# abhisrkckl/PulsePortraiture

Hardware: AMD Instinct MI355X
Metric: subint portrait fits/sec (phase+DM, 512ch×2048bin) at 1/2/4/8 MI355X (higher is better)
Workload: dtype f64

## Files before the change

pulseportraiture_amd/csrc/ppf_api.cpp:

```cpp
#include <hip/hip_runtime.h>

#include <algorithm>
#include <atomic>
#include <chrono>
#include <cmath>
#include <cstdarg>
#include <cstdio>
#include <cstdlib>
#include <cstring>
#include <map>
#include <mutex>
#include <string>
#include <thread>
#include <utility>
#include <vector>

#include "../../include/ppfit.h"
#include "ppf_internal.hpp"
#include "ppf_device.hpp"

struct ppf_ctx {
    int device;
    std::string err;
    mutable std::mutex err_mu;
    std::map<int, double2 *> tw;
    std::map<std::pair<int, int>, double2 *> cz;
    std::mutex tw_mu;
    bool prof = false;
    static constexpr int kRing = 256;
    static constexpr int kEv = 9;
    hipEvent_t ring[kRing][kEv] = {};
    bool ran[kRing][6] = {};
    std::vector<std::pair<hipEvent_t, hipEvent_t>> pass_ev[kRing];
    int npass[kRing] = {};
    std::vector<std::pair<hipEvent_t, hipEvent_t>> solv_ev[kRing];
    std::vector<int> solv_kind[kRing];
    int nsolv[kRing] = {};
    long ncalls = 0;
    unsigned *host_active = nullptr;
    void *lscr = nullptr;
    size_t lscr_bytes = 0;
    std::mutex lscr_mu;
};

namespace {

int fail(ppf_ctx *ctx, int code, const char *fmt, ...) {
    char buf[512];
    va_list ap;
    va_start(ap, fmt);
    vsnprintf(buf, sizeof buf, fmt, ap);
    va_end(ap);
    if (ctx) {
        std::lock_guard<std::mutex> lk(ctx->err_mu);
        ctx->err = buf;
    }
    return code;
}

int hip_fail(ppf_ctx *ctx, hipError_t e, const char *where) {
    return fail(ctx, PPF_EHIP, "%s: %s", where, hipGetErrorString(e));
}

bool pow2_in_range(int nbin) {
    return nbin >= 32 && nbin <= 8192 && (nbin & (nbin - 1)) == 0;
}

bool nbin_supported(int nbin) {
    return nbin >= 32 && nbin <= 8192 && ppf::fft_len_supported(ppf::rfft_len(nbin));
}

int fft_log2(int n) {
    if (n < 1 || (n & (n - 1))) return 0;
    int l = 0;
    while ((1 << l) < n) ++l;
    return l;
}

int rfft_log2(int nbin) { return (nbin & 1) ? 0 : fft_log2(nbin / 2); }

int ilog2(int n) {
    int l = 0;
    while ((1 << l) < n) ++l;
    return l;
}

int noise_kc(int nharm, int frac) {
    return (int)((1.0 - std::pow((double)frac, -1.0)) * (double)nharm);
}

int twiddles(ppf_ctx *ctx, int nbin, hipStream_t st, const double2 **T, const double2 **T2) {
    std::lock_guard<std::mutex> lock(ctx->tw_mu);
    auto it = ctx->tw.find(nbin);
    if (it == ctx->tw.end()) {
        const int N = ppf::rfft_len(nbin);
        double2 *p = nullptr;
        hipError_t e = hipMalloc(&p, sizeof(double2) * 2 * (size_t)N);
        if (e != hipSuccess) return hip_fail(ctx, e, "hipMalloc(twiddles)");
        e = ppf::launch_twiddles(N, p, p + N, st);
        if (e != hipSuccess) return hip_fail(ctx, e, "k_twiddles");
        e = hipStreamSynchronize(st);
        if (e != hipSuccess) return hip_fail(ctx, e, "hipStreamSynchronize(twiddles)");
        it = ctx->tw.emplace(nbin, p).first;
    }
    *T = it->second;
    *T2 = it->second + ppf::rfft_len(nbin);
    return PPF_OK;
}

constexpr unsigned kUnset = 0xFFFFFFFFu;
int read_back(ppf_ctx *ctx, unsigned *host, const unsigned *dev, int n, hipStream_t st, bool spin) {
    volatile unsigned *h = host;
    for (int i = 0; i < n; ++i) h[i] = kUnset;
    std::atomic_thread_fence(std::memory_order_seq_cst);
    hipError_t e = hipMemcpyAsync(host, dev, n * sizeof(unsigned), hipMemcpyDeviceToHost, st);
    if (e != hipSuccess) return hip_fail(ctx, e, "hipMemcpyAsync");
    if (spin) {
        const auto t0 = std::chrono::steady_clock::now();
        for (;;) {
            bool done = true;
            for (int i = 0; i < n; ++i) done = done && h[i] != kUnset;
            if (done) {
                std::atomic_thread_fence(std::memory_order_seq_cst);
                return PPF_OK;
            }
            const auto dt = std::chrono::steady_clock::now() - t0;
            if (dt > std::chrono::seconds(2)) break;
            if (dt > std::chrono::microseconds(50)) std::this_thread::yield();
            else __builtin_ia32_pause();
        }
    }
    if ((e = hipStreamSynchronize(st)) != hipSuccess) return hip_fail(ctx, e, "hipStreamSynchronize");
    return PPF_OK;
}

bool cz_plan(int Ns, int K, ppf::CzPlan &c) {
    if (Ns < 2 * ppf::kBlock || K < 2) return false;
    int P = 64;
    while (P < K + 255) P *= 2;
    if (P < 512 || P > 2048) return false;
    c.Ns = Ns; c.K = K; c.P = P; c.J = P - K + 1; c.Q = (Ns + c.J - 1) / c.J;
    return true;
}
int cz_tables(ppf_ctx *ctx, const ppf::CzPlan &c, hipStream_t st, const double2 **B, const double2 **T) {
    const double2 *T2;
    int rc = twiddles(ctx, 2 * c.P, st, T, &T2);
    if (rc) return rc;
    std::lock_guard<std::mutex> lock(ctx->tw_mu);
    const auto key = std::make_pair(c.Ns, c.K);
    auto it = ctx->cz.find(key);
    if (it == ctx->cz.end()) {
        double2 *p = nullptr;
        hipError_t e = hipMalloc(&p, sizeof(double2) * (size_t)c.Q * c.P);
        if (e != hipSuccess) return hip_fail(ctx, e, "hipMalloc(cz)");
        e = ppf::launch_cz_table(c, p, *T, st);
        if (e != hipSuccess) return hip_fail(ctx, e, "k_cz_table");
        e = hipStreamSynchronize(st);
        if (e != hipSuccess) return hip_fail(ctx, e, "hipStreamSynchronize(cz)");
        it = ctx->cz.emplace(key, p).first;
    }
    *B = it->second;
    return PPF_OK;
}

struct FitLayout {
    size_t M, X, chan, stats, x0, gP, gw, nuref, Msum, gpart, gwx, gflag, state, partials, active, mom, dphi,
        mres, hcen, Mpow, MP, KC, needx, xslot, xtile, rclist, Bt, total;
    int lng;
    size_t spec, lchirp, lA, lY, gprof, gspec, gsh;
    int64_t lrows;
    int nblk, cb, cbd, nblkd;
    int fused;
    int momx;
    int xcap;
    int tiled;
    int xnh;
};

static bool mom16_layout(const FitLayout &L, int nbin) {
    return L.momx || (!L.fused && !ppf::is_pow2(ppf::rfft_len(nbin)));
}


size_t align256(size_t x) { return (x + 255) & ~(size_t)255; }

bool bluestein_plan(int64_t nbin, int64_t n, bool packed, ppf::LongNoiseArgs &a);

bool grid_gsh(int nbin, int Ns, bool lng) {
    const size_t fb = lng ? 0 : (size_t)ppf::rfft_len(nbin) * sizeof(double2);
    return fb + ((size_t)nbin / 2 + 2) * sizeof(double2) + (size_t)(Ns + 8) * sizeof(double) > 150u * 1024u;
}
bool long_fit_ok(const ppf_fit_desc *d) {
    ppf::LongNoiseArgs f;
    if (d->guess && ((size_t)d->nbin / 2 + 2) * sizeof(double2) > 150u * 1024u) return false;
    return !nbin_supported(d->nbin) && d->nbin > 4095 &&
           bluestein_plan(d->nbin, (d->nbin & 1) ? d->nbin : d->nbin / 2, !(d->nbin & 1), f);
}

FitLayout fit_layout(const ppf_fit_desc *d) {
    FitLayout L{};
    const size_t nharm = (size_t)d->nbin / 2 + 1;
    const size_t nsub = (size_t)d->nsub, nchan = (size_t)d->nchan;
    L.cb = d->nchan < 32 ? d->nchan : 32;
    L.nblk = (d->nchan + L.cb - 1) / L.cb;
    L.fused = ppf::xspec_wave_supported(rfft_log2(d->nbin), L.cb) ? 1 : 0;
    const bool mom_auto = d->guess && rfft_log2(d->nbin) == 10;
    L.momx = (L.fused && !(d->options & PPF_OPT_FUSED_MOM) &&
              ((d->options & PPF_OPT_MOM_X) || mom_auto)) ? 1 : 0;
    L.xcap = (L.fused && d->x_subints > 0 && d->x_subints < d->nsub) ? d->x_subints : d->nsub;
    if (L.fused && (d->options & PPF_OPT_NO_X)) L.xcap = 0;
    if (L.momx) L.xcap = d->nsub;
    L.cbd = d->nchan < 128 ? d->nchan : 128;
    L.nblkd = (d->nchan + L.cbd - 1) / L.cbd;
    size_t o = 0;
    L.M = o;     o += align256(sizeof(double2) * (size_t)(d->nmodel > 0 ? d->nmodel : 1) * nchan * nharm);
    L.tiled = (L.momx && ppf::xspec_tiled(rfft_log2(d->nbin))) ? 1 : 0;
    L.xnh = L.tiled ? (int)ppf::xtile_harm((int64_t)nharm) : (int)nharm;
    L.X = o;     o += align256(sizeof(double2) * (size_t)L.xcap * nchan * (size_t)L.xnh);
    L.chan = o;  o += align256(sizeof(double) * nsub * nchan * 4);
    L.stats = o; o += align256(sizeof(double) * nsub * 2 * nchan * 10);
    L.x0 = o;    o += align256(sizeof(double) * nsub * 8);
    L.state = o; o += align256(ppf::tr_state_bytes() * nsub);
    L.partials = o; o += align256(sizeof(double) * nsub * (size_t)ppf::pass_blocks(d->nchan) * 21);
    L.active = o; o += 256;
    L.mom = o;   o += align256(sizeof(double2) * nsub * 2 * nchan * (size_t)ppf::kMoments);
    L.dphi = o;  o += align256(sizeof(double) * nsub * nchan * 2);
    L.mres = o;  o += align256(sizeof(double) * nsub * 2 * nchan);
    L.hcen = o;  o += mom16_layout(L, d->nbin) ? align256(sizeof(double) * nsub * 2 * nchan) : 0;
    L.Mpow = o;  o += align256(sizeof(double) * (size_t)(d->nmodel > 0 ? d->nmodel : 1) * nchan);
    L.MP = o;    o += align256(sizeof(double) * (size_t)(d->nmodel > 0 ? d->nmodel : 1) * nchan * nharm);
    L.KC = o;    o += align256(sizeof(int32_t) * (size_t)(d->nmodel > 0 ? d->nmodel : 1) * nchan);
    L.needx = o; o += align256(nsub);
    L.xslot = o; o += align256(sizeof(int32_t) * nsub);
    L.xtile = o; o += L.tiled ? align256(nsub) : 0;
    L.rclist = o; o += align256(sizeof(int32_t) * nsub);
    L.Bt = o;    o += align256(sizeof(double) * (nharm - 1) / 2 * 16);
    if (d->guess) {
        L.gP = o; o += align256(sizeof(double) * nsub * (size_t)L.nblkd * (size_t)d->nbin);
        L.gw = o; o += align256(sizeof(double) * nsub * (size_t)L.nblkd * 2);
        L.nuref = o; o += align256(sizeof(double) * nsub);
        L.Msum = o; o += align256(sizeof(double2) * (size_t)(d->nmodel > 0 ? d->nmodel : 1) * nharm);
        if (L.fused) {
            const size_t ng = (size_t)ppf::guess_slots(rfft_log2(d->nbin));
            L.gpart = o; o += align256(sizeof(double2) * nsub * (size_t)L.nblk * ng);
            L.gwx = o;   o += align256(sizeof(double) * nsub * (size_t)L.nblk * 3);
            L.gflag = o; o += align256(nsub);
        }
    }
    L.lng = long_fit_ok(d) ? 1 : 0;
    if (L.lng) {
        ppf::LongNoiseArgs f;
        bluestein_plan(d->nbin, (d->nbin & 1) ? d->nbin : d->nbin / 2, !(d->nbin & 1), f);
        const size_t row_b = (size_t)f.M * sizeof(double2);
        const int64_t rows = (int64_t)(nsub > (size_t)(d->nmodel > 0 ? d->nmodel : 1) ? nsub
                                       : (size_t)(d->nmodel > 0 ? d->nmodel : 1)) * (int64_t)nchan;
        int64_t rc = (int64_t)((size_t)(256u << 20) / (2 * row_b));
        if (rc < 1) rc = 1;
        L.lrows = rows < rc ? rows : rc;
        L.spec = o;   o += align256(sizeof(double2) * nsub * nchan * nharm);
        if (d->guess) {
            L.gprof = o; o += align256(sizeof(double) * nsub * (size_t)d->nbin);
            L.gspec = o; o += align256(sizeof(double2) * nsub * nharm);
        }
        L.lchirp = o; o += align256(2 * row_b);
        L.lA = o;     o += align256((size_t)L.lrows * row_b);
        L.lY = o;     o += align256((size_t)L.lrows * row_b);
    }
    if (d->guess && grid_gsh(d->nbin, d->guess_Ns, L.lng)) {
        L.gsh = o; o += align256(sizeof(double) * nsub * ((size_t)d->guess_Ns + 8));
    }
    L.total = o;
    return L;
}

int long_rfft_rows(ppf_ctx *ctx, const FitLayout &L, char *ws, int64_t nbin, int64_t nrows, int dtype,
                   const void *in, double2 *out, bool chirp_ready, hipStream_t st) {
    ppf::LongNoiseArgs f;
    if (!bluestein_plan(nbin, (nbin & 1) ? nbin : nbin / 2, !(nbin & 1), f))
        return fail(ctx, PPF_EUNSUP, "nbin=%lld", (long long)nbin);
    const double2 *T1, *T2, *unused;
    int rc;
    if ((rc = twiddles(ctx, (int)(2 * f.M1), st, &T1, &unused))) return rc;
    if ((rc = twiddles(ctx, (int)(2 * f.M2), st, &T2, &unused))) return rc;
    double2 *Bf = (double2 *)(ws + L.lchirp);
    hipError_t e;
    if (!chirp_ready && (e = ppf::launch_chirp_ft(f, Bf, Bf + f.M, T1, T2, st)) != hipSuccess)
        return hip_fail(ctx, e, "k_lf_chirp");
    f.in_dtype = dtype;
    f.in = in;
    for (int64_t r0 = 0; r0 < nrows; r0 += L.lrows) {
        f.row0 = r0;
        const int64_t nr = nrows - r0 < L.lrows ? nrows - r0 : L.lrows;
        if ((e = ppf::launch_rfft_long(f, nr, (double2 *)(ws + L.lA), (double2 *)(ws + L.lY), Bf, out, T1, T2,
                                       st)) != hipSuccess)
            return hip_fail(ctx, e, "k_lr_spec");
    }
    return PPF_OK;
}

int check_fit_desc(ppf_ctx *ctx, const ppf_fit_desc *d) {
    if (!d) return fail(ctx, PPF_EINVAL, "null descriptor");
    if (d->nsub < 1 || d->nchan < 1) return fail(ctx, PPF_EINVAL, "nsub=%d nchan=%d", d->nsub, d->nchan);
    if (!nbin_supported(d->nbin) && !long_fit_ok(d))
        return fail(ctx, PPF_EUNSUP,
                    "nbin=%d: must be even in [32, 8192] or odd in [33, 4095], or longer without the "
                    "GetTOAs guess (up to 2^23 transform points)", d->nbin);
    if (d->data_dtype != PPF_F32 && d->data_dtype != PPF_F64)
        return fail(ctx, PPF_EINVAL, "data_dtype=%d", d->data_dtype);
    if (d->nmodel < 1) return fail(ctx, PPF_EINVAL, "nmodel=%d", d->nmodel);
    if (!d->data || !d->model || !d->freqs || !d->P || !d->init || !d->fit_flags || !d->nu_fits ||
        !d->nu_outs || !d->results || !d->scales || !d->scale_errs || !d->channel_snrs ||
        !d->covariance)
        return fail(ctx, PPF_EINVAL, "required pointer is NULL");
    if (d->mode != PPF_MODE_FULL && d->mode != PPF_MODE_LEGACY2)
        return fail(ctx, PPF_EINVAL, "mode=%d", d->mode);
    if (d->guess) {
        if (!d->guess_weights || !d->guess_DM) return fail(ctx, PPF_EINVAL, "guess needs weights and DM");
        if (d->guess_Ns < 1 || d->guess_Ns > 65536) return fail(ctx, PPF_EINVAL, "guess_Ns=%d", d->guess_Ns);
    }
    if (!d->workspace) return fail(ctx, PPF_EINVAL, "workspace is NULL");
    FitLayout L = fit_layout(d);
    if (d->workspace_bytes < L.total)
        return fail(ctx, PPF_ENOMEM, "workspace %zu < %zu bytes", d->workspace_bytes, L.total);
    return PPF_OK;
}

}

extern "C" {

int ppf_abi_version(void) { return PPF_ABI_VERSION; }
size_t ppf_sizeof_fit_desc(void) { return sizeof(ppf_fit_desc); }
size_t ppf_sizeof_result(void) { return sizeof(ppf_result); }

int ppf_create(int device, ppf_ctx **out) {
    if (!out) return PPF_EINVAL;
    *out = nullptr;
    int n = 0;
    hipError_t e = hipGetDeviceCount(&n);
    if (e != hipSuccess || n == 0) return PPF_EHIP;
    if (device < 0 || device >= n) return PPF_EINVAL;
    ppf_ctx *c = new ppf_ctx();
    c->device = device;
    *out = c;
    return PPF_OK;
}

void ppf_destroy(ppf_ctx *ctx) {
    if (!ctx) return;
    (void)hipSetDevice(ctx->device);
    for (auto &kv : ctx->tw) (void)hipFree(kv.second);
    for (auto &kv : ctx->cz) (void)hipFree(kv.second);
    for (auto &set : ctx->ring)
        for (auto &e : set)
            if (e) (void)hipEventDestroy(e);
    for (auto &v : ctx->pass_ev)
        for (auto &pr : v) {
            (void)hipEventDestroy(pr.first);
            (void)hipEventDestroy(pr.second);
        }
    for (auto &v : ctx->solv_ev)
        for (auto &pr : v) {
            (void)hipEventDestroy(pr.first);
            (void)hipEventDestroy(pr.second);
        }
    if (ctx->host_active) (void)hipHostFree(ctx->host_active);
    if (ctx->lscr) (void)hipFree(ctx->lscr);
    delete ctx;
}

int ppf_set_profiling(ppf_ctx *ctx, int enable) {
    if (!ctx) return PPF_EINVAL;
    hipError_t e = hipSetDevice(ctx->device);
    if (e != hipSuccess) return hip_fail(ctx, e, "hipSetDevice");
    if (enable && !ctx->ring[0][0])
        for (auto &set : ctx->ring)
            for (auto &ev : set)
                if ((e = hipEventCreate(&ev)) != hipSuccess) return hip_fail(ctx, e, "hipEventCreate");
    ctx->prof = enable != 0;
    ctx->ncalls = 0;
    return PPF_OK;
}

int ppf_stage_ms_history(ppf_ctx *ctx, int n, double *ms) {
    if (!ctx || !ms || n < 0) return PPF_EINVAL;
    if (!ctx->prof) return fail(ctx, PPF_EINVAL, "profiling is off");
    long avail = ctx->ncalls < ppf_ctx::kRing ? ctx->ncalls : ppf_ctx::kRing;
    if (n > avail) n = (int)avail;
    for (int c = 0; c < n; ++c) {
        int slot = (int)((ctx->ncalls - n + c) % ppf_ctx::kRing);
        hipError_t e = hipEventSynchronize(ctx->ring[slot][4]);
        if (e != hipSuccess) return hip_fail(ctx, e, "hipEventSynchronize");
        for (int i = 0; i < 4; ++i) {
            float t = 0.f;
            if (ctx->ran[slot][i]) {
                e = hipEventElapsedTime(&t, ctx->ring[slot][i], ctx->ring[slot][i + 1]);
                if (e != hipSuccess) return hip_fail(ctx, e, "hipEventElapsedTime");
            }
// ... 11 lines not shown
    for (int c = 0; c < n; ++c) {
        int slot = (int)((ctx->ncalls - n + c) % ppf_ctx::kRing);
        hipError_t e = hipEventSynchronize(ctx->ring[slot][4]);
        if (e != hipSuccess) return hip_fail(ctx, e, "hipEventSynchronize");
        for (int i = 0; i < 2; ++i) {
            float t = 0.f;
            if (ctx->ran[slot][4 + i]) {
                e = hipEventElapsedTime(&t, ctx->ring[slot][5 + 2 * i], ctx->ring[slot][6 + 2 * i]);
                if (e != hipSuccess) return hip_fail(ctx, e, "hipEventElapsedTime");
            }
            ms[c * 2 + i] = (double)t;
        }
    }
    return n;
}

int ppf_pass_ms_history(ppf_ctx *ctx, int n, double *ms) {
    if (!ctx || !ms || n < 0) return PPF_EINVAL;
    if (!ctx->prof) return fail(ctx, PPF_EINVAL, "profiling is off");
    long avail = ctx->ncalls < ppf_ctx::kRing ? ctx->ncalls : ppf_ctx::kRing;
    if (n > avail) n = (int)avail;
    for (int c = 0; c < n; ++c) {
        int slot = (int)((ctx->ncalls - n + c) % ppf_ctx::kRing);
        double tot = 0.0;
        for (int i = 0; i < ctx->npass[slot]; ++i) {
            const auto &pr = ctx->pass_ev[slot][i];
            hipError_t e = hipEventSynchronize(pr.second);
            if (e != hipSuccess) return hip_fail(ctx, e, "hipEventSynchronize");
            float t = 0.f;
            e = hipEventElapsedTime(&t, pr.first, pr.second);
            if (e != hipSuccess) return hip_fail(ctx, e, "hipEventElapsedTime");
            tot += (double)t;
        }
        ms[c * 2 + 0] = tot;
        ms[c * 2 + 1] = (double)ctx->npass[slot];
    }
    return n;
}

int ppf_solver_ms_history(ppf_ctx *ctx, int n, double *ms) {
    if (!ctx || !ms || n < 0) return PPF_EINVAL;
    if (!ctx->prof) return fail(ctx, PPF_EINVAL, "profiling is off");
    long avail = ctx->ncalls < ppf_ctx::kRing ? ctx->ncalls : ppf_ctx::kRing;
    if (n > avail) n = (int)avail;
    for (int c = 0; c < n; ++c) {
        int slot = (int)((ctx->ncalls - n + c) % ppf_ctx::kRing);
        double *o = ms + c * 6;
        for (int i = 0; i < 6; ++i) o[i] = 0.0;
        for (int i = 0; i < ctx->nsolv[slot]; ++i) {
            const auto &pr = ctx->solv_ev[slot][i];
            hipError_t e = hipEventSynchronize(pr.second);
            if (e != hipSuccess) return hip_fail(ctx, e, "hipEventSynchronize");
            float t = 0.f;
            e = hipEventElapsedTime(&t, pr.first, pr.second);
            if (e != hipSuccess) return hip_fail(ctx, e, "hipEventElapsedTime");
            const int k = ctx->solv_kind[slot][i];
            o[2 * k] += (double)t;
            o[2 * k + 1] += 1.0;
        }
    }
    return n;
}

int ppf_last_stage_ms(ppf_ctx *ctx, double *ms4) {
    int n = ppf_stage_ms_history(ctx, 1, ms4);
    if (n < 0) return n;
    return n == 1 ? PPF_OK : fail(ctx, PPF_EINVAL, "no profiled call yet");
}

const char *ppf_last_error(const ppf_ctx *ctx) {
    if (!ctx) return "null context";
    thread_local std::string copy;
    std::lock_guard<std::mutex> lk(ctx->err_mu);
    copy = ctx->err;
    return copy.c_str();
}

size_t ppf_fit_workspace_bytes(const ppf_fit_desc *desc) {
    if (!desc || desc->nsub < 1 || desc->nchan < 1 || (!nbin_supported(desc->nbin) && !long_fit_ok(desc)))
        return 0;
    return fit_layout(desc).total;
}

int ppf_fit_batch(ppf_ctx *ctx, const ppf_fit_desc *d, void *stream) {
    if (!ctx) return PPF_EINVAL;
    int rc = check_fit_desc(ctx, d);
    if (rc) return rc;
    hipError_t e = hipSetDevice(ctx->device);
    if (e != hipSuccess) return hip_fail(ctx, e, "hipSetDevice");
    hipStream_t st = (hipStream_t)stream;
    const FitLayout L = fit_layout(d);
    const double2 *T = nullptr, *T2 = nullptr;
    if (!L.lng && (rc = twiddles(ctx, d->nbin, st, &T, &T2))) return rc;
    char *ws = (char *)d->workspace;
    double2 *Mft = (double2 *)(ws + L.M);
    const int nharm = d->nbin / 2 + 1;
    const int kc = noise_kc(nharm, 4);

    const int slot = (int)(ctx->ncalls % ppf_ctx::kRing);
    auto mark = [&](int i) {
        if (ctx->prof) (void)hipEventRecord(ctx->ring[slot][i], st);
    };
    for (int i = 0; i < 4; ++i) ctx->ran[slot][i] = true;
    ctx->npass[slot] = 0;
    ctx->nsolv[slot] = 0;
    auto solv_begin = [&](int kind) -> std::pair<hipEvent_t, hipEvent_t> * {
        if (!ctx->prof) return nullptr;
        auto &v = ctx->solv_ev[slot];
        auto &kv = ctx->solv_kind[slot];
        if ((int)v.size() <= ctx->nsolv[slot]) {
            std::pair<hipEvent_t, hipEvent_t> pr{};
            if (hipEventCreate(&pr.first) != hipSuccess) return nullptr;
            if (hipEventCreate(&pr.second) != hipSuccess) {
                (void)hipEventDestroy(pr.first);
                return nullptr;
            }
            v.push_back(pr);
            kv.push_back(0);
        }
        kv[ctx->nsolv[slot]] = kind;
        auto *pe = &v[ctx->nsolv[slot]++];
        (void)hipEventRecord(pe->first, st);
        return pe;
    };
    auto solv_end = [&](std::pair<hipEvent_t, hipEvent_t> *pe) {
        if (pe) (void)hipEventRecord(pe->second, st);
    };
    ctx->ran[slot][2] = d->guess != 0;
    ctx->ran[slot][4] = ctx->ran[slot][5] = false;
    mark(0);
    if (L.lng) {
        if ((rc = long_rfft_rows(ctx, L, ws, d->nbin, (int64_t)d->nmodel * d->nchan, PPF_F64, d->model, Mft,
                                 false, st)))
            return rc;
    } else {
        ppf::RfftArgs ra{d->nbin, rfft_log2(d->nbin), PPF_F64, d->model, T, T2, Mft};
        if ((e = ppf::launch_rfft_rows(ra, (int64_t)d->nmodel * d->nchan, st)) != hipSuccess)
            return hip_fail(ctx, e, "k_rfft_rows");
    }
    double *Mpow = (double *)(ws + L.Mpow);
    if ((e = ppf::launch_model_pow_t(Mft, d->nchan, nharm, d->nmodel, (double *)(ws + L.MP), st)) !=
        hipSuccess)
        return hip_fail(ctx, e, "k_model_pow_t");
    if ((e = ppf::launch_model_cut((const double *)(ws + L.MP), d->nchan, nharm, d->nmodel,
                                   (d->options & PPF_OPT_NO_HCUT) != 0, (int32_t *)(ws + L.KC),
                                   st)) != hipSuccess)
        return hip_fail(ctx, e, "k_model_cut");
    if ((e = ppf::launch_model_pow(Mft, d->nchan, nharm, d->nmodel, Mpow, st)) != hipSuccess)
        return hip_fail(ctx, e, "k_model_pow");
    const int use_moments = 1;
    uint8_t *needx = (uint8_t *)(ws + L.needx);
    int32_t *xslot = (int32_t *)(ws + L.xslot);
    uint8_t *xtile = L.tiled ? (uint8_t *)(ws + L.xtile) : nullptr;
    if ((e = ppf::launch_classify(d->nsub, d->fit_flags, d->init, d->log10_tau, L.fused && !L.momx, L.xcap,
                                  needx, xslot, xtile, st)) != hipSuccess)
        return hip_fail(ctx, e, "k_classify");
    uint8_t *gflag = nullptr;
    if (d->guess && L.fused && ppf::xspec_guess_fused_n(rfft_log2(d->nbin))) {
        gflag = (uint8_t *)(ws + L.gflag);
        const int klim = 64 * ppf::guess_npl(rfft_log2(d->nbin));
        if ((e = ppf::launch_gflag(d->nsub, d->nchan, needx, (const int32_t *)(ws + L.KC),
                                   d->model_index, klim, gflag, st)) != hipSuccess)
            return hip_fail(ctx, e, "k_gflag");
    }
    mark(1);

    ppf::XspecArgs xa{};
    xa.nsub = d->nsub; xa.nchan = d->nchan; xa.nbin = d->nbin; xa.log2N = rfft_log2(d->nbin);
    xa.kc = kc; xa.nblk = L.nblk; xa.cb = L.cb; xa.dtype = d->data_dtype;
    constexpr long long kOrder2Bytes = 32ll << 20;
    const long long model_bytes = (long long)d->nchan * (d->nbin / 2 + 1) * 16;
    const int xcd1 = (L.nblk % 8 == 0) ? 1 : 0;
    xa.xcd_swizzle = (xcd1 && model_bytes > kOrder2Bytes) ? 2 : xcd1;
    xa.data = d->data; xa.Mft = Mft; xa.model_index = d->model_index; xa.mask = d->chan_mask;
    xa.errs = d->errs; xa.freqs = d->freqs; xa.P = d->P; xa.T = T; xa.T2 = T2;
    xa.X = (double2 *)(ws + L.X); xa.chan = (double *)(ws + L.chan);
    xa.Mpow = Mpow;
    xa.xslot = xslot;
    xa.xtile = xtile;
    xa.xnh = L.xnh;
    xa.gflag = gflag;
    if (gflag) {
        xa.gpart = (double2 *)(ws + L.gpart);
        xa.gw = (double *)(ws + L.gwx);
        xa.guess_weights = d->guess_weights;
        xa.guess_DM = d->guess_DM;
        xa.nu_fits = d->nu_fits;
        xa.guess_ref = d->guess_ref;
    }
    const bool wave = L.fused != 0;
    const bool fused = wave && use_moments && !L.momx;
    xa.needx = (fused || L.momx) ? needx : nullptr;
    xa.KC = (fused || L.momx || !wave) ? (const int32_t *)(ws + L.KC) : nullptr;
    if (wave) {
        if (!(fused && L.xcap == 0) &&
            (e = ppf::launch_xspec_wave(xa, st)) != hipSuccess)
            return hip_fail(ctx, e, "k_xspec_w");
    } else if (L.lng) {
        double2 *spec = (double2 *)(ws + L.spec);
        if ((rc = long_rfft_rows(ctx, L, ws, d->nbin, (int64_t)d->nsub * d->nchan, d->data_dtype, d->data, spec,
                                 true, st)))
            return rc;
        xa.spec = spec;
        if ((e = ppf::launch_xspec_spec(xa, st)) != hipSuccess) return hip_fail(ctx, e, "k_xspec_spec");
    } else {
        if ((e = ppf::launch_xspec(xa, st)) != hipSuccess) return hip_fail(ctx, e, "k_xspec");
    }
    mark(2);

    if (d->guess) {
        ppf::DsumArgs da{};
        da.nsub = d->nsub; da.nchan = d->nchan; da.nbin = d->nbin; da.dtype = d->data_dtype;
        da.cbd = L.cbd; da.nblkd = L.nblkd; da.data = d->data; da.mask = d->chan_mask;
        da.freqs = d->freqs; da.P = d->P; da.guess_DM = d->guess_DM;
        da.guess_weights = d->guess_weights;
        da.guess_ref = d->guess_ref; da.nu_fits = d->nu_fits;
        da.gP = (double *)(ws + L.gP); da.gw = (double *)(ws + L.gw);
        da.nuref = (double *)(ws + L.nuref);
        da.gflag = gflag;
        mark(7);
        if ((e = ppf::launch_dsum(da, st)) != hipSuccess) return hip_fail(ctx, e, "k_dsum");
        mark(8);
        ctx->ran[slot][5] = true;
        double2 *msum = (double2 *)(ws + L.Msum);
        if ((e = ppf::launch_model_sum(Mft, d->nchan, nharm, d->nmodel, msum, st)) != hipSuccess)
            return hip_fail(ctx, e, "k_model_sum");
        ppf::GuessArgs ga{};
        ga.nsub = d->nsub; ga.nchan = d->nchan; ga.nbin = d->nbin; ga.log2N = rfft_log2(d->nbin);
        ga.kc = kc; ga.nblkd = L.nblkd; ga.Ns = d->guess_Ns; ga.mask = d->chan_mask;
        ga.guess_ref = d->guess_ref;
        ga.freqs = d->freqs; ga.P = d->P; ga.guess_DM = d->guess_DM; ga.guess_tau = d->guess_tau;
        ga.nu_fits = d->nu_fits; ga.gP = da.gP; ga.gw = da.gw; ga.T = T; ga.T2 = T2;
        ga.KC = (const int32_t *)(ws + L.KC);
        ga.x0 = (double *)(ws + L.x0); ga.Msum = msum; ga.Mft = Mft;
        ga.model_index = d->model_index;
        ga.gflag = gflag;
        ga.gpart = xa.gpart;
        ga.gwx = xa.gw;
        ga.nblk = L.nblk;
        if (L.lng) {
            double *prof = (double *)(ws + L.gprof);
            double2 *gspec = (double2 *)(ws + L.gspec);
            if ((e = ppf::launch_gsum(d->nsub, L.nblkd, d->nbin, da.gP, prof, st)) != hipSuccess)
                return hip_fail(ctx, e, "k_gsum");
            if ((rc = long_rfft_rows(ctx, L, ws, d->nbin, d->nsub, PPF_F64, prof, gspec, true, st))) return rc;
            ga.gspec = gspec;
        }
        if (grid_gsh(d->nbin, ga.Ns, L.lng)) ga.gsh = (double *)(ws + L.gsh);
        ppf::CzPlan cz{};
        if (cz_plan(ga.Ns, d->nbin / 2 + 1, cz)) {
            if ((rc = cz_tables(ctx, cz, st, &ga.czB, &ga.czT))) return rc;
            ga.czP = cz.P; ga.czJ = cz.J; ga.czQ = cz.Q; ga.czK = cz.K;
        }
        if ((e = ppf::launch_guess(ga, st)) != hipSuccess) return hip_fail(ctx, e, "k_guess");
    }
    mark(3);

    ppf::SolveArgs sa{};
    sa.nsub = d->nsub; sa.nchan = d->nchan; sa.nbin = d->nbin;
    sa.X = xa.X; sa.Mft = Mft; sa.model_index = d->model_index; sa.chan = xa.chan;
    sa.MP = (const double *)(ws + L.MP);
    sa.KC = (const int32_t *)(ws + L.KC);
    sa.freqs = d->freqs; sa.P = d->P; sa.mask = d->chan_mask; sa.init = d->init;
    sa.fit_flags = d->fit_flags; sa.nu_fits = d->nu_fits; sa.nu_outs = d->nu_outs;
    sa.bounds = d->bounds;
    sa.log10_tau = d->log10_tau; sa.option = d->option; sa.is_toa = d->is_toa; sa.mode = d->mode;
    sa.max_iter = d->max_iter; sa.guess = d->guess; sa.x0 = (double *)(ws + L.x0);
    sa.newton = (d->options & PPF_OPT_SCIPY_TR) ? 0 : 1;
    sa.stats = (double *)(ws + L.stats); sa.results = d->results; sa.scales = d->scales;
    sa.scale_errs = d->scale_errs; sa.channel_snrs = d->channel_snrs; sa.covariance = d->covariance;
    sa.any_plain = 1;
    sa.any_scat = 1;
    sa.state = (ppf::TRState *)(ws + L.state);
    sa.partials = (double *)(ws + L.partials);
    sa.active = (unsigned *)(ws + L.active);
    sa.rc_count = sa.active + 1;
    sa.rc_list = (int32_t *)(ws + L.rclist);
    sa.kinds = (unsigned *)(ws + L.active + 16);
    if (!ctx->host_active) {
        e = hipHostMalloc((void **)&ctx->host_active, 4 * sizeof(unsigned));
        if (e != hipSuccess) return hip_fail(ctx, e, "hipHostMalloc");
    }
    if ((e = hipMemsetAsync(sa.kinds, 0, 2 * sizeof(unsigned), st)) != hipSuccess)
        return hip_fail(ctx, e, "hipMemsetAsync");
    sa.moments = use_moments;
    sa.mom = (double2 *)(ws + L.mom);
    sa.dphi = (double *)(ws + L.dphi);
    sa.mres = (double *)(ws + L.mres);
    const bool m16 = mom16_layout(L, d->nbin);
    sa.mom16 = m16;
    sa.hcen = m16 ? (double *)(ws + L.hcen) : nullptr;
    sa.xslot = xslot;
    sa.xtile = xtile;
    sa.xnh = L.xnh;
    if (sa.moments) sa.any_plain = 0;
    if ((e = ppf::launch_tr_init(sa, st)) != hipSuccess) return hip_fail(ctx, e, "k_tr_init");
    const bool no_stream = sa.moments && L.fused && L.xcap == 0;
    bool kinds_late = !no_stream && sa.moments && (d->options & PPF_OPT_NO_X);
    bool any_mom = true, any_pass = false;
    if (!no_stream && !kinds_late) {
        if ((rc = read_back(ctx, ctx->host_active + 1, sa.kinds, 2, st, d->options & PPF_OPT_SPIN_WAIT))) return rc;
        any_mom = ctx->host_active[1] != 0;
        any_pass = ctx->host_active[2] != 0;
    }
    ppf::XmomArgs ma{};
    ma.nsub = d->nsub; ma.nchan = d->nchan; ma.nbin = d->nbin; ma.log2N = xa.log2N;
    ma.nblk = L.nblk; ma.cb = L.cb; ma.dtype = d->data_dtype; ma.xcd_swizzle = xcd1;
    ma.data = d->data; ma.Mft = Mft; ma.model_index = d->model_index; ma.mask = d->chan_mask;
    ma.chan = xa.chan; ma.dphi = sa.dphi; ma.T = T; ma.T2 = T2; ma.state = sa.state;
    ma.mom = (double *)sa.mom;
    ma.Bt = (const double *)(ws + L.Bt);
    ma.kc = kc; ma.errs = d->errs; ma.Mpow = Mpow; ma.mres = sa.mres; ma.nmodel = d->nmodel;
    ma.rc_count = sa.rc_count; ma.rc_list = sa.rc_list;
    ma.KC = (const int32_t *)(ws + L.KC);
    if (fused && (e = ppf::launch_btab(d->nbin / 2, (double *)(ws + L.Bt), st)) != hipSuccess)
        return hip_fail(ctx, e, "k_btab");
    const int maxiter = d->max_iter > 0 ? d->max_iter : 200 * 5;
    int iter = 0;
    for (int group = (sa.moments && !any_pass) ? 1 : (sa.moments ? 3 : 6); any_mom || any_pass;
         group = sa.moments ? 2 : 4) {
        for (int g = 0; g < group; ++g) {
            if (any_pass) {
                std::pair<hipEvent_t, hipEvent_t> *pe = nullptr;
                if (ctx->prof) {
                    auto &v = ctx->pass_ev[slot];
                    if ((int)v.size() <= ctx->npass[slot]) {
                        std::pair<hipEvent_t, hipEvent_t> pr{};
                        if ((e = hipEventCreate(&pr.first)) != hipSuccess)
                            return hip_fail(ctx, e, "hipEventCreate");
                        if ((e = hipEventCreate(&pr.second)) != hipSuccess) {
                            (void)hipEventDestroy(pr.first);
                            return hip_fail(ctx, e, "hipEventCreate");
                        }
                        v.push_back(pr);
                    }
                    pe = &v[ctx->npass[slot]++];
                    (void)hipEventRecord(pe->first, st);
                }
                if ((e = ppf::launch_pass(sa, st)) != hipSuccess) return hip_fail(ctx, e, "k_pass");
                if (pe) (void)hipEventRecord(pe->second, st);
            }
            if (sa.moments && any_mom) {
                const bool full = iter == 0 && g == 0;
                if (full) mark(5);
                if (fused && !full) {
                    ppf::XmomArgs mr = ma;
                    if (mr.cb > 8) {
                        mr.cb = 8;
                        mr.nblk = (d->nchan + 7) / 8;
                        mr.xcd_swizzle = (mr.nblk % 8 == 0) ? 1 : 0;
                    }
                    e = ppf::launch_xmom(mr, false, st);
                } else {
                    e = fused ? ppf::launch_xmom(ma, full, st) : ppf::launch_moments(sa, st);
                }
                if (e != hipSuccess) return hip_fail(ctx, e, fused ? "k_xmom" : "k_moments");
                if (full) {
                    mark(6);
                    ctx->ran[slot][4] = true;
                }
            }
            if ((e = hipMemsetAsync(sa.active, 0, 2 * sizeof(unsigned), st)) != hipSuccess)
                return hip_fail(ctx, e, "hipMemsetAsync");
            if (any_pass) {
                auto *pe = solv_begin(1);
                if ((e = ppf::launch_tr_step(sa, st)) != hipSuccess) return hip_fail(ctx, e, "k_tr_step");
                solv_end(pe);
            }
            if (sa.moments && any_mom) {
                auto *pe = solv_begin(0);
                if ((e = ppf::launch_tr_mom(sa, st)) != hipSuccess) return hip_fail(ctx, e, "k_tr_mom");
                solv_end(pe);
            }
        }
        iter += group;
        if (kinds_late && (e = hipMemcpyAsync(ctx->host_active + 1, sa.kinds, 2 * sizeof(unsigned),
                                              hipMemcpyDeviceToHost, st)) != hipSuccess)
            return hip_fail(ctx, e, "hipMemcpyAsync");
        if ((rc = read_back(ctx, ctx->host_active, sa.active, 1, st, d->options & PPF_OPT_SPIN_WAIT))) return rc;
        if (kinds_late) {
            kinds_late = false;
            if (ctx->host_active[2] != 0) {
                any_pass = true;
                continue;
            }
        }
        if (*ctx->host_active == 0 || iter > maxiter + 2) break;
    }
    {
        auto *pe = solv_begin(2);
        if ((e = ppf::launch_postfit(sa, st)) != hipSuccess) return hip_fail(ctx, e, "k_postfit");
        solv_end(pe);
    }
    mark(4);
    if (ctx->prof) ++ctx->ncalls;
    return PPF_OK;
}

int ppf_fit2_batch(ppf_ctx *ctx, const ppf_fit_desc *desc, void *stream) {
    if (!desc) return fail(ctx, PPF_EINVAL, "null descriptor");
    ppf_fit_desc d = *desc;
    d.mode = PPF_MODE_LEGACY2;
    return ppf_fit_batch(ctx, &d, stream);
}

static int rotate_batch(ppf_ctx *ctx, int64_t nrows, int32_t nbin, int32_t in_dtype, const void *in,
                        const double *phases, double *out, void *stream, bool ref_len) {
    if (!ctx) return PPF_EINVAL;
    if (!nbin_supported(nbin)) return fail(ctx, PPF_EUNSUP, "nbin=%d unsupported", nbin);
    if (nrows < 0 || (nrows > 0 && (!in || !phases || !out)))
        return fail(ctx, PPF_EINVAL, "bad rotate arguments");
    if (in_dtype != PPF_F32 && in_dtype != PPF_F64) return fail(ctx, PPF_EINVAL, "in_dtype");
    if (nrows == 0) return PPF_OK;
    hipError_t e = hipSetDevice(ctx->device);
    if (e != hipSuccess) return hip_fail(ctx, e, "hipSetDevice");
    hipStream_t st = (hipStream_t)stream;
    const double2 *T, *T2;
    int rc = twiddles(ctx, nbin, st, &T, &T2);
    if (rc) return rc;
    ppf::RotateArgs a{nbin, rfft_log2(nbin), in_dtype, in, phases, T, T2, out, 0, T, T2};
    if (ref_len && (nbin & 1)) {
        a.ref_len = 1;
        if ((rc = twiddles(ctx, nbin - 1, st, &a.Te, &a.T2e))) return rc;
    }
    if ((e = ppf::launch_rotate(a, nrows, st)) != hipSuccess) return hip_fail(ctx, e, "k_rotate");
    return PPF_OK;
}

int ppf_rotate_batch(ppf_ctx *ctx, int64_t nrows, int32_t nbin, int32_t in_dtype, const void *in,
                     const double *phases, double *out, void *stream) {
    return rotate_batch(ctx, nrows, nbin, in_dtype, in, phases, out, stream, false);
}

int ppf_rotate_batch_ref(ppf_ctx *ctx, int64_t nrows, int32_t nbin, int32_t in_dtype, const void *in,
                         const double *phases, double *out, void *stream) {
    return rotate_batch(ctx, nrows, nbin, in_dtype, in, phases, out, stream, true);
}
// ... 623 lines not shown
```

pulseportraiture_amd/csrc/ppf_internal.hpp:

```cpp
#pragma once
#include <hip/hip_runtime.h>
#include <stdint.h>

#include "../../include/ppfit.h"

namespace ppf {

struct RfftArgs {
    int nbin, log2N, dtype;
    const void *in;
    const double2 *T, *T2;
    double2 *out;
};

struct XspecArgs {
    int nsub, nchan, nbin, log2N, kc, nblk, cb, dtype, xcd_swizzle;
    const void *data;
    const double2 *Mft;
    const int32_t *model_index;
    const uint8_t *mask;
    const double *errs;
    const double *freqs, *P;
    const double2 *T, *T2;
    double2 *X;
    double *chan;
    const double2 *spec;
    const double *Mpow;
    const uint8_t *needx;
    const int32_t *KC;
    const int32_t *xslot;
    const uint8_t *xtile;
    int xnh;
    const uint8_t *gflag;
    double2 *gpart;
    double *gw;
    const double *guess_weights, *guess_DM, *nu_fits;
    int guess_ref;
};

__host__ __device__ constexpr int guess_npl(int log2N) { return log2N >= 10 ? 7 : (log2N == 9 ? 3 : (log2N == 8 ? 2 : 1)); }
__host__ __device__ constexpr int guess_slots(int log2N) { return 64 * guess_npl(log2N); }

struct DsumArgs {
    int nsub, nchan, nbin, dtype, cbd, nblkd;
    int guess_ref;
    const double *nu_fits;
    const void *data;
    const uint8_t *mask;
    const double *freqs, *P, *guess_DM, *guess_weights;
    double *gP;
    double *gw;
    const uint8_t *gflag;
    double *nuref;
};

struct XmomArgs {
    int nsub, nchan, nbin, log2N, nblk, cb, dtype, xcd_swizzle, nmodel;
    const void *data;
    const double2 *Mft;
    const int32_t *model_index;
    const uint8_t *mask;
    double *chan;
    const double *dphi;
    const double2 *T, *T2;
    const void *state;
    double *mom;
    const double *Bt;
    int kc;
    const double *errs;
    const double *Mpow;
    double *mres;
    const int32_t *KC;
    const unsigned *rc_count;
    const int32_t *rc_list;
};

struct GuessArgs {
    int nsub, nchan, nbin, log2N, kc, nblkd, Ns;
    int guess_ref;
    const uint8_t *mask;
    const double *freqs, *P, *guess_DM, *guess_tau, *nu_fits;
    const double *gP;
    const double *gw;
    const double2 *T, *T2;
    double *x0;
    const double2 *Msum;
    const double2 *Mft;
    const int32_t *model_index;
    const int32_t *KC;
    const uint8_t *gflag;
    const double2 *gpart;
    const double *gwx;
    int nblk;
    const double2 *czB, *czT;
    int czP, czJ, czQ, czK;
    const double2 *gspec;
    double *gsh;
};

struct CzPlan {
    int Ns, K, P, J, Q;
};
hipError_t launch_cz_table(const CzPlan &c, double2 *B, const double2 *T, hipStream_t st);

struct TRState;

struct SolveArgs {
    int nsub, nchan, nbin;
    const double2 *X, *Mft;
    const double *MP;
    const int32_t *KC;
    const int32_t *model_index;
    const double *chan;
    const double *freqs, *P;
    const uint8_t *mask;
    const double *init;
    const int32_t *fit_flags;
    const double *nu_fits, *nu_outs;
    const double *bounds;
    int log10_tau, option, is_toa, mode, max_iter, guess;
    int newton;
    const double *x0;
    double *stats;
    ppf_result *results;
    double *scales, *scale_errs, *channel_snrs, *covariance;
    int any_plain, any_scat;
    TRState *state;
    double *partials;
    unsigned *active;
    unsigned *kinds;
    int moments;
    double2 *mom;
    double *dphi;
    double *mres;
    int mom16;
    double *hcen;
    const int32_t *xslot;
    const uint8_t *xtile;
    int xnh;
    unsigned *rc_count;
    int32_t *rc_list;
};

struct RotateArgs {
    int nbin, log2N, dtype;
    const void *in;
    const double *phases;
    const double2 *T, *T2;
    double *out;
    int ref_len;
    const double2 *Te, *T2e;
};

struct InstRespArgs {
    int nbin;
    const double *src;
    const int32_t *src_row;
    const double *table;
    const double *widths;
    const double2 *T, *T2;
    double *out;
};

struct AlignArgs {
    int nsub, nchan, nbin, log2N, dtype, ngroup;
    const void *in;
    const double *phases;
    const double *weights;
    const double2 *T, *T2;
    double2 *part;
    double *wpart;
    double *out;
    double *wsum;
};
int align_groups(int nsub, int nchan);
hipError_t launch_align(const AlignArgs &a, hipStream_t st);
bool align_wave_supported(int log2N);
hipError_t launch_align_part_w(const AlignArgs &a, hipStream_t st);
hipError_t launch_align_phases(int nsub, int nchan, const double *results, const double *freqs, const double *P,
                               const uint8_t *mask, const double *scales, const double *errs, double *phases,
                               double *weights, hipStream_t st);

struct ResidArgs {
    int nbin, log2N, dtype;
    const void *in;
    const double *phases;
    const double *model;
    const int32_t *model_row;
    const double *scales, *errs;
    double dof;
    const double2 *T, *T2;
    double *out;
};
hipError_t launch_resid_chi2(const ResidArgs &a, int64_t nrows, hipStream_t st);

struct NoiseArgs {
    int nbin, log2N, dtype, kc;
    const void *in;
    const double2 *T, *T2;
    double *out;
};

struct LongNoiseArgs {
    int64_t nbin;
    int64_t n;
    int64_t M, M1, M2;
    int log2M, log2M1;
    int packed;
    int bluestein;
    int64_t nharm, kc;
    int in_dtype;
    const void *in;
    int64_t row0;
};
struct LongRotArgs {
    LongNoiseArgs f, b;
    int out_even;
    int64_t nout;
    const double *phases;
    const double *taus;
    double *out;
};
struct LongPassArgs {
    int64_t nbatch;
    int len, log2len;
    int64_t in_stride, in_bstride, out_stride, out_bstride, row_elems, M;
    int twiddle, inverse;
    const double2 *in;
    double2 *out;
    const double2 *T;
};

struct PhaseShiftArgs {
    int nbin, log2N, dtype, kc, Ns;
    double lo, hi;
    const void *data;
    const double *model;
    const int32_t *model_index;
    const double *noise;
    const double2 *T, *T2;
    double *out;
    const double2 *Dspec, *Mspec;
    double *gsh;
};

struct SynthArgs {
    int nsub, nchan, nbin, log2N, dtype;
    const double2 *Mft;
    const double *freqs, *phi, *DM, *P;
    double nu_ref, noise;
    uint64_t seed;
    int64_t first;
    const double2 *T, *T2;
    void *out;
};

struct ScalesArgs {
    int nsub, nchan, nharm, log10_tau;
    const double2 *D;
    const double2 *M;
    const int32_t *model_index;
    const double *errs_FT;
    const double *params;
    const double *P;
    const double *freqs;
    const double *nus;
    double *out;
};
hipError_t launch_scales(const ScalesArgs &a, hipStream_t st);

struct UnpackArgs {
    int nsub, npol, nchan, nbin;
    int elem;
    int pol_mode;
    int rm_baseline, win;
    const uint8_t *raw;
    int64_t sub_stride;
    const float *scl, *offs;
    const float *wts;
    float *out;
    double *part;
    double *total;
    int32_t *wstart;
    double *stats;
};
hipError_t launch_unpack(const UnpackArgs &a, hipStream_t st);
hipError_t launch_copy_host(const void *src_dev, void *dst, int64_t nbytes, hipStream_t st);
size_t unpack_partials(int nsub, int nchan, int nbin);

struct GaussArgs {
    int nport, nchan, nbin, log2N, ngauss, npar;
    int code[3];
    const double *params;
    const double *scat_index;
    const double *freqs;
    const double *nu_ref;
    const double2 *T, *T2;
    const double2 *Te, *T2e;
    double *out;
    double *taus_out;
};
hipError_t launch_gauss_port(const GaussArgs &a, hipStream_t st);

struct SplineArgs {
    int nport, nchan, nbin_model, nbin, ncomp, nknots, degree;
    int log2N0, log2N1;
    const double *mean_prof;
    const double *eigvec;
    const double *knots;
    const double *coefs;
    const double *freqs;
    const double2 *T0, *T20;
    const double2 *T1, *T21;
    double *out;
};
constexpr int kSplineMaxComp = 64;
constexpr int kSplineMaxDeg = 5;
hipError_t launch_spline_port(const SplineArgs &a, hipStream_t st);

hipError_t launch_twiddles(int N, double2 *T, double2 *T2, hipStream_t st);
hipError_t launch_rfft_rows(const RfftArgs &a, int64_t nrows, hipStream_t st);
hipError_t launch_xspec(const XspecArgs &a, hipStream_t st);
hipError_t launch_guess(const GuessArgs &a, hipStream_t st);
hipError_t launch_gflag(int nsub, int nchan, const uint8_t *needx, const int32_t *KC,
                        const int32_t *model_index, int klim, uint8_t *gflag, hipStream_t st);
hipError_t launch_dsum(const DsumArgs &a, hipStream_t st);
bool xspec_wave_supported(int log2N, int cb);
bool xspec_wm_supported(int nbin);
bool xspec_guess_fused_n(int log2N);
hipError_t launch_xspec_wm(const XspecArgs &a, hipStream_t st);
hipError_t launch_xspec_wave(const XspecArgs &a, hipStream_t st);
hipError_t launch_xmom(const XmomArgs &a, bool full, hipStream_t st);
hipError_t launch_btab(int N, double *Bt, hipStream_t st);
hipError_t launch_classify(int nsub, const int32_t *fit_flags, const double *init, int log10_tau,
                           int fused, int xcap, uint8_t *needx, int32_t *xslot, uint8_t *xtile,
                           hipStream_t st);
bool xspec_tiled(int log2N);
constexpr int kXTile = 8;
inline int64_t xtile_harm(int64_t nharm) { return (nharm + kXTile - 1) / kXTile * kXTile; }
hipError_t launch_model_pow(const double2 *Mft, int nchan, int nharm, int nmodel, double *out,
                            hipStream_t st);
hipError_t launch_model_sum(const double2 *Mft, int nchan, int nharm, int nmodel, double2 *out,
                            hipStream_t st);
hipError_t launch_tr_init(const SolveArgs &a, hipStream_t st);
hipError_t launch_pass(const SolveArgs &a, hipStream_t st);
hipError_t launch_tr_step(const SolveArgs &a, hipStream_t st);
hipError_t launch_moments(const SolveArgs &a, hipStream_t st);
hipError_t launch_tr_mom(const SolveArgs &a, hipStream_t st);
constexpr int kMoments = 32;
constexpr double kNewtonR0 = 10.0;
constexpr double kNewtonTol = 1e-12;
constexpr double kSubsetSwitch = 1.0;
constexpr int kSubsetMaxStride = 16;
hipError_t launch_postfit(const SolveArgs &a, hipStream_t st);
size_t tr_state_bytes();
int pass_blocks(int nchan);
hipError_t launch_rotate(const RotateArgs &a, int64_t nrows, hipStream_t st);
hipError_t launch_inst_resp(const InstRespArgs &a, int64_t nrows, hipStream_t st);
hipError_t launch_noise(const NoiseArgs &a, int64_t nrows, hipStream_t st);
int lf_pow_blocks(const LongNoiseArgs &a);
hipError_t launch_chirp_ft(const LongNoiseArgs &a, double2 *Bf, double2 *Bs, const double2 *T1,
                           const double2 *T2, hipStream_t st);
hipError_t launch_rfft_long(const LongNoiseArgs &f, int64_t nrows, double2 *A, double2 *Y, const double2 *Bf,
                            double2 *out, const double2 *T1, const double2 *T2, hipStream_t st);
hipError_t launch_xspec_spec(const XspecArgs &a, hipStream_t st);
hipError_t launch_gsum(int nsub, int nblkd, int nbin, const double *gP, double *prof, hipStream_t st);
hipError_t launch_rotate_long(const LongRotArgs &r, int64_t nrows, double2 *A, double2 *Y, const double2 *Bff,
                              const double2 *Bfb, const double2 *T1f, const double2 *T2f, const double2 *T1b,
                              const double2 *T2b, hipStream_t st);
hipError_t launch_noise_long(const LongNoiseArgs &a, int64_t nrows, double2 *A, double2 *Y,
                             const double2 *Bf, double *part, double *out, const double2 *T1,
                             const double2 *T2, hipStream_t st);
bool noise_wave_supported(int log2N);
hipError_t launch_noise_wave(const NoiseArgs &a, int64_t nrows, hipStream_t st);
hipError_t launch_phase_shift(const PhaseShiftArgs &a, int nprof, hipStream_t st);
hipError_t launch_synth(const SynthArgs &a, hipStream_t st);
constexpr double kCutRel = 1e-28;
hipError_t launch_model_cut(const double *MP, int nchan, int nharm, int nmodel, bool off,
                            int32_t *KC, hipStream_t st);
hipError_t launch_model_pow_t(const double2 *Mft, int nchan, int nharm, int nmodel, double *MP,
                              hipStream_t st);

}
```

pulseportraiture_amd/csrc/ppf_kernels.hip:

```cpp
#include <cstdlib>
#include <type_traits>

#include "ppf_device.hpp"
#include "ppf_internal.hpp"

namespace ppf {

__device__ __forceinline__ void load_row(double2 *buf, const void *src, int dtype, int64_t row,
                                         int nbin) {
    const int N = nbin >> 1;
    if (nbin & 1) {
        if (dtype == 0) {
            const float *s = reinterpret_cast<const float *>(src) + row * (int64_t)nbin;
            for (int j = threadIdx.x; j < nbin; j += kBlock) buf[j] = cmk((double)s[j], 0.0);
        } else {
            const double *s = reinterpret_cast<const double *>(src) + row * (int64_t)nbin;
            for (int j = threadIdx.x; j < nbin; j += kBlock) buf[j] = cmk(s[j], 0.0);
        }
        return;
    }
    if (dtype == 0) {
        const float2 *s = reinterpret_cast<const float2 *>(src) + row * (int64_t)N;
        for (int j = threadIdx.x; j < N; j += kBlock) {
            float2 v = s[j];
// ... 386 lines not shown
                }
            }
            sh[j0] = -acc0 * inv_err2;
            if (j1 < Ns) sh[j1] = -acc1 * inv_err2;
        }
    } else {
        for (int j = wave; j < Ns; j += kWaves) {
            double ph = (double)j * step + lo;
            double f = wave_fps_eval(xm, nharm, ph, inv_err2);
            if (lane == 0) sh[j] = f;
        }
    }
    __syncthreads();
    if (wave == 0) {
        int jmin = 0;
        double fmin_ = sh[0];
        for (int j = 1; j < Ns; ++j)
            if (sh[j] < fmin_) { fmin_ = sh[j]; jmin = j; }
        double x0 = (double)jmin * step + lo;
        double sim0 = x0, sim1 = (x0 != 0.0) ? 1.05 * x0 : 0.00025;
        int nf = 0;
        double f0 = wave_fps_eval(xm, nharm, sim0, inv_err2); ++nf;
        double f1 = wave_fps_eval(xm, nharm, sim1, inv_err2); ++nf;
        if (f1 < f0) { double t = sim0; sim0 = sim1; sim1 = t; t = f0; f0 = f1; f1 = t; }
        int iters = 1;
        while (nf < 200 && iters < 200) {
            if (fabs(sim1 - sim0) <= 1e-4 && fabs(f0 - f1) <= 1e-4) break;
            double xbar = sim0;
            double xr = 2.0 * xbar - sim1;
            double fxr = wave_fps_eval(xm, nharm, xr, inv_err2); ++nf;
            bool shrink = false;
            if (fxr < f0) {
                double xe = 3.0 * xbar - 2.0 * sim1;
                double fxe = wave_fps_eval(xm, nharm, xe, inv_err2); ++nf;
                if (fxe < fxr) { sim1 = xe; f1 = fxe; } else { sim1 = xr; f1 = fxr; }
            } else {
                if (fxr < f1) {
                    double xc = 1.5 * xbar - 0.5 * sim1;
                    double fxc = wave_fps_eval(xm, nharm, xc, inv_err2); ++nf;
                    if (fxc <= fxr) { sim1 = xc; f1 = fxc; } else shrink = true;
                } else {
                    double xcc = 0.5 * xbar + 0.5 * sim1;
                    double fxcc = wave_fps_eval(xm, nharm, xcc, inv_err2); ++nf;
                    if (fxcc < f1) { sim1 = xcc; f1 = fxcc; } else shrink = true;
                }
                if (shrink) {
                    sim1 = sim0 + 0.5 * (sim1 - sim0);
                    f1 = wave_fps_eval(xm, nharm, sim1, inv_err2); ++nf;
                }
            }
            ++iters;
            if (f1 < f0) { double t = sim0; sim0 = sim1; sim1 = t; t = f0; f0 = f1; f1 = t; }
        }
        if (lane == 0) { sh[Ns] = sim0; sh[Ns + 1] = fmin(f0, f1); sh[Ns + 2] = (double)nf; }
    }
    __syncthreads();
    double ph = sh[Ns];
    if (fval) *fval = sh[Ns + 1];
    if (nfev) *nfev = (int)sh[Ns + 2];
    __syncthreads();
    return ph;
}

template <int DT, int JB>
__global__ __launch_bounds__(kBlock) void k_dsum(DsumArgs a) {
    using ElT = typename std::conditional<DT == 0, float, double>::type;
    __shared__ double red[kWaves * 4];
    const int tid = threadIdx.x;
    const int s = blockIdx.x / a.nblkd, blk = blockIdx.x % a.nblkd;
    if (a.gflag && a.gflag[s]) return;
    const int nbin = a.nbin;
    const uint8_t *mask = a.mask ? a.mask + (int64_t)s * a.nchan : nullptr;
    const double *fr = a.freqs + (int64_t)s * a.nchan;
    double v[2] = {0.0, 0.0};
    for (int n = tid; n < a.nchan; n += kBlock)
        if (!mask || mask[n]) { v[0] += fr[n]; v[1] += 1.0; }
    block_sum<2>(v, red);
    const double Dg = kDconst * a.guess_DM[s] / a.P[s];
    double nu_mean_m2 = pow(v[0] / v[1], -2.0);
    if (a.guess_ref) {
        const double nf = a.nu_fits[(int64_t)s * 3];
        if (nf == nf) nu_mean_m2 = pow(nf, -2.0);
    }
    const int c0 = blk * a.cbd, c1 = min(a.nchan, c0 + a.cbd);
    const ElT *rows = reinterpret_cast<const ElT *>(a.data) + (int64_t)s * a.nchan * nbin;
    double wsum = 0.0, wcnt = 0.0;
    for (int t0 = 0; t0 < nbin; t0 += JB * kBlock) {
        double p[JB];
#pragma unroll
        for (int j = 0; j < JB; ++j) p[j] = 0.0;
        for (int n = c0; n < c1; ++n) {
            if (mask && !mask[n]) continue;
            const double w = a.guess_weights[(int64_t)s * a.nchan + n];
            const double tau = (double)nbin * Dg * (pow(fr[n], -2.0) - nu_mean_m2);
            const double fl = floor(tau);
            const double f = tau - fl;
            const int i0 = (int)(fl - (double)nbin * floor(fl / (double)nbin));
            const double wa = w * (1.0 - f), wb = w * f;
            const ElT *x = rows + (int64_t)n * nbin;
#pragma unroll
            for (int j = 0; j < JB; ++j) {
                const int t = t0 + tid + j * kBlock;
                if (t < nbin) {
                    const int ia = t + i0 >= nbin ? t + i0 - nbin : t + i0;
                    const int ib = ia + 1 == nbin ? 0 : ia + 1;
                    p[j] = fma(wa, (double)x[ia], fma(wb, (double)x[ib], p[j]));
                }
            }
            if (t0 == 0) { wsum += w; wcnt += 1.0; }
        }
        double *out = a.gP + ((int64_t)s * a.nblkd + blk) * nbin;
#pragma unroll
        for (int j = 0; j < JB; ++j) {
            const int t = t0 + tid + j * kBlock;
            if (t < nbin) out[t] = p[j];
        }
    }
    if (tid == 0) {
        a.gw[((int64_t)s * a.nblkd + blk) * 2 + 0] = wsum;
        a.gw[((int64_t)s * a.nblkd + blk) * 2 + 1] = wcnt;
    }
}

__device__ __forceinline__ double nu_ref_m2(const DsumArgs &a, int s, int lane) {
    const uint8_t *mask = a.mask ? a.mask + (int64_t)s * a.nchan : nullptr;
    const double *fr = a.freqs + (int64_t)s * a.nchan;
    double v0 = 0.0, v1 = 0.0;
#pragma unroll 8
    for (int n = lane; n < a.nchan; n += 64) {
        const double f = fr[n];
        const bool ok = !mask || mask[n];
        v0 += ok ? f : 0.0;
        v1 += ok ? 1.0 : 0.0;
    }
    v0 = wave_sum(v0);
    v1 = wave_sum(v1);
    const double mu = v0 / v1;
    double nu_mean_m2 = 1.0 / (mu * mu);
    if (a.guess_ref) {
        const double nf = a.nu_fits[(int64_t)s * 3];
        if (nf == nf) nu_mean_m2 = 1.0 / (nf * nf);
    }
    return nu_mean_m2;
}

__global__ __launch_bounds__(64) void k_nu_ref(DsumArgs a) {
    const int s = blockIdx.x;
    if (a.gflag && a.gflag[s]) return;
    const double v = nu_ref_m2(a, s, threadIdx.x);
    if (threadIdx.x == 0) a.nuref[s] = v;
}

template <int DT, int LOG2NB>
__global__ __launch_bounds__(kBlock) void k_dsum_w(DsumArgs a) {
    using ElT = typename std::conditional<DT == 0, float, double>::type;
    typedef float vf4 __attribute__((ext_vector_type(4)));
    typedef double vd2 __attribute__((ext_vector_type(2)));
    using VecT = typename std::conditional<DT == 0, vf4, vd2>::type;
    constexpr int NB = 1 << LOG2NB, J = NB / 64, VW = 16 / (int)sizeof(ElT);
    constexpr int NL = NB / (64 * VW);
    extern __shared__ __attribute__((aligned(16))) double dlds[];
    const int lane = threadIdx.x & 63, wave = threadIdx.x >> 6;
    ElT *xs = reinterpret_cast<ElT *>(dlds) + wave * NB;
    const int s = blockIdx.x / a.nblkd, blk = blockIdx.x % a.nblkd;
    if (a.gflag && a.gflag[s]) return;
    const uint8_t *mask = a.mask ? a.mask + (int64_t)s * a.nchan : nullptr;
    const double *fr = a.freqs + (int64_t)s * a.nchan;
    const double *gwt = a.guess_weights + (int64_t)s * a.nchan;
    const double Dg = (double)NB * kDconst * a.guess_DM[s] / a.P[s];
    const double nu_mean_m2 = a.nuref ? a.nuref[s] : nu_ref_m2(a, s, lane);
    const int c0 = blk * a.cbd, c1 = min(a.nchan, c0 + a.cbd);
    const VecT *rows = reinterpret_cast<const VecT *>(a.data) + (int64_t)s * a.nchan * (NB / VW);
    double t_w[2], t_f[2];
    int t_m[2];
#pragma unroll
    for (int k = 0; k < 2; ++k) {
        const int ch = c0 + lane + 64 * k;
        const bool in = ch < c1;
        t_w[k] = in ? gwt[ch] : 0.0;
        t_f[k] = in ? fr[ch] : 1.0;
        t_m[k] = (in && (!mask || mask[ch])) ? 1 : 0;
    }
    auto usable = [&](int n) {
        const int r = n - c0;
        return n < c1 && __builtin_amdgcn_readlane(r < 64 ? t_m[0] : t_m[1], r & 63) != 0;
    };
    double acc[J];
#pragma unroll
    for (int j = 0; j < J; ++j) acc[j] = 0.0;
    double wsum = 0.0, wcnt = 0.0;
    int n = c0 + wave;
    while (n < c1 && !usable(n)) n += kWaves;
    VecT pre[NL];
    {
        const VecT *src = rows + (int64_t)min(n, c1 - 1) * (NB / VW);
#pragma unroll
        for (int i = 0; i < NL; ++i) pre[i] = src[lane + 64 * i];
    }
    while (n < c1) {
        wave_lds_sync();
#pragma unroll
        for (int i = 0; i < NL; ++i) reinterpret_cast<VecT *>(xs)[lane + 64 * i] = pre[i];
        int nn = n + kWaves;
        while (nn < c1 && !usable(nn)) nn += kWaves;
        {
            const VecT *src = rows + (int64_t)(nn < c1 ? nn : n) * (NB / VW);
#pragma unroll
            for (int i = 0; i < NL; ++i) pre[i] = src[lane + 64 * i];
        }
        const int r = n - c0;
        const double w = readlane_d(r < 64 ? t_w[0] : t_w[1], r & 63),
                     f0 = readlane_d(r < 64 ? t_f[0] : t_f[1], r & 63);
        const double tau = Dg * (1.0 / (f0 * f0) - nu_mean_m2);
        const double fl = floor(tau), f = tau - fl;
        const int i0 = (int)(fl - (double)NB * floor(fl / (double)NB));
        const double wa = w * (1.0 - f), wb = w * f;
        wave_lds_sync();
#pragma unroll
        for (int j = 0; j < J; ++j) {
            const int ia = (lane + 64 * j + i0) & (NB - 1);
            acc[j] = fma(wa, (double)xs[ia], fma(wb, (double)xs[(ia + 1) & (NB - 1)], acc[j]));
        }
        wsum += w;
        wcnt += 1.0;
        n = nn;
    }
    __syncthreads();
    double *part = dlds;
    for (int w2 = 0; w2 < kWaves; ++w2) {
        if (wave == w2) {
#pragma unroll
            for (int j = 0; j < J; ++j) {
                const int t = lane + 64 * j;
                part[t] = w2 == 0 ? acc[j] : part[t] + acc[j];
            }
        }
        __syncthreads();
    }
    double *out = a.gP + ((int64_t)s * a.nblkd + blk) * NB;
    for (int t = threadIdx.x; t < NB; t += kBlock) out[t] = part[t];
    __shared__ double wred[kWaves * 2];
    if (lane == 0) { wred[wave * 2] = wsum; wred[wave * 2 + 1] = wcnt; }
    __syncthreads();
    if (threadIdx.x == 0) {
        double s0 = 0.0, s1 = 0.0;
        for (int w2 = 0; w2 < kWaves; ++w2) { s0 += wred[w2 * 2]; s1 += wred[w2 * 2 + 1]; }
        a.gw[((int64_t)s * a.nblkd + blk) * 2 + 0] = s0;
        a.gw[((int64_t)s * a.nblkd + blk) * 2 + 1] = s1;
    }
}

template <int DT, int NBMAX>
__global__ __launch_bounds__(kBlock) void k_dsum_wn(DsumArgs a) {
    using ElT = typename std::conditional<DT == 0, float, double>::type;
    constexpr int J = NBMAX / 64;
    extern __shared__ __attribute__((aligned(16))) double dlds[];
    const int lane = threadIdx.x & 63, wave = threadIdx.x >> 6;
    const int nb = a.nbin;
    ElT *xs = reinterpret_cast<ElT *>(dlds) + wave * NBMAX;
    const int s = blockIdx.x / a.nblkd, blk = blockIdx.x % a.nblkd;
    if (a.gflag && a.gflag[s]) return;
    const uint8_t *mask = a.mask ? a.mask + (int64_t)s * a.nchan : nullptr;
    const double *fr = a.freqs + (int64_t)s * a.nchan;
    const double *gwt = a.guess_weights + (int64_t)s * a.nchan;
    const double Dg = (double)nb * kDconst * a.guess_DM[s] / a.P[s];
    const double nu_mean_m2 = a.nuref ? a.nuref[s] : nu_ref_m2(a, s, lane);
    const int c0 = blk * a.cbd, c1 = min(a.nchan, c0 + a.cbd);
    const ElT *rows = reinterpret_cast<const ElT *>(a.data) + (int64_t)s * a.nchan * nb;
    double t_w[2], t_f[2];
    int t_m[2];
#pragma unroll
    for (int k = 0; k < 2; ++k) {
        const int ch = c0 + lane + 64 * k;
        const bool in = ch < c1;
        t_w[k] = in ? gwt[ch] : 0.0;
        t_f[k] = in ? fr[ch] : 1.0;
        t_m[k] = (in && (!mask || mask[ch])) ? 1 : 0;
    }
    auto usable = [&](int n) {
        const int r = n - c0;
        return n < c1 && __builtin_amdgcn_readlane(r < 64 ? t_m[0] : t_m[1], r & 63) != 0;
    };
    double acc[J];
#pragma unroll
    for (int j = 0; j < J; ++j) acc[j] = 0.0;
    double wsum = 0.0, wcnt = 0.0;
    auto load = [&](ElT (&p)[J], int m) {
        const ElT *src = rows + (int64_t)m * nb;
#pragma unroll
        for (int i = 0; i < J; ++i) {
            const int t = lane + 64 * i;
            p[i] = src[t < nb ? t : nb - 1];
        }
    };
    int n = c0 + wave;
    while (n < c1 && !usable(n)) n += kWaves;
    ElT pre[J];
    load(pre, min(n, c1 - 1));
    while (n < c1) {
        wave_lds_sync();
#pragma unroll
        for (int i = 0; i < J; ++i) xs[lane + 64 * i] = pre[i];
        int nn = n + kWaves;
        while (nn < c1 && !usable(nn)) nn += kWaves;
        load(pre, nn < c1 ? nn : n);
        const int r = n - c0;
        const double w = readlane_d(r < 64 ? t_w[0] : t_w[1], r & 63),
                     f0 = readlane_d(r < 64 ? t_f[0] : t_f[1], r & 63);
        const double tau = Dg * (1.0 / (f0 * f0) - nu_mean_m2);
        const double fl = floor(tau), f = tau - fl;
        const int i0 = (int)(fl - (double)nb * floor(fl / (double)nb));
        const double wa = w * (1.0 - f), wb = w * f;
        wave_lds_sync();
#pragma unroll
        for (int j = 0; j < J; ++j) {
            const int t = lane + 64 * j;
            int ia = t + i0;
            ia -= ia >= nb ? nb : 0;
            const int ib = ia + 1 == nb ? 0 : ia + 1;
            if (t < nb) acc[j] = fma(wa, (double)xs[ia], fma(wb, (double)xs[ib], acc[j]));
        }
        wsum += w;
        wcnt += 1.0;
        n = nn;
    }
    __syncthreads();
    double *part = dlds;
    for (int w2 = 0; w2 < kWaves; ++w2) {
        if (wave == w2) {
#pragma unroll
            for (int j = 0; j < J; ++j) {
                const int t = lane + 64 * j;
                part[t] = w2 == 0 ? acc[j] : part[t] + acc[j];
            }
        }
        __syncthreads();
    }
    double *out = a.gP + ((int64_t)s * a.nblkd + blk) * nb;
    for (int t = threadIdx.x; t < nb; t += kBlock) out[t] = part[t];
    __shared__ double wred[kWaves * 2];
    if (lane == 0) { wred[wave * 2] = wsum; wred[wave * 2 + 1] = wcnt; }
    __syncthreads();
    if (threadIdx.x == 0) {
        double s0 = 0.0, s1 = 0.0;
        for (int w2 = 0; w2 < kWaves; ++w2) { s0 += wred[w2 * 2]; s1 += wred[w2 * 2 + 1]; }
        a.gw[((int64_t)s * a.nblkd + blk) * 2 + 0] = s0;
        a.gw[((int64_t)s * a.nblkd + blk) * 2 + 1] = s1;
    }
}

template <bool MX, int CZL = 0, bool GS = false>
__global__ __launch_bounds__(kBlock) void k_guess(GuessArgs a) {
    extern __shared__ __attribute__((aligned(16))) double2 lds[];
    __shared__ double red[kWaves * 4];
    const int N = a.nbin >> 1, nharm = N + 1, s = blockIdx.x, tid = threadIdx.x;
    const bool odd = a.nbin & 1;
    const bool pre = a.gspec != nullptr;
    double2 *z = lds,
            *xm = lds + (pre ? 0 : (a.czB && a.czP > rfft_len(a.nbin) ? a.czP : rfft_len(a.nbin)));
    double *sh = GS ? a.gsh + (int64_t)s * (a.Ns + 8) : reinterpret_cast<double *>(xm + nharm + 1);
    const bool fused = a.gflag && a.gflag[s];
    const int NL = guess_slots(a.log2N);
    if (tid == 0) {
        double w0 = 0.0, w1 = 0.0, w2 = 0.0;
        if (fused) {
#pragma unroll 8
            for (int b = 0; b < a.nblk; ++b) {
                w0 += a.gwx[((int64_t)s * a.nblk + b) * 3 + 0];
                w1 += a.gwx[((int64_t)s * a.nblk + b) * 3 + 1];
                w2 += a.gwx[((int64_t)s * a.nblk + b) * 3 + 2];
            }
        } else {
#pragma unroll 8
            for (int b = 0; b < a.nblkd; ++b) {
                w0 += a.gw[((int64_t)s * a.nblkd + b) * 2 + 0];
                w1 += a.gw[((int64_t)s * a.nblkd + b) * 2 + 1];
            }
        }
        sh[0] = w0; sh[1] = w1; sh[2] = w2;
    }
    if (!fused && !pre) {
        for (int j = tid; odd && j < a.nbin; j += kBlock) {
            double pj = 0.0;
#pragma unroll 8
            for (int b = 0; b < a.nblkd; ++b) pj += a.gP[((int64_t)s * a.nblkd + b) * a.nbin + j];
            z[j] = cmk(pj, 0.0);
        }
        for (int j = tid; !odd && j < N; j += kBlock) {
            double pe = 0.0, po = 0.0;
#pragma unroll 8
            for (int b = 0; b < a.nblkd; ++b) {
                const double *pp = a.gP + ((int64_t)s * a.nblkd + b) * a.nbin;
                pe += pp[2 * j];
                po += pp[2 * j + 1];
            }
            z[j] = cmk(pe, po);
        }
    }
    __syncthreads();
    const double wsum = sh[0], cnt = sh[1];
    if (!fused && !pre) lds_fft_n<MX>(z, rfft_len(a.nbin), a.T, false);
// ... 433 lines not shown
#pragma unroll
            for (int i = 0; i < 2 * KMAX; ++i) {
                const int j = threadIdx.x + i * kBlock;
                if (j < nbin) v[i] = row[j];
            }
            __syncthreads();
#pragma unroll
            for (int i = 0; i < 2 * KMAX; ++i) {
                const int j = threadIdx.x + i * kBlock;
                if (j < nbin) lds[j] = cmk(v[i], 0.0);
            }
            __syncthreads();
        }
        lds_fft_n<MX>(lds, rfft_len(nbin), a.T, false);
        double2 Xk[KMAX], Xn[KMAX];
#pragma unroll
        for (int i = 0; i < KMAX; ++i) {
            const int k = threadIdx.x + i * kBlock;
            if (k < KH) {
                double2 X1 = rbin(lds, nbin, a.T2, k);
                double2 X2 = odd ? cmk(0.0, 0.0) : rfft_bin(lds, N, a.T2, N - k);
                if (tn != 0.0) {
                    X1 = cmul(X1, scat_recip((2.0 * kPi * (double)k) * tn));
                    if (!odd) X2 = cmul(X2, scat_recip((2.0 * kPi * (double)(N - k)) * tn));
                }
                if (k == 0) { X1.y = 0.0; X2.y = 0.0; }
                Xk[i] = X1;
                Xn[i] = X2;
            }
        }
        __syncthreads();
        if (odd) {
#pragma unroll
            for (int i = 0; i < KMAX; ++i) {
                const int k = threadIdx.x + i * kBlock;
                if (k < KH) lds[k] = Xk[i];
            }
            __syncthreads();
#pragma unroll
            for (int i = 0; i < KMAX; ++i) {
                const int k = threadIdx.x + i * kBlock;
                if (k < N) {
                    Xk[i] = lds[k];
                    Xn[i] = lds[N - k];
                    if (k == 0) Xn[i].y = 0.0;
                }
            }
            __syncthreads();
#pragma unroll
            for (int i = 0; i < KMAX; ++i) {
                const int k = threadIdx.x + i * kBlock;
                if (k < N) lds[k] = irfft_prebin(Xk[i], Xn[i], a.T2e[k]);
            }
            __syncthreads();
            lds_fft_n<MX>(lds, N, a.Te, true);
            const double sc = 1.0 / (double)N;
            double *o = a.out + (int64_t)blockIdx.x * nbin;
            for (int j = threadIdx.x; j < N; j += kBlock) {
                const double2 z = cscale(lds[j], sc);
                o[2 * j] = z.x;
                o[2 * j + 1] = z.y;
            }
            if (threadIdx.x == 0) o[nbin - 1] = 0.0;
            return;
        }
#pragma unroll
        for (int i = 0; i < KMAX; ++i) {
            const int k = threadIdx.x + i * kBlock;
            if (k < KH) lds[k] = irfft_prebin(Xk[i], Xn[i], a.T2[k]);
        }
        __syncthreads();
        lds_fft_n<MX>(lds, rfft_len(nbin), a.T, true);
        const double sc = 1.0 / (double)N;
        double2 *o = reinterpret_cast<double2 *>(a.out) + (int64_t)blockIdx.x * N;
        for (int j = threadIdx.x; j < N; j += kBlock) o[j] = cscale(lds[j], sc);
        return;
    }
    __syncthreads();
    if (nbin & 1) {
        double *o = a.out + (int64_t)blockIdx.x * nbin;
        for (int j = threadIdx.x; j < nbin; j += kBlock) o[j] = row[j];
        return;
    }
    double2 *o = reinterpret_cast<double2 *>(a.out) + (int64_t)blockIdx.x * N;
    for (int j = threadIdx.x; j < N; j += kBlock) o[j] = lds[j];
}

static inline int kmax_pow2(int N) {
    int q = (N + kBlock - 1) / kBlock, k = 1;
    while (k < q) k <<= 1;
    return k;
}
static inline int log2i(int n) {
    int l = 0;
    while ((1 << l) < n) ++l;
    return l;
}

#define MXL(mx, KER, A, ...)                                          \
    do {                                                              \
        if (mx) hipLaunchKernelGGL((KER<A, true>), __VA_ARGS__);      \
        else hipLaunchKernelGGL((KER<A, false>), __VA_ARGS__);        \
    } while (0)

hipError_t launch_twiddles(int N, double2 *T, double2 *T2, hipStream_t st) {
    hipLaunchKernelGGL(k_twiddles, dim3((N + 255) / 256), dim3(256), 0, st, N, T, T2);
    return hipGetLastError();
}
hipError_t launch_rfft_rows(const RfftArgs &a, int64_t nrows, hipStream_t st) {
    size_t lds = (size_t)rfft_len(a.nbin) * sizeof(double2);
    if (is_pow2(rfft_len(a.nbin))) hipLaunchKernelGGL(k_rfft_rows<false>, dim3((unsigned)nrows), dim3(kBlock), lds, st, a);
    else hipLaunchKernelGGL(k_rfft_rows<true>, dim3((unsigned)nrows), dim3(kBlock), lds, st, a);
    return hipGetLastError();
}
template <int L2>
static void launch_xspec_t(const XspecArgs &a, hipStream_t st) {
    constexpr int N = 1 << L2;
    size_t lds = (size_t)N * sizeof(double2) * (N <= 1024 ? 3 : 1);
    dim3 g((unsigned)((int64_t)a.nsub * a.nblk)), b(kBlock);
    if (a.dtype == 0) hipLaunchKernelGGL((k_xspec<L2, 0>), g, b, lds, st, a);
    else hipLaunchKernelGGL((k_xspec<L2, 1>), g, b, lds, st, a);
}

hipError_t launch_xspec(const XspecArgs &a, hipStream_t st) {
    switch (a.log2N) {
        case 4: launch_xspec_t<4>(a, st); break;
        case 5: launch_xspec_t<5>(a, st); break;
        case 6: launch_xspec_t<6>(a, st); break;
        case 7: launch_xspec_t<7>(a, st); break;
        case 8: launch_xspec_t<8>(a, st); break;
        case 9: launch_xspec_t<9>(a, st); break;
        case 10: launch_xspec_t<10>(a, st); break;
        case 11: launch_xspec_t<11>(a, st); break;
        case 12: launch_xspec_t<12>(a, st); break;
        case 0: {
            if (xspec_wm_supported(a.nbin) && a.cb <= 64) return launch_xspec_wm(a, st);
            dim3 g((unsigned)((int64_t)a.nsub * a.nblk)), b(kBlock);
            const size_t lds = (size_t)rfft_len(a.nbin) * sizeof(double2);
            if (a.dtype == 0) hipLaunchKernelGGL((k_xspec_any<0>), g, b, lds, st, a);
            else hipLaunchKernelGGL((k_xspec_any<1>), g, b, lds, st, a);
            break;
        }
        default: return hipErrorInvalidValue;
    }
    return hipGetLastError();
}
bool dsum_wave_supported(int nbin) { return nbin >= 256 && nbin <= 2048 && is_pow2(nbin); }

template <int DT, int L2>
static void launch_dsum_w(const DsumArgs &a, hipStream_t st) {
    constexpr int NB = 1 << L2;
    const size_t row = (size_t)kWaves * NB * (DT == 0 ? 4 : 8);
    const size_t lds = row > (size_t)NB * 8 ? row : (size_t)NB * 8;
    hipLaunchKernelGGL((k_dsum_w<DT, L2>), dim3((unsigned)((int64_t)a.nsub * a.nblkd)), dim3(kBlock),
                       lds, st, a);
}

hipError_t launch_dsum(const DsumArgs &a_in, hipStream_t st) {
    DsumArgs a = a_in;
    if (a.nuref && a.nchan >= 2048 && a.nbin <= 2048) {
        hipLaunchKernelGGL(k_nu_ref, dim3((unsigned)a.nsub), dim3(64), 0, st, a);
    } else {
        a.nuref = nullptr;
    }
    if (dsum_wave_supported(a.nbin)) {
        switch (__builtin_ctz((unsigned)a.nbin) * 2 + a.dtype) {
            case 16: launch_dsum_w<0, 8>(a, st); break;
            case 17: launch_dsum_w<1, 8>(a, st); break;
            case 18: launch_dsum_w<0, 9>(a, st); break;
            case 19: launch_dsum_w<1, 9>(a, st); break;
            case 20: launch_dsum_w<0, 10>(a, st); break;
            case 21: launch_dsum_w<1, 10>(a, st); break;
            case 22: launch_dsum_w<0, 11>(a, st); break;
            case 23: launch_dsum_w<1, 11>(a, st); break;
            default: return hipErrorInvalidValue;
        }
        return hipGetLastError();
    }
    dim3 g((unsigned)((int64_t)a.nsub * a.nblkd)), b(kBlock);
    if (a.nbin <= 2048 && a.cbd <= 128) {
        const int nbm = a.nbin <= 1024 ? 1024 : 2048;
        const size_t row = (size_t)kWaves * nbm * (a.dtype == 0 ? 4 : 8);
        const size_t lds = row > (size_t)nbm * 8 ? row : (size_t)nbm * 8;
        if (nbm == 1024) {
            if (a.dtype == 0) hipLaunchKernelGGL((k_dsum_wn<0, 1024>), g, b, lds, st, a);
            else hipLaunchKernelGGL((k_dsum_wn<1, 1024>), g, b, lds, st, a);
        } else {
            if (a.dtype == 0) hipLaunchKernelGGL((k_dsum_wn<0, 2048>), g, b, lds, st, a);
            else hipLaunchKernelGGL((k_dsum_wn<1, 2048>), g, b, lds, st, a);
        }
        return hipGetLastError();
    }
    const int jb = a.nbin >= 2048 ? 8 : (a.nbin + kBlock - 1) / kBlock;
    if (a.dtype == 0) {
        if (jb >= 8) hipLaunchKernelGGL((k_dsum<0, 8>), g, b, 0, st, a);
        else if (jb >= 4) hipLaunchKernelGGL((k_dsum<0, 4>), g, b, 0, st, a);
        else if (jb >= 2) hipLaunchKernelGGL((k_dsum<0, 2>), g, b, 0, st, a);
        else hipLaunchKernelGGL((k_dsum<0, 1>), g, b, 0, st, a);
    } else {
        if (jb >= 8) hipLaunchKernelGGL((k_dsum<1, 8>), g, b, 0, st, a);
        else if (jb >= 4) hipLaunchKernelGGL((k_dsum<1, 4>), g, b, 0, st, a);
        else if (jb >= 2) hipLaunchKernelGGL((k_dsum<1, 2>), g, b, 0, st, a);
        else hipLaunchKernelGGL((k_dsum<1, 1>), g, b, 0, st, a);
    }
    return hipGetLastError();
}

__global__ __launch_bounds__(kBlock) void k_align_phases(int nsub, int nchan, const double *results,
                                                         const double *freqs, const double *P,
                                                         const uint8_t *mask, const double *scales,
                                                         const double *errs, double *phases, double *weights) {
    const int64_t i = (int64_t)blockIdx.x * kBlock + threadIdx.x;
    if (i >= (int64_t)nsub * nchan) return;
    const int64_t s = i / nchan;
    const double *r = results + s * (int64_t)(sizeof(ppf_result) / sizeof(double));
    const double phi = r[offsetof(ppf_result, params) / sizeof(double)];
    const double DM = r[offsetof(ppf_result, params) / sizeof(double) + 1];
    const double nu_ref = r[offsetof(ppf_result, nu_out) / sizeof(double)];
    const bool ok = !mask || mask[i];
    phases[i] = ok ? phi + kDconst * DM / P[s] * (pow(freqs[i], -2.0) - pow(nu_ref, -2.0)) : 0.0;
    weights[i] = ok ? scales[i] / (errs[i] * errs[i]) : 0.0;
}

hipError_t launch_align_phases(int nsub, int nchan, const double *results, const double *freqs, const double *P,
                               const uint8_t *mask, const double *scales, const double *errs, double *phases,
                               double *weights, hipStream_t st) {
    const int64_t n = (int64_t)nsub * nchan;
    hipLaunchKernelGGL(k_align_phases, dim3((unsigned)((n + kBlock - 1) / kBlock)), dim3(kBlock), 0, st, nsub,
                       nchan, results, freqs, P, mask, scales, errs, phases, weights);
    return hipGetLastError();
}

hipError_t launch_guess(const GuessArgs &a, hipStream_t st) {
    const int zs = a.gspec ? 0 : ((a.czB && a.czP > rfft_len(a.nbin)) ? a.czP : rfft_len(a.nbin));
    size_t lds = (size_t)(zs + a.nbin / 2 + 2) * sizeof(double2) +
                 (a.gsh ? 0 : (size_t)(a.Ns + 8) * sizeof(double));
    const dim3 g((unsigned)a.nsub), b(kBlock);
    if (a.gsh) {
        if (a.gspec || is_pow2(rfft_len(a.nbin))) hipLaunchKernelGGL((k_guess<false, 0, true>), g, b, lds, st, a);
        else hipLaunchKernelGGL((k_guess<true, 0, true>), g, b, lds, st, a);
    } else if (a.czB && is_pow2(rfft_len(a.nbin))) {
        switch (a.czP) {
            case 512: hipLaunchKernelGGL((k_guess<false, 9>), g, b, lds, st, a); break;
            case 1024: hipLaunchKernelGGL((k_guess<false, 10>), g, b, lds, st, a); break;
            case 2048: hipLaunchKernelGGL((k_guess<false, 11>), g, b, lds, st, a); break;
            default: return hipErrorInvalidValue;
        }
    } else if (is_pow2(rfft_len(a.nbin))) {
        hipLaunchKernelGGL((k_guess<false, 0>), g, b, lds, st, a);
    } else {
        hipLaunchKernelGGL((k_guess<true, 0>), g, b, lds, st, a);
    }
    return hipGetLastError();
}
hipError_t launch_gauss_port(const GaussArgs &a, hipStream_t st) {
    size_t lds = (size_t)rfft_len(a.nbin) * sizeof(double2);
    dim3 g((unsigned)((int64_t)a.nport * a.nchan)), b(kBlock);
    if (!fft_len_supported(rfft_len(a.nbin))) {
        hipLaunchKernelGGL((k_gauss_port<1, false>), g, b, (size_t)a.nbin * sizeof(double), st, a);
        return hipGetLastError();
    }
    const bool mx = !is_pow2(rfft_len(a.nbin));
    switch (kmax_pow2(a.nbin / 2 + (a.nbin & 1))) {
        case 1: MXL(mx, k_gauss_port, 1, g, b, lds, st, a); break;
        case 2: MXL(mx, k_gauss_port, 2, g, b, lds, st, a); break;
        case 4: MXL(mx, k_gauss_port, 4, g, b, lds, st, a); break;
        case 8: MXL(mx, k_gauss_port, 8, g, b, lds, st, a); break;
        case 16: MXL(mx, k_gauss_port, 16, g, b, lds, st, a); break;
        default: return hipErrorInvalidValue;
    }
    return hipGetLastError();
}
hipError_t launch_rotate(const RotateArgs &a, int64_t nrows, hipStream_t st) {
    size_t lds = (size_t)rfft_len(a.nbin) * sizeof(double2);
    dim3 g((unsigned)nrows), b(kBlock);
    const bool mx = !is_pow2(rfft_len(a.nbin));
    switch (kmax_pow2(a.nbin / 2 + (a.nbin & 1))) {
        case 1: MXL(mx, k_rotate, 1, g, b, lds, st, a); break;
        case 2: MXL(mx, k_rotate, 2, g, b, lds, st, a); break;
        case 4: MXL(mx, k_rotate, 4, g, b, lds, st, a); break;
        case 8: MXL(mx, k_rotate, 8, g, b, lds, st, a); break;
        case 16: MXL(mx, k_rotate, 16, g, b, lds, st, a); break;
        default: return hipErrorInvalidValue;
    }
    return hipGetLastError();
}
hipError_t launch_inst_resp(const InstRespArgs &a, int64_t nrows, hipStream_t st) {
    const int N = a.nbin / 2;
    size_t lds = (size_t)N * sizeof(double2);
    dim3 g((unsigned)nrows), b(kBlock);
    const bool mx = !is_pow2(N);
    switch (kmax_pow2(N)) {
        case 1: MXL(mx, k_inst_resp, 1, g, b, lds, st, a); break;
        case 2: MXL(mx, k_inst_resp, 2, g, b, lds, st, a); break;
        case 4: MXL(mx, k_inst_resp, 4, g, b, lds, st, a); break;
        case 8: MXL(mx, k_inst_resp, 8, g, b, lds, st, a); break;
        case 16: MXL(mx, k_inst_resp, 16, g, b, lds, st, a); break;
        default: return hipErrorInvalidValue;
    }
    return hipGetLastError();
}
int align_groups(int nsub, int nchan) {
    int g = (2048 + nchan - 1) / nchan;
    if (g > nsub) g = nsub;
    return g < 1 ? 1 : g;
}

template <int KMAX, bool MX>
// ... 362 lines not shown
```

pulseportraiture_amd/csrc/ppf_solve.hip:

```cpp
#include <type_traits>
#include "ppf_device.hpp"
#include "ppf_internal.hpp"
#include "ppf_state.hpp"

namespace ppf {

struct Fac {
    double dphi[3];
    double t[2];
    double u[3];
    bool br_tt, br_ta, br_aa;
};

__device__ __forceinline__ void chan_derivs(const double *st, const Fac &fc, double dC[5],
                                            double dS[5], double d2C[5][5], double d2S[5][5]) {
    const double Cp = st[1], Cpp = st[2], Q1 = st[3], Q1p = st[4], Q2 = st[5];
    const double S1 = st[7], S2a = st[8], S2b = st[9];
    for (int i = 0; i < 3; ++i) { dC[i] = Cp * fc.dphi[i]; dS[i] = 0.0; }
    for (int j = 0; j < 2; ++j) { dC[3 + j] = Q1 * fc.t[j]; dS[3 + j] = S1 * fc.t[j]; }
    for (int i = 0; i < 3; ++i) {
        for (int j = 0; j < 3; ++j) { d2C[i][j] = Cpp * fc.dphi[i] * fc.dphi[j]; d2S[i][j] = 0.0; }
        for (int j = 0; j < 2; ++j) {
            d2C[i][3 + j] = d2C[3 + j][i] = fc.dphi[i] * fc.t[j] * Q1p;
            d2S[i][3 + j] = d2S[3 + j][i] = 0.0;
        }
    }
    const bool br[3] = {fc.br_tt, fc.br_ta, fc.br_aa};
    const int ii[3] = {0, 0, 1}, jj[3] = {0, 1, 1};
    for (int q = 0; q < 3; ++q) {
        double tt = fc.t[ii[q]] * fc.t[jj[q]];
        double c2, s2;
        if (br[q]) {
            c2 = 2.0 * tt * Q2 + fc.u[q] * Q1;
            s2 = tt * S2a + 2.0 * tt * S2b + fc.u[q] * S1;
        } else {
            c2 = tt * Q1;
            s2 = tt * S2a + tt * S1;
        }
        d2C[3 + ii[q]][3 + jj[q]] = d2C[3 + jj[q]][3 + ii[q]] = c2;
        d2S[3 + ii[q]][3 + jj[q]] = d2S[3 + jj[q]][3 + ii[q]] = s2;
    }
}

__device__ __forceinline__ void chan_hess(const double *st, const Fac &fc, double H[5][5]) {
    double dC[5], dS[5], d2C[5][5], d2S[5][5];
    chan_derivs(st, fc, dC, dS, d2C, d2S);
    const double C = st[0], S = st[6];
    const double iS = 1.0 / S, iS2 = iS * iS, iS3 = iS2 * iS, C2 = C * C;
    for (int i = 0; i < 5; ++i)
        for (int j = 0; j < 5; ++j)
            H[i][j] = -2.0 * (C * d2C[i][j] * iS - 0.5 * C2 * d2S[i][j] * iS2 + dC[i] * dC[j] * iS +
                              C2 * dS[i] * dS[j] * iS3 - C * (dC[i] * dS[j] + dS[i] * dC[j]) * iS2);
}

struct FitGeom {
    double P, nu_DM, nu_GM, nu_tau, tau_lin;
    int log10_tau;
    bool g_sum, g_tau, g_alpha;
};

__device__ __forceinline__ Fac make_fac(double nu, const FitGeom &g, double alpha) {
    Fac f;
    const double P = g.P;
    f.dphi[0] = 1.0;
    f.dphi[1] = kDconst * (pow(nu, -2.0) - pow(g.nu_DM, -2.0)) / P;
    f.dphi[2] = kDconst * kDconst * (pow(nu, -4.0) - pow(g.nu_GM, -4.0)) / P;
    const double lnf = log(nu / g.nu_tau);
    if (!g.g_sum) {
        f.t[0] = f.t[1] = 0.0;
        f.u[0] = f.u[1] = f.u[2] = 0.0;
    } else if (g.log10_tau) {
        f.t[0] = kLn10;
        f.t[1] = lnf;
        f.u[0] = kLn10 * kLn10;
        f.u[1] = kLn10 * lnf;
        f.u[2] = lnf * lnf;
    } else {
        f.t[0] = 1.0 / g.tau_lin;
        f.t[1] = lnf;
        f.u[0] = 0.0;
        f.u[1] = lnf / g.tau_lin;
        f.u[2] = lnf * lnf;
    }
    (void)alpha;
    f.br_tt = g.g_tau;
    f.br_aa = g.g_alpha;
    f.br_ta = g.g_alpha && g.g_tau;
    return f;
}

__device__ void wave_gates(const double *lnr, const uint8_t *mask, int nchan, double tau_lin,
                           double alpha, int log10_tau, int &g_sum, int &g_tau, int &g_alpha) {
    const int lane = threadIdx.x & 63;
    double s0 = 0.0, s1 = 0.0, s2 = 0.0;
    for (int n = lane; n < nchan; n += 64) {
        if (mask && !mask[n]) continue;
        const double l = lnr[n];
        const double tn = tau_lin * exp(alpha * l);
        s0 += tn;
        s1 += log10_tau ? kLn10 * tn : tn / tau_lin;
        s2 += l * tn;
    }
    s0 = wave_sum(s0); s1 = wave_sum(s1); s2 = wave_sum(s2);
    g_sum = s0 != 0.0;
    g_tau = g_sum && s1 != 0.0;
    g_alpha = s2 != 0.0;
}

constexpr int kClassifyBlock = 1024;
__global__ __launch_bounds__(kClassifyBlock) void k_classify(int nsub, const int32_t *fit_flags,
                                                             const double *init, int log10_tau,
                                                             int fused, int xcap, uint8_t *needx,
                                                             int32_t *xslot, uint8_t *xtile) {
    __shared__ int wtot[kClassifyBlock / 64];
    const int tid = threadIdx.x, lane = tid & 63, wave = tid >> 6;
    int base_slot = 0;
    for (int s0 = 0; s0 < nsub; s0 += kClassifyBlock) {
        const int s = s0 + tid;
        int need = 0, tile = 0;
        if (s < nsub) {
            const double x3 = init[(int64_t)s * 5 + 3];
            const double tau0 = log10_tau ? pow(10.0, x3) : x3;
            const bool scat =
                fit_flags[(int64_t)s * 5 + 3] || fit_flags[(int64_t)s * 5 + 4] || tau0 != 0.0;
            need = (!fused || scat) ? 1 : 0;
            tile = scat ? 0 : 1;
        }
        const unsigned long long bal = __ballot(need);
        const int below = __popcll(bal & ((1ull << lane) - 1ull));
        if (lane == 0) wtot[wave] = __popcll(bal);
        __syncthreads();
        int off = base_slot;
        for (int w = 0; w < wave; ++w) off += wtot[w];
        int chunk = 0;
        for (int w = 0; w < kClassifyBlock / 64; ++w) chunk += wtot[w];
        if (s < nsub) {
            const int slot = off + below;
            needx[s] = (need && slot < xcap) ? 1 : 0;
            xslot[s] = need ? (slot < xcap ? slot : -2) : -1;
            if (xtile) xtile[s] = (uint8_t)tile;
        }
        base_slot += chunk;
        __syncthreads();
    }
}

__global__ __launch_bounds__(kBlock) void k_gflag(int nsub, int nchan, const uint8_t *needx,
                                                  const int32_t *KC, const int32_t *model_index,
                                                  int klim, uint8_t *gflag) {
    const int s = blockIdx.x * kBlock + threadIdx.x;
    if (s >= nsub) return;
    int ok = 0;
    if (!needx || needx[s]) {
        const int64_t m = model_index ? model_index[s] : 0;
        int mx = 0;
        for (int n = 0; n < nchan; ++n) mx = max(mx, KC[m * nchan + n]);
        ok = mx <= klim ? 1 : 0;
    }
    gflag[s] = (uint8_t)ok;
}

hipError_t launch_gflag(int nsub, int nchan, const uint8_t *needx, const int32_t *KC,
                        const int32_t *model_index, int klim, uint8_t *gflag, hipStream_t st) {
    hipLaunchKernelGGL(k_gflag, dim3((unsigned)((nsub + kBlock - 1) / kBlock)), dim3(kBlock), 0, st,
                       nsub, nchan, needx, KC, model_index, klim, gflag);
    return hipGetLastError();
}

__global__ __launch_bounds__(kBlock) void k_tr_init(SolveArgs a) {
    const int lane = threadIdx.x & 63;
    const int s = blockIdx.x * kWaves + (threadIdx.x >> 6);
    if (s >= a.nsub) return;
    const double *fr = a.freqs + (int64_t)s * a.nchan;
    const uint8_t *mask = a.mask ? a.mask + (int64_t)s * a.nchan : nullptr;
    double sf = 0.0, cnt = 0.0;
    for (int n = lane; n < a.nchan; n += 64)
        if (!mask || mask[n]) { sf += fr[n]; cnt += 1.0; }
    sf = wave_sum(sf); cnt = wave_sum(cnt);
    TRState &S = a.state[s];
    int flagmask = 0, nf = 0;
    for (int i = 0; i < 5; ++i)
        if (a.fit_flags[(int64_t)s * 5 + i]) { flagmask |= 1 << i; ++nf; }
    double x[5];
    for (int i = 0; i < 5; ++i) x[i] = a.init[(int64_t)s * 5 + i];
    if (a.guess) x[0] = a.x0[(int64_t)s * 8 + 0];
    double lo[5], hi[5];
    int bnd = 0;
    for (int i = 0; i < 5; ++i) {
        lo[i] = -INFINITY;
        hi[i] = INFINITY;
        if (a.bounds) {
            const double l = a.bounds[((int64_t)s * 5 + i) * 2], u = a.bounds[((int64_t)s * 5 + i) * 2 + 1];
            if (l == l) lo[i] = l;
            if (u == u) hi[i] = u;
        }
        x[i] = fmin(fmax(x[i], lo[i]), hi[i]);
        if ((flagmask >> i & 1) && (lo[i] > -INFINITY || hi[i] < INFINITY)) bnd = 1;
    }
    const double tau0 = a.log10_tau ? pow(10.0, x[3]) : x[3];
    const int scat = ((flagmask & 0x18) || tau0 != 0.0) ? 1 : 0;
    const double nu_mean = sf / cnt;
    double nu_fit[3];
    for (int i = 0; i < 3; ++i) {
        nu_fit[i] = a.nu_fits[(int64_t)s * 3 + i];
        if (nu_fit[i] != nu_fit[i]) nu_fit[i] = nu_mean;
    }
    int gs = 0, gt = 0, ga = 0;
    if (scat) {
        double *lnr = a.dphi + (int64_t)s * a.nchan * 2;
        for (int n = lane; n < a.nchan; n += 64) lnr[n] = log(fr[n] / nu_fit[2]);
        wave_lds_sync();
        __builtin_amdgcn_fence(__ATOMIC_RELEASE, "workgroup");
        wave_gates(lnr, mask, a.nchan, tau0, x[4], a.log10_tau, gs, gt, ga);
    }
    if (lane == 0) {
        for (int i = 0; i < 5; ++i) { S.x[i] = x[i]; S.th[i] = x[i]; S.g[i] = 0.0; }
        S.f = 0.0;
        for (int i = 0; i < 15; ++i) S.H[i] = 0.0;
        S.newton = (a.newton && !bnd) ? 1 : 0;
        S.radius = S.newton ? kNewtonR0 : 1.0;
        int sub = 1;
        if (S.newton && scat) {
            const int ng = (a.nchan + 63) / 64;
            while (sub * 2 <= kSubsetMaxStride && sub * 2 <= ng / 2) sub *= 2;
        }
        S.sub = sub;
        S.sub0 = sub;
        S.nsubev = 0;
        S.pnorm = 0.0;
        S.pred = 0.0;
        for (int i = 0; i < 3; ++i) S.nu_fit[i] = nu_fit[i];
        S.nu_mean = nu_mean;
        S.Sd = 0.0;
        S.dof = cnt * (double)a.nbin - (double)(nf + (int)cnt);
        S.phi_guess = x[0];
        S.k = 0;
        S.status = PPF_ST_CONVERGED;
        S.nfev = 0;
        S.slot_cur = 0;
        S.slot_eval = 0;
        S.flagmask = flagmask;
        S.nchanx = (int)cnt;
        S.scat = scat;
        S.hb = 0;
        S.g_sum = gs; S.g_tau = gt; S.g_alpha = ga;
        for (int i = 0; i < 5; ++i) { S.lo[i] = lo[i]; S.hi[i] = hi[i]; }
        S.bnd = bnd;
        if (nf == 0 || cnt == 0.0) {
            S.phase = PH_DONE;
            S.status = PPF_ST_NOFIT;
        } else if (a.xslot && a.xslot[s] == -2) {
            S.phase = PH_DONE;
            S.status = PPF_ST_NOSPACE;
        } else {
            S.phase = PH_INIT;
        }
    }
    const int mmode = (a.moments && !scat && nf > 0 && cnt > 0.0) ? 1 : 0;
    if (lane == 0) {
        S.mmode = mmode;
        S.mom16 = (mmode && a.mom16) ? 1 : 0;
        S.need_mom = mmode;
        S.mtarget = 0;
        S.macc = 0;
        S.meval = 0;
        S.nmom = 0;
        S.mvalid[0] = mmode;
        S.mvalid[1] = 0;
        for (int i = 0; i < 3; ++i) { S.mc[0][i] = x[i]; S.mc[1][i] = x[i]; }
        if (a.kinds && S.phase == PH_INIT) atomicAdd(a.kinds + (mmode ? 0 : 1), 1u);
    }
    if (mmode) {
        const double P = a.P[s];
        const double nuDM2 = pow(nu_fit[0], -2.0), nuGM4 = pow(nu_fit[1], -4.0);
        double *dp = a.dphi + (int64_t)s * a.nchan * 2;
        for (int n = lane; n < a.nchan; n += 64) {
            const double nu = fr[n];
            dp[2 * n + 0] = kDconst * (pow(nu, -2.0) - nuDM2) / P;
            dp[2 * n + 1] = kDconst * kDconst * (pow(nu, -4.0) - nuGM4) / P;
        }
    }
}

constexpr int kPassChans = kBlock;

template <bool SCAT>
__global__ __launch_bounds__(kBlock) __attribute__((amdgpu_waves_per_eu(3))) void k_pass(SolveArgs a) {
    __shared__ double red[kWaves * 21];
    const int nblk = (a.nchan + kPassChans - 1) / kPassChans;
    int s, blk;
    if (nblk % 8 == 0) {
        const int x = blockIdx.x & 7, r = blockIdx.x >> 3;
        blk = x * (nblk >> 3) + r / a.nsub;
        s = r % a.nsub;
    } else {
        blk = blockIdx.x / a.nsub;
        s = blockIdx.x % a.nsub;
    }
    const TRState &S = a.state[s];
    if (S.phase == PH_DONE || S.scat != (SCAT ? 1 : 0) || S.mmode) return;
    const int lane = threadIdx.x & 63, wave = threadIdx.x >> 6;
    const int nharm = (a.nbin >> 1) + 1;
    const double *fr = a.freqs + (int64_t)s * a.nchan;
    const uint8_t *mask = a.mask ? a.mask + (int64_t)s * a.nchan : nullptr;
    const double *chan = a.chan + (int64_t)s * a.nchan * 4;
    const int mi = a.model_index ? a.model_index[s] : 0;
    double *stats = a.stats + ((int64_t)s * 2 + S.slot_eval) * a.nchan * 10;
    double th[5];
    for (int i = 0; i < 5; ++i) th[i] = S.th[i];
    const int flagmask = S.flagmask;
    FitGeom g;
    g.P = a.P[s];
    g.nu_DM = S.nu_fit[0];
    g.nu_GM = S.nu_fit[1];
    g.nu_tau = S.nu_fit[2];
    g.log10_tau = a.log10_tau;
    const double tau_lin = a.log10_tau ? pow(10.0, th[3]) : th[3];
    const double alpha = th[4];
    g.tau_lin = tau_lin;
    g.g_sum = S.g_sum; g.g_tau = S.g_tau; g.g_alpha = S.g_alpha;
    const double nuDM2 = pow(g.nu_DM, -2.0), nuGM4 = pow(g.nu_GM, -4.0);

    const bool split = S.sub >= kWaves;
    const int n = blk * kPassChans + (split ? lane : (int)threadIdx.x);
    const bool in_sub = S.sub <= 1 || ((n >> 6) % S.sub) == 0;
    const bool use_n = in_sub && n < a.nchan && (!mask || mask[n]);
    const int kend = (int)wave_max(use_n ? (double)a.KC[(int64_t)mi * a.nchan + n] : 1.0);
    int kb0 = 0, kb1 = kend;
    if (split) {
        const int Q = ((kend + 64 * kWaves - 1) / (64 * kWaves)) * 64;
        kb0 = min(kend, wave * Q);
        kb1 = min(kend, kb0 + Q);
    }
    double nu = 0.0, aa = 0.0, inv_e2 = 0.0;
    double a0 = 0.0, a1 = 0.0, a2 = 0.0;
    double q1 = 0.0, q1p = 0.0, q2 = 0.0, s0 = 0.0, t1 = 0.0, t2 = 0.0;
    if (use_n) {
        nu = fr[n];
        const double phin = th[0] + kDconst * th[1] * (pow(nu, -2.0) - nuDM2) / g.P +
                            kDconst * kDconst * th[2] * (pow(nu, -4.0) - nuGM4) / g.P;
        const double2 W = cexp2pi(phin);
        const double2 *Xc = a.X + (int64_t)(a.xslot ? a.xslot[s] : s) *
                                      a.xnh * a.nchan + n;
        const double *Pc = a.MP + (int64_t)mi * nharm * a.nchan + n;
        const int64_t xs = a.nchan;
        if (SCAT) {
            aa = kTwoPi * tau_lin * pow(nu / g.nu_tau, alpha);
            inv_e2 = chan[n * 4 + 1];
        }
        constexpr int KB = 3;
        double2 xa[KB], xb[KB];
        double pa[KB], pb[KB];
        auto ldg = [&](int kb, double2 (&xo)[KB], double (&po)[KB]) {
#pragma unroll
// ... 1108 lines not shown
            }
        }
        blk_sum<NZ_MAX + 8, PB>(accv, red);
        if (tid == 0) {
            for (int i = 0; i < NZ_MAX + 8; ++i) sh_acc[i] = accv[i];
            int nr_flag = 0;
            nz_solve(sh_acc, nzcase, a.option, nu_mean, nz, &nr_flag);
            no_root = nr_flag != 0;
            sh_misc[4] = nz[0]; sh_misc[5] = nz[1]; sh_misc[6] = nz[2];
            sh_misc[7] = no_root ? 1.0 : 0.0;
        }
        __syncthreads();
        nz[0] = sh_misc[4]; nz[1] = sh_misc[5]; nz[2] = sh_misc[6];
        no_root = sh_misc[7] != 0.0;
        __syncthreads();
    }
    if (need_nz)
        for (int i = 0; i < 3; ++i)
            if (!(nu_out[i] == nu_out[i]) || nu_out[i] == 0.0) nu_out[i] = nz[i];
    if (a.mode == PPF_MODE_LEGACY2) { nu_out[1] = nu_out[0]; nu_out[2] = g.nu_tau; }
    if (a.is_toa) {
        if (flagmask & 2) nu_out[1] = nu_out[0];
        else if (flagmask & 4) nu_out[0] = nu_out[1];
    }

    const double P = g.P;
    double phi_inf = x[0] + kDconst * x[1] * (0.0 - pow(g.nu_DM, -2.0)) / P +
                     kDconst * kDconst * x[2] * (0.0 - pow(g.nu_GM, -4.0)) / P;
    double phi_out = phi_inf + (kDconst / P) * x[1] * pow(nu_out[0], -2.0) +
                     (kDconst * kDconst / P) * x[2] * pow(nu_out[1], -4.0);
    if (fabs(phi_out) >= 0.5) phi_out = phi_out - floor(phi_out);
    if (phi_out >= 0.5) phi_out -= 1.0;
    double tau_out_lin = tau_fit_lin * pow(nu_out[2] / g.nu_tau, x[4]);
    double tau_out = a.log10_tau ? log10(tau_out_lin) : tau_out_lin;

    FitGeom go = g;
    go.nu_DM = nu_out[0];
    go.nu_GM = nu_out[1];
    go.nu_tau = nu_out[2];
    gates(go, tau_out_lin, x[4]);
    double cv[31];
    for (int i = 0; i < 31; ++i) cv[i] = 0.0;
    for (int n = tid; n < v.nchan; n += PB) {
        if (v.mask && !v.mask[n]) continue;
        const double *st = st_fit + (int64_t)n * 10;
        Fac fc = make_fac(v.fr[n], go, x[4]);
        double dC[5], dS[5], d2C[5][5], d2S[5][5];
        chan_derivs(st, fc, dC, dS, d2C, d2S);
        const double C = st[0], S = st[6], an = C / S;
        double U[5];
        for (int i = 0; i < 5; ++i) U[i] = (flagmask >> i & 1) ? -2.0 * (dC[i] - an * dS[i]) : 0.0;
        const double cinv = 1.0 / (2.0 * S);
        int q = 0;
        for (int i = 0; i < 5; ++i)
            for (int j = i; j < 5; ++j) {
                if ((flagmask >> i & 1) && (flagmask >> j & 1)) {
                    cv[q] += -2.0 * (C * d2C[i][j] / S - 0.5 * C * C * d2S[i][j] / (S * S));
                    cv[15 + q] += U[i] * U[j] * cinv;
                }
                ++q;
            }
    }
    blk_sum<31, PB>(cv, red);
    int sing = 0;
    if (tid == 0) {
        double Xm[5][5], Xi[5][5];
        double full[5][5];
        int q = 0;
        for (int i = 0; i < 5; ++i)
            for (int j = i; j < 5; ++j) { full[i][j] = full[j][i] = cv[q] - cv[15 + q]; ++q; }
        for (int i2 = 0; i2 < nf; ++i2)
            for (int j2 = 0; j2 < nf; ++j2) Xm[i2][j2] = full[idx[i2]][idx[j2]];
        if (!invert_small(Xm, Xi, nf)) sing = 1;
        for (int i2 = 0; i2 < 25; ++i2) sh_Xinv[i2] = 0.0;
        for (int i2 = 0; i2 < nf; ++i2)
            for (int j2 = 0; j2 < nf; ++j2) sh_Xinv[idx[i2] * 5 + idx[j2]] = Xi[i2][j2];
        sh_misc[8] = (double)sing;
    }
    __syncthreads();
    sing = (int)sh_misc[8];
    double Xinv[5][5];
    for (int i2 = 0; i2 < 5; ++i2)
        for (int j2 = 0; j2 < 5; ++j2) Xinv[i2][j2] = sh_Xinv[i2 * 5 + j2];
    double sn[1] = {0.0};
    for (int n = tid; n < v.nchan; n += PB) {
        const int64_t o2 = (int64_t)s * a.nchan + n;
        if (v.mask && !v.mask[n]) {
            a.scales[o2] = 0.0; a.scale_errs[o2] = 0.0; a.channel_snrs[o2] = 0.0;
            continue;
        }
        const double *st = st_fit + (int64_t)n * 10;
        Fac fc = make_fac(v.fr[n], go, x[4]);
        double dC[5], dS[5], d2C[5][5], d2S[5][5];
        chan_derivs(st, fc, dC, dS, d2C, d2S);
        const double C = st[0], S = st[6], an = C / S;
        double U[5];
#pragma unroll
        for (int i2 = 0; i2 < 5; ++i2) U[i2] = (flagmask >> i2 & 1) ? -2.0 * (dC[i2] - an * dS[i2]) : 0.0;
        double quad = 0.0;
#pragma unroll
        for (int i2 = 0; i2 < 5; ++i2)
#pragma unroll
            for (int j2 = 0; j2 < 5; ++j2)
                if ((flagmask >> i2 & 1) && (flagmask >> j2 & 1)) quad += U[i2] * Xinv[i2][j2] * U[j2];
        const double cinv = 1.0 / (2.0 * S);
        double var = 2.0 * (cinv + quad * cinv * cinv);
        double serr = (a.mode == PPF_MODE_LEGACY2) ? pow(S, -0.5) : sqrt(var);
        double csnr = an * sqrt(S);
        a.scales[o2] = an;
        a.scale_errs[o2] = serr;
        a.channel_snrs[o2] = csnr;
        sn[0] += csnr * csnr;
    }
    blk_sum<1, PB>(sn, red);
    if (tid == 0) {
        double pe[5] = {0, 0, 0, 0, 0};
        double *cov = a.covariance + (int64_t)s * 25;
        for (int i2 = 0; i2 < 25; ++i2) cov[i2] = 0.0;
        for (int i2 = 0; i2 < nf; ++i2) {
            for (int j2 = 0; j2 < nf; ++j2) cov[i2 * 5 + j2] = 2.0 * sh_Xinv[idx[i2] * 5 + idx[j2]];
            pe[idx[i2]] = sqrt(2.0 * sh_Xinv[idx[i2] * 5 + idx[i2]]);
        }
        double params[5] = {phi_out, x[1], x[2], tau_out, x[4]};
        for (int i2 = 0; i2 < 5; ++i2) { res->params[i2] = params[i2]; res->param_errs[i2] = pe[i2]; }
        for (int i2 = 0; i2 < 3; ++i2) res->nu_out[i2] = nu_out[i2];
        res->nu_fit[0] = g.nu_DM; res->nu_fit[1] = g.nu_GM; res->nu_fit[2] = g.nu_tau;
        res->chi2 = Sd + fun;
        res->red_chi2 = (Sd + fun) / dof;
        res->snr = sqrt(sn[0]);
        res->fun = fun;
        res->Sd = Sd;
        res->phi_guess = phi_guess;
        res->nfeval = (double)nfev;
        int st2 = status;
        if (no_root) st2 |= PPF_ST_NO_ROOT;
        if (sing) st2 |= PPF_ST_SINGULAR;
        if (!(fun == fun)) st2 |= PPF_ST_NONFINITE;
        res->status = (double)st2;
        res->niter = (double)k;
        res->dof = dof;
        res->nchanx = (double)nchanx;
        res->x_fit_phi = x[0];
        res->x_fit_tau = x[3];
        double npass = S.mmode ? (double)S.nmom + 1.0 : (double)nfev;
        if (!S.mmode && S.nsubev > 0) {
            const int ng = (a.nchan + 63) / 64, nsel = (ng + S.sub0 - 1) / S.sub0;
            npass -= (double)S.nsubev * (1.0 - (double)nsel / (double)ng);
        }
        res->npass = npass;
        res->reserved[0] = res->reserved[1] = 0.0;
    }
}

hipError_t launch_classify(int nsub, const int32_t *fit_flags, const double *init, int log10_tau,
                           int fused, int xcap, uint8_t *needx, int32_t *xslot, uint8_t *xtile,
                           hipStream_t st) {
    hipLaunchKernelGGL(k_classify, dim3(1), dim3(kClassifyBlock), 0, st, nsub, fit_flags, init,
                       log10_tau, fused, xcap, needx, xslot, xtile);
    return hipGetLastError();
}

hipError_t launch_tr_init(const SolveArgs &a, hipStream_t st) {
    hipLaunchKernelGGL(k_tr_init, dim3((unsigned)((a.nsub + kWaves - 1) / kWaves)), dim3(kBlock), 0,
                       st, a);
    return hipGetLastError();
}

template <bool SCAT>
static void launch_pass_t(const SolveArgs &a, hipStream_t st, dim3 g) {
    hipLaunchKernelGGL((k_pass<SCAT>), g, dim3(kBlock), 0, st, a);
}

hipError_t launch_pass(const SolveArgs &a, hipStream_t st) {
    const int nblk = (a.nchan + kPassChans - 1) / kPassChans;
    dim3 g((unsigned)((int64_t)a.nsub * nblk));
    if (a.any_plain) launch_pass_t<false>(a, st, g);
    if (a.any_scat) launch_pass_t<true>(a, st, g);
    return hipGetLastError();
}

hipError_t launch_tr_step(const SolveArgs &a, hipStream_t st) {
    const dim3 g((unsigned)((a.nsub + kWaves - 1) / kWaves));
    const bool lane = a.nsub >= 2048 && a.nchan <= 2048;
    if (lane) {
        const dim3 gl((unsigned)((a.nsub + 63) / 64));
        const size_t lds = 64 * sizeof(TRState);
        if (a.bounds) hipLaunchKernelGGL(k_tr_step_l<true>, gl, dim3(64), lds, st, a);
        else hipLaunchKernelGGL(k_tr_step_l<false>, gl, dim3(64), lds, st, a);
        hipError_t e = hipGetLastError();
        if (e != hipSuccess) return e;
        if (a.any_scat) hipLaunchKernelGGL(k_tr_gates, g, dim3(kBlock), 0, st, a);
        return hipGetLastError();
    }
    if (a.bounds)
        hipLaunchKernelGGL(k_tr_step<true>, g, dim3(kBlock), 0, st, a);
    else
        hipLaunchKernelGGL(k_tr_step<false>, g, dim3(kBlock), 0, st, a);
    return hipGetLastError();
}

hipError_t launch_moments(const SolveArgs &a, hipStream_t st) {
    const int nblk = (a.nchan + kMomChans - 1) / kMomChans;
    if (a.mom16) hipLaunchKernelGGL(k_moments<true>, dim3((unsigned)((int64_t)a.nsub * nblk)), dim3(kBlock), 0, st, a);
    else hipLaunchKernelGGL(k_moments<false>, dim3((unsigned)((int64_t)a.nsub * nblk)), dim3(kBlock), 0, st, a);
    return hipGetLastError();
}

hipError_t launch_tr_mom(const SolveArgs &a, hipStream_t st) {
    const int tb = 128;
    if (tb == 64) hipLaunchKernelGGL(k_tr_mom<64>, dim3((unsigned)a.nsub), dim3(64), 0, st, a);
    else if (tb == 128) hipLaunchKernelGGL(k_tr_mom<128>, dim3((unsigned)a.nsub), dim3(128), 0, st, a);
    else hipLaunchKernelGGL(k_tr_mom<256>, dim3((unsigned)a.nsub), dim3(256), 0, st, a);
    return hipGetLastError();
}

hipError_t launch_postfit(const SolveArgs &a, hipStream_t st) {
    const int pb = a.nchan <= 2048 ? 64 : 256;
    if (pb == 64) hipLaunchKernelGGL(k_postfit<64>, dim3((unsigned)a.nsub), dim3(64), 0, st, a);
    else hipLaunchKernelGGL(k_postfit<256>, dim3((unsigned)a.nsub), dim3(256), 0, st, a);
    return hipGetLastError();
}

size_t tr_state_bytes() { return sizeof(TRState); }
int pass_blocks(int nchan) { return (nchan + kPassChans - 1) / kPassChans; }

}

#ifdef PPF_TM_PROF
extern "C" int ppf_debug_tprof(unsigned long long *out, int reset) {
    if (hipMemcpyFromSymbol(out, HIP_SYMBOL(ppf::g_tprof), sizeof(unsigned long long) * 8) != hipSuccess)
        return -1;
    if (reset) {
        unsigned long long z[8] = {};
        if (hipMemcpyToSymbol(HIP_SYMBOL(ppf::g_tprof), z, sizeof(z)) != hipSuccess) return -1;
    }
    return 0;
}
#endif
```

pulseportraiture_amd/csrc/ppf_xspec.hip:

```cpp
#include <cstdlib>
#include <cstring>
#include <type_traits>

#include "ppf_internal.hpp"
#include "ppf_state.hpp"
#include "ppf_wfft.hpp"
#include "ppf_wfft2.hpp"

namespace ppf {

constexpr int kXW = 8;
template <int LOG2N>
__host__ __device__ constexpr int xsw() { return LOG2N == 10 ? 4 : 8; }
typedef double f64x4 __attribute__((ext_vector_type(4)));
typedef float vf2 __attribute__((ext_vector_type(2)));
typedef double vd2 __attribute__((ext_vector_type(2)));
typedef float vf4 __attribute__((ext_vector_type(4)));
#define SCHED_CUT() __builtin_amdgcn_sched_barrier(0)

__device__ __forceinline__ void block_map(int xcd_swizzle, int nblk, int &s, int &cb, int nsub = 0) {
    if (xcd_swizzle == 2) {
        const int per = nblk / 8, x = blockIdx.x % 8, r = blockIdx.x / 8;
        cb = x * per + r / nsub;
        s = r % nsub;
// ... 447 lines not shown
                    const int klo = lpp + 64 * i, khi = N - klo;
                    double2 Dlo, Dhi;
                    rfft_pair<LOG2N>(buf, klo, w, Dlo, Dhi);
                    w = cmul(w, w_step);
                    const double p0 = cabs2(Dlo), p1 = cabs2(Dhi);
                    if (klo >= a.kc) pn += p0;
                    if (khi >= a.kc) pn += p1;
                    if (klo >= 1) pd += p0;
                    pd += p1;
                    const double2 Ylo = klo == 0 ? cmk(0.0, 0.0) : cmulc(Dlo, Mr[klo]);
                    const double2 Yhi = cmulc(Dhi, Mr[khi]);
                    const double uk = (double)(klo - N / 2) * ih;
                    double2 ys = cadd(Ylo, Yhi), yd = cscale(csub(Ylo, Yhi), uk);
                    if constexpr (!SH) {
                        if (klo >= kz) ys = yd = cmk(0.0, 0.0);
                    }
                    buf[wfft::pad<LOG2N>(klo)] = ys;
                    buf[klo == 0 ? wfft::pad<LOG2N>(N / 2) : wfft::pad<LOG2N>(khi)] = yd;
            };
            const double2 *Mr = SH ? mrow : Mwave + (int64_t)n * NH;
            double2 w = w_seed;
#pragma unroll
            for (int i = 0; i < NP; ++i) {
                pair(Mr, i, w);
                SCHED_CUT();
            }
            if (lane == 0) buf[SIDE] = cmulc(Dm, Mr[N / 2]);
            const double mpow = SH ? mrow[NH].x : Pwave[n];
            if (lane == 0) {
                const double p = cabs2(Dm);
                if (N / 2 >= a.kc) pn += p;
                pd += p;
            }
            pn = wave_sum(pn);
            pd = wave_sum(pd);
            const double errs_FT = a.errs ? errs_in * sqrtN
                                          : sqrt(pn / (double)(NH - a.kc) / (double)(2 * N)) * sqrtN;
            const double inv_e2 = 1.0 / (errs_FT * errs_FT);
            if (lane == 0) {
                buf[SIDE2] = cmk(inv_e2, 0.0);
                double *chan = a.chan + crow * 4;
                chan[0] = errs_FT;
                chan[1] = inv_e2;
                chan[2] = pd * inv_e2;
                chan[3] = mpow * inv_e2;
                mres[n] = res_in;
            }
        } else if (act && n < cend && lane < 4) {
            unsigned lo = (unsigned)lane;
            asm volatile("" : "+v"(lo));
            a.chan[((int64_t)s * a.nchan + n) * 4 + lo] = 0.0;
        }
        XP(2);
        __syncthreads();
        XP(3);
        mstore();

        f64x4 d0 = {0.0, 0.0, 0.0, 0.0}, d1 = d0;
        int nb = N / 8;
        if constexpr (SH) nb = min(nb, (__builtin_amdgcn_readlane(ch_kc, n - cbase) + 3) >> 2);
#pragma unroll 4
        for (int t = 0; t < KPW / 4; ++t) {
            const int b = XW * t + wave;
            if (b >= nb) break;
            const int k = 4 * b + kk;
            const int se = wfft::pad<LOG2N>(k);
            const int so = k == 0 ? wfft::pad<LOG2N>(N / 2) : wfft::pad<LOG2N>(N - k);
            const double u = (double)(k - N / 2) * ih;
            const double v = u * u, v2 = v * v, v4 = v2 * v2, v8 = v4 * v4;
            const double bv = ((bj & 1) ? v : 1.0) * ((bj & 2) ? v2 : 1.0) * ((bj & 4) ? v4 : 1.0) *
                              ((bj & 8) ? v8 : 1.0);
            d0 = __builtin_amdgcn_mfma_f64_16x16x4f64(abase[2 * se], bv, d0, 0, 0, 0);
            d1 = __builtin_amdgcn_mfma_f64_16x16x4f64(abase[2 * so], bv, d1, 0, 0, 0);
        }
        XP(4);
        const int om = (tid >> 1) & 31, ori = tid & 1;
        double val = 0.0;
        if (om == 0) val = reinterpret_cast<const double *>(buf + SIDE)[ori];
        const double ie = reinterpret_cast<const double *>(buf + SIDE2)[0];
        __syncthreads();
        {
            double *sc = reinterpret_cast<double *>(buf);
#pragma unroll
            for (int rr = 0; rr < 4; ++rr) {
                sc[rr * 64 + lane] = d0[rr];
                sc[256 + rr * 64 + lane] = d1[rr];
            }
        }
        __syncthreads();
        {
            const int row = 2 * wave + ori;
            const int idx = (om & 1) * 256 + (row >> 2) * 64 + ((row & 3) << 4) + (om >> 1);
#pragma unroll
            for (int w2 = 0; w2 < XW; ++w2) val += reinterpret_cast<const double *>(lds + w2 * SLW)[idx];
            unsigned mo = (unsigned)(om * 2 + ori);
            asm volatile("" : "+v"(mo));
            if (live) mom[(int64_t)n * kMoments * 2 + mo] = val * ie;
        }
        __syncthreads();
        XP(5);
    }
    XP_DONE();
}

__global__ void k_btab(int N, double *Bt) {
    const int i = blockIdx.x * blockDim.x + threadIdx.x;
    if (i >= N / 2 * 16) return;
    const int k = i >> 4, j = i & 15;
    const double u = (double)(k - N / 2) * (2.0 / (double)N);
    const double v = u * u, v2 = v * v, v4 = v2 * v2, v8 = v4 * v4;
    Bt[i] = ((j & 1) ? v : 1.0) * ((j & 2) ? v2 : 1.0) * ((j & 4) ? v4 : 1.0) * ((j & 8) ? v8 : 1.0);
}

__global__ void k_model_pow(const double2 *Mft, int nrows, int nharm, double *out) {
    const int lane = threadIdx.x & 63;
    const int row = blockIdx.x * (blockDim.x >> 6) + (threadIdx.x >> 6);
    if (row >= nrows) return;
    const double2 *M = Mft + (int64_t)row * nharm;
    double acc = 0.0;
    for (int k = lane + 1; k < nharm; k += 64) acc += cabs2(M[k]);
    acc = wave_sum(acc);
    if (lane == 0) out[row] = acc;
}

__global__ __launch_bounds__(256) void k_model_sum(const double2 *Mft, int nchan, int nharm,
                                                   int nmodel, double2 *out) {
    __shared__ double2 part[16][17];
    const int kl = threadIdx.x & 15, grp = threadIdx.x >> 4;
    const int k = blockIdx.x * 16 + kl;
    const int m = blockIdx.y;
    const int per = (nchan + 15) / 16;
    const int n0 = grp * per, n1 = min(nchan, n0 + per);
    double2 acc = cmk(0.0, 0.0);
    if (k < nharm) {
        const double2 *M = Mft + (int64_t)m * nchan * nharm + k;
#pragma unroll 8
        for (int n = n0; n < n1; ++n) acc = cadd(acc, M[(int64_t)n * nharm]);
    }
    part[grp][kl] = acc;
    __syncthreads();
    if (grp == 0 && k < nharm) {
        double2 t = part[0][kl];
        for (int g = 1; g < 16; ++g) t = cadd(t, part[g][kl]);
        out[(int64_t)m * nharm + k] = t;
    }
}

constexpr int kX2W = 4;
constexpr int kX2SL = wf2::kXSlots + wf2::kSpSlots;
constexpr int kX2IE = 1041;
__device__ __forceinline__ int x2slot(int k) { return k + (k >> 6); }

template <int DT, bool GS, bool TL>
__global__ __launch_bounds__(64 * kX2W) __attribute__((amdgpu_waves_per_eu(2)))
void k_xspec_w2(XspecArgs a) {
    constexpr int N = 1024, NH = N + 1;
    constexpr bool GR = TL;
    constexpr bool LT = GR && GS;
    constexpr int MD = 4;
    using RowT = typename std::conditional<DT == 0, vf2, vd2>::type;
    extern __shared__ __attribute__((aligned(16))) double2 lds[];
    const int lane0 = threadIdx.x & 63;
    const int wave = __builtin_amdgcn_readfirstlane(threadIdx.x >> 6);
    double2 *buf = lds + wave * kX2SL;

    int s, cb;
    block_map(a.xcd_swizzle, a.nblk, s, cb, a.nsub);
    if (a.needx && !a.needx[s]) return;
    if (a.xtile ? (a.xtile[s] != 0) != TL : TL) return;
    const int cbase = cb * a.cb, cend = min(a.nchan, cbase + a.cb);
    const int nround = (a.cb + kX2W - 1) / kX2W;
    const int mi = a.model_index ? a.model_index[s] : 0;
    const uint8_t *mask = a.mask ? a.mask + (int64_t)s * a.nchan : nullptr;
    const double sqrtN = sqrt((double)N);
    const RowT *rows = reinterpret_cast<const RowT *>(a.data);
    const wf2::Seeds sd = wf2::make_seeds(lane0);
    double2 wA0, wstep;
    {
        double sn, cs;
        sincospi(-(double)wf2::pair_k0(lane0) / (double)N, &sn, &cs);
        wA0 = cmk(cs, sn);
        sincospi(-64.0 / (double)N, &sn, &cs);
        wstep = cmk(cs, sn);
    }
    double2 *Xs = a.X + (int64_t)(a.xslot ? a.xslot[s] : s) * a.xnh * a.nchan;
    int kw = NH;
    if (a.KC) {
        const int nn = (cbase & ~63) + lane0;
        kw = (int)wave_max(nn < a.nchan ? (double)a.KC[(int64_t)mi * a.nchan + nn] : 1.0);
    }
    auto store_tiles = [&](int n, const double2 *b, double ie2, bool ok) {
        const int kwp = (kw + kXTile - 1) & ~(kXTile - 1);
        double2 *Xn = Xs + (int64_t)n * kXTile + (lane0 & (kXTile - 1));
#pragma unroll 1
        for (int h = lane0; h < kwp; h += 64) {
            const double2 v = (ok && h < kw) ? cscale(b[x2slot(h)], ie2) : cmk(0.0, 0.0);
            __builtin_nontemporal_store(vd2{v.x, v.y},
                                        reinterpret_cast<vd2 *>(Xn + (int64_t)(h >> 3) * a.nchan * kXTile));
        }
    };
    const int mlane = (cbase + lane0 < cend && (!mask || mask[cbase + lane0])) ? 1 : 0;
    auto usable = [&](int n) {
        return n < cend && __builtin_amdgcn_readlane(mlane, n - cbase) != 0;
    };
    constexpr int NL = 64 * guess_npl(10);
    bool gon = false;
    double g_Dg = 0.0, g_nrm2 = 0.0, g_w2e2 = 0.0;
    double2 *gacc = lds + kX2W * kX2SL;
    if constexpr (GS) {
        gon = a.gflag[s] != 0;
        if (gon) {
            if constexpr (!GR)
                for (int t = threadIdx.x; t < NL; t += 64 * kX2W) gacc[t] = cmk(0.0, 0.0);
            const double *fr = a.freqs + (int64_t)s * a.nchan;
            double v0 = 0.0, v1 = 0.0;
            for (int nn = lane0; nn < a.nchan; nn += 64)
                if (!mask || mask[nn]) { v0 += fr[nn]; v1 += 1.0; }
            v0 = wave_sum(v0);
            v1 = wave_sum(v1);
            const double mu = v0 / v1;
            double nu_ref_m2 = 1.0 / (mu * mu);
            if (a.guess_ref) {
                const double nf = a.nu_fits[(int64_t)s * 3];
                if (nf == nf) nu_ref_m2 = 1.0 / (nf * nf);
            }
            g_Dg = readlane_d(kDconst * a.guess_DM[s] / a.P[s], 0);
            g_nrm2 = readlane_d(nu_ref_m2, 0);
            if constexpr (!GR) __syncthreads();
        }
    }
    double2 gr[8];
#pragma unroll
    for (int i = 0; i < 8; ++i) gr[i] = cmk(0.0, 0.0);
    const int nl = cbase + lane0;
    const bool lin = nl < cend;
    const double ch_mpow = lin ? a.Mpow[(int64_t)mi * a.nchan + nl] : 0.0;
    const double ch_err = (a.errs && lin) ? a.errs[(int64_t)s * a.nchan + nl] : 0.0;
    double ch_wn = 0.0, ch_dg = 0.0;
    if (GS && gon && lin) {
        ch_wn = a.guess_weights[(int64_t)s * a.nchan + nl];
        const double f = a.freqs[(int64_t)s * a.nchan + nl];
        ch_dg = g_Dg * (1.0 / (f * f) - g_nrm2);
    }
    double2 ch_e1 = cmk(1.0, 0.0);
    if constexpr (GR) {
        if (GS && gon) ch_e1 = cexp2pi(ch_dg);
    }
    double2 *ltab = lds + kX2W * kX2SL;
    if constexpr (LT) {
        if (wave == 0) {
            ltab[lane0] = sd.w1;
            ltab[64 + lane0] = sd.v1;
            ltab[128 + lane0] = wA0;
            ltab[192 + lane0] = ch_e1;
        }
        __syncthreads();
    }
    RowT zr[16];
    auto fetch = [&](int n) {
        const RowT *src = rows + ((int64_t)s * a.nchan + n) * N;
#pragma unroll
        for (int q = 0; q < 16; ++q) zr[q] = __builtin_nontemporal_load(src + lane0 + 64 * q);
    };
    auto fetch_c = [&](int m) { fetch(m < cend ? m : cend - 1); };
    auto rows_ready = [&]() {
#pragma unroll
        for (int q = 0; q < 16; ++q) asm volatile("" ::"v"(zr[q].x), "v"(zr[q].y));
    };
    int n = cbase + wave;
    fetch_c(n);
    rows_ready();
    XP_INIT();
    for (int r = 0; r < nround; ++r, n += kX2W) {
        const bool live = usable(n);
        if (n < cend && !live && lane0 < 4) a.chan[((int64_t)s * a.nchan + n) * 4 + lane0] = 0.0;
        double2 x[16];
#pragma unroll
        for (int q = 0; q < 16; ++q) {
            x[q] = cmk((double)zr[q].x, (double)zr[q].y);
            asm volatile("" : "+v"(x[q].x), "+v"(x[q].y));
        }
        int lane = lane0;
        asm volatile("" : "+v"(lane));
        const bool lo = lane <= 32;
        const int kA = wf2::pair_k0(lane);
        const int hl0 = lo ? kA : N - kA, hstep = lo ? 64 : -64;
        const double2 *Mrow = a.Mft + ((int64_t)mi * a.nchan + (n < cend ? n : cend - 1)) * NH;
        double2 Mq[MD > 0 ? MD : 1];
        auto mpre = [&]() {
#pragma unroll
            for (int i = 0; i < MD; ++i) Mq[i] = Mrow[(unsigned)(hl0 + hstep * i)];
        };
        SCHED_CUT();
        fetch_c(n + kX2W);
        if (live) {
            const int64_t crow = (int64_t)s * a.nchan + n;
            const int rr = n - cbase;
            XP(0);
            if constexpr (LT) {
                wf2::Seeds sdl;
                sdl.w1 = ltab[lane];
                sdl.v1 = ltab[64 + lane];
                wf2::fft1024(x, buf, lane, sdl);
            } else {
                wf2::fft1024(x, buf, lane, sd);
            }
            XP(1);
            SCHED_CUT();
            mpre();
            double2 zm = cmk(0.0, 0.0);
            wf2::pairs(x, buf + wf2::kXSlots, lane, zm);
            XP(2);
            double2 El = cmk(0.0, 0.0), Est = El;
            if constexpr (GR) {
                if (GS && gon) {
                    const double2 b1 = LT ? ltab[192 + rr] : cmk(readlane_d(ch_e1.x, rr), readlane_d(ch_e1.y, rr));
                    const double2 b2 = cmul(b1, b1), b4 = cmul(b2, b2), b8 = cmul(b4, b4);
                    const double2 b16 = cmul(b8, b8), b32 = cmul(b16, b16), b64 = cmul(b32, b32);
                    const int m = lane == 32 ? 32 : (lane & 31);
                    double2 pw = (m & 1) ? b1 : cmk(1.0, 0.0);
                    if (m & 2) pw = cmul(pw, b2);
                    if (m & 4) pw = cmul(pw, b4);
                    if (m & 8) pw = cmul(pw, b8);
                    if (m & 16) pw = cmul(pw, b16);
                    if (m & 32) pw = b32;
                    double2 E1 = pw;
                    if (!lo) {
                        const double2 b128 = cmul(b64, b64), b256 = cmul(b128, b128);
                        E1 = cmulc(cmul(b256, b256), pw);
                    }
                    El = cscale(E1, readlane_d(ch_wn, rr));
                    Est = lo ? b64 : cconj(b64);
                }
            } else if (GS && gon) {
                const double dg = readlane_d(ch_dg, rr);
                const double2 E1 = cexp2pi((double)hl0 * dg);
                El = cscale(E1, readlane_d(ch_wn, rr));
                Est = cmk(readlane_d(E1.x, 1), readlane_d(E1.y, 1));
#pragma unroll
                for (int q = 0; q < 6; ++q) Est = cmul(Est, Est);
                if (!lo) Est = cconj(Est);
            }
            const double sg = lo ? 1.0 : -1.0;
            const int hcut = N - a.kc;
            double pn = 0.0, pd = 0.0;
            double2 w = LT ? ltab[128 + lane] : wA0;
#pragma unroll
            for (int i = 0; i < 8; ++i) {
                const double2 zk = x[i], zn = x[i + 8];
                const double ex = zk.x + zn.x, ey = zk.y - zn.y;
                const double ox = zk.x - zn.x, oy = zk.y + zn.y;
                const double wox = fma(w.x, ox, -w.y * oy), woy = fma(w.x, oy, w.y * ox);
                w = cmul(w, wstep);
                const double ux = fma(sg, woy, ex), uy = fma(-sg, wox, ey);
                const double vx = fma(-sg, woy, ex), vy = fma(sg, wox, ey);
                const double2 Dl = cmk(ux, sg * uy);
                const double ph = fma(vx, vx, vy * vy), pl = fma(ux, ux, uy * uy);
                const int hl = hl0 + hstep * i;
                if (hl <= hcut) pn += ph;
                if (i == 0) pd += lane == 0 ? ph : pl + ph;
                else pd += pl + ph;
                double2 Ml;
                if constexpr (MD > 0) {
                    Ml = Mq[i % MD];
                    if (i + MD < 8) Mq[i % MD] = Mrow[(unsigned)(hl + hstep * MD)];
                } else {
                    Ml = Mrow[(unsigned)hl];
                }
                if (hl < kw) buf[x2slot(hl)] = cmulc(Dl, Ml);
                if (GS && gon) {
                    if constexpr (GR) gr[i] = cadd(gr[i], cmul(Dl, El));
                    else if (hl >= 1 && hl < NL) buf[x2slot(N - hl)] = cmul(Dl, El);
                    El = cmul(El, Est);
                } else if (kw > N / 2) {
                    const int hh = N - hl;
                    if (hh < kw) buf[x2slot(hh)] = cmulc(cmk(vx, -sg * vy), Mrow[(unsigned)hh]);
                }
            }
            XP(3);
            if (lane == 0) {
                buf[x2slot(0)] = cmk(0.0, 0.0);
                const double2 Dm = cmk(2.0 * zm.x, -2.0 * zm.y);
                const double p = cabs2(Dm);
                if (N / 2 >= a.kc) pn += p;
                pd += p;
                if (N / 2 < kw) buf[x2slot(N / 2)] = cmulc(Dm, Mrow[N / 2]);
            }
            pn *= 0.25;
            pd *= 0.25;
            pn = wave_sum(pn);
            pd = wave_sum(pd);
            double errs_FT;
            if (a.errs) errs_FT = readlane_d(ch_err, rr) * sqrtN;
            else errs_FT = sqrt(pn / (double)(NH - a.kc) / (double)(2 * N)) * sqrtN;
            const double inv_e2 = 1.0 / (errs_FT * errs_FT);
            if (GS && gon) {
                const double wn = readlane_d(ch_wn, rr);
                g_w2e2 += wn * wn * errs_FT * errs_FT;
            }
            const double mpow = readlane_d(ch_mpow, rr);
            if (lane == 0) {
                if constexpr (!TL) reinterpret_cast<double *>(buf + kX2IE)[0] = 0.5 * inv_e2;
                double *chan = a.chan + crow * 4;
                chan[0] = errs_FT;
                chan[1] = inv_e2;
                chan[2] = pd * inv_e2;
                chan[3] = mpow * inv_e2;
            }
            if constexpr (TL) {
                rows_ready();
                XP(4);
                wfft::wave_sync();
                store_tiles(n, buf, 0.5 * inv_e2, true);
                wfft::wave_sync();
                XP(5);
            }
        } else if constexpr (TL) {
            rows_ready();
            if (n < cend) store_tiles(n, buf, 0.0, false);
        }
        if constexpr (GR) continue;
        if (TL && !(GS && gon)) continue;
        if constexpr (!TL) {
            rows_ready();
            XP(4);
        }
        __syncthreads();
        XP(5);
        if constexpr (!TL) {
            const int c = threadIdx.x % kX2W, n0 = cbase + r * kX2W;
            const int nc = n0 + c;
            if (nc < cend) {
                const bool ok = !mask || mask[nc];
                const double2 *b = lds + c * kX2SL;
                const double ie2 = ok ? reinterpret_cast<const double *>(b + kX2IE)[0] : 0.0;
                for (int k = threadIdx.x / kX2W; k < kw; k += 64) {
                    const double2 v = ok ? cscale(b[x2slot(k)], ie2) : cmk(0.0, 0.0);
                    __builtin_nontemporal_store(vd2{v.x, v.y}, reinterpret_cast<vd2 *>(Xs + (int64_t)k * a.nchan + nc));
                }
            }
        }
        if (GS && gon) {
            for (int t = threadIdx.x; t < NL; t += 64 * kX2W) {
                if (t == 0) continue;
                double2 acc = gacc[t];
#pragma unroll
                for (int w2 = 0; w2 < kX2W; ++w2)
                    if (usable(cbase + r * kX2W + w2)) acc = cadd(acc, lds[w2 * kX2SL + x2slot(N - t)]);
                gacc[t] = acc;
            }
        }
        __syncthreads();
        XP(6);
    }
    {
        const int lane = lane0;
        (void)lane;
        XP_DONE();
    }
    if constexpr (GS) {
        if (gon) {
            double2 *gp = a.gpart + ((int64_t)s * a.nblk + cb) * NL;
            if constexpr (!GR)
                for (int t = threadIdx.x; t < NL; t += 64 * kX2W) gp[t] = cscale(gacc[t], 0.5);
            const double gwl = mlane ? a.guess_weights[(int64_t)s * a.nchan + cbase + lane0] : 0.0;
            const double wsum = wave_sum(gwl), cnt = wave_sum(mlane ? 1.0 : 0.0);
            if constexpr (GR) {
                const bool lo = lane0 <= 32;
                const int kA = wf2::pair_k0(lane0);
                const int hl0 = lo ? kA : N - kA, hstep = lo ? 64 : -64;
#pragma unroll
                for (int i = 0; i < 8; ++i) {
                    const int hl = hl0 + hstep * i;
                    if (hl >= 1 && hl < NL) buf[hl] = gr[i];
                }
            }
            if (lane0 == 0) reinterpret_cast<double *>(buf)[0] = g_w2e2;
            __syncthreads();
            if constexpr (GR) {
                for (int t = threadIdx.x; t < NL; t += 64 * kX2W) {
                    double2 acc = cmk(0.0, 0.0);
                    if (t > 0) {
                        acc = lds[t];
#pragma unroll
                        for (int w2 = 1; w2 < kX2W; ++w2) acc = cadd(acc, lds[w2 * kX2SL + t]);
                    }
                    gp[t] = cscale(acc, 0.5);
                }
            }
            if (threadIdx.x == 0) {
                double acc = 0.0;
                for (int w2 = 0; w2 < kX2W; ++w2) acc += reinterpret_cast<const double *>(lds + w2 * kX2SL)[0];
                double *o = a.gw + ((int64_t)s * a.nblk + cb) * 3;
                o[0] = wsum;
                o[1] = cnt;
                o[2] = acc;
            }
        }
    }
}

constexpr int kWmW = 4;
constexpr int kWmMaxN = 1024;

__device__ __forceinline__ int mod_small(int j, int L, float invL) {
    const int q = (int)((float)j * invL);
    int k = j - q * L;
    k += k < 0 ? L : 0;
    k -= k >= L ? L : 0;
    return k;
}

template <int R, int NMAX>
__device__ __forceinline__ void wmr_stage(double2 *buf, int N, int L, const double2 *tw, int lane) {
    constexpr int QM = (NMAX / R + 63) / 64;
    const int nb = N / R, ts = N / (R * L);
    const float invL = 1.0f / (float)L;
    double2 x[QM][R];
#pragma unroll
    for (int q = 0; q < QM; ++q) {
        const int j = lane + 64 * q;
        if (j < nb) {
            const int k = mod_small(j, L, invL);
#pragma unroll
            for (int r = 0; r < R; ++r) x[q][r] = buf[j + r * nb];
#pragma unroll
            for (int r = 1; r < R; ++r) x[q][r] = cmul(x[q][r], tw[r * k * ts]);
            dft_small<R>(x[q], false);
        }
    }
    wfft::wave_sync();
#pragma unroll
    for (int q = 0; q < QM; ++q) {
        const int j = lane + 64 * q;
        if (j < nb) {
            const int k = mod_small(j, L, invL);
            const int o = (j - k) * R + k;
#pragma unroll
            for (int r = 0; r < R; ++r) buf[o + r * L] = x[q][r];
        }
    }
    wfft::wave_sync();
}

template <int NMAX>
__device__ __forceinline__ void wmr_stage_g(double2 *buf, int N, int L, int R, const double2 *tw, int lane) {
    double2 y[NMAX / 64];
    gr_stage_read4<NMAX / 64>(buf, N, L, R, tw, false, lane, 64, y);
    wfft::wave_sync();
    gr_stage_write<NMAX / 64>(buf, N, lane, 64, y);
    wfft::wave_sync();
}

template <int DT, int NMAX, bool ODD>
__global__ __launch_bounds__(64 * kWmW) __attribute__((amdgpu_waves_per_eu(NMAX <= 512 ? 3 : 2)))
void k_xspec_wm(XspecArgs a) {
    const int N = a.nbin >> 1, NH = N + 1;
    const int NF = ODD ? a.nbin : N;
    const int SL = ODD ? NF : N + 2, IE = N + 1;
    extern __shared__ __attribute__((aligned(16))) double2 lds[];
    const int lane = threadIdx.x & 63, wave = threadIdx.x >> 6;
    double2 *buf = lds + wave * SL;
    double2 *twl = lds + kWmW * SL;
    int s, cb;
    block_map(a.xcd_swizzle, a.nblk, s, cb, a.nsub);
    if (a.needx && !a.needx[s]) return;
    for (int i = threadIdx.x; i < NF; i += 64 * kWmW) twl[i] = a.T[i];
    __syncthreads();
    const int cbase = cb * a.cb, cend = min(a.nchan, cbase + a.cb);
    const int nround = (a.cb + kWmW - 1) / kWmW;
    const int mi = a.model_index ? a.model_index[s] : 0;
    const uint8_t *mask = a.mask ? a.mask + (int64_t)s * a.nchan : nullptr;
    const double sqrtN = sqrt((double)a.nbin / 2.0);
    double2 *Xs = a.X + (int64_t)(a.xslot ? a.xslot[s] : s) * NH * a.nchan;
    int kw = NH;
    if (a.KC) {
        const int nn = (cbase & ~63) + lane;
        kw = (int)wave_max(nn < a.nchan ? (double)a.KC[(int64_t)mi * a.nchan + nn] : 1.0);
    }
    const int mlane = (cbase + lane < cend && (!mask || mask[cbase + lane])) ? 1 : 0;
    auto usable = [&](int n) {
        return n < cend && __builtin_amdgcn_readlane(mlane, n - cbase) != 0;
    };
    const int nl = cbase + lane;
    const double ch_mpow = nl < cend ? a.Mpow[(int64_t)mi * a.nchan + nl] : 0.0;
    const double ch_err = (a.errs && nl < cend) ? a.errs[(int64_t)s * a.nchan + nl] : 0.0;
    const bool two0 = !ODD && (__builtin_ctz((unsigned)N) & 1) != 0;
    using ET = typename std::conditional<DT == 0, float, double>::type;
    using LT = typename std::conditional<ODD, ET, typename std::conditional<DT == 0, float2, double2>::type>::type;
    constexpr int PJ = NMAX / 64;
    LT pre[PJ];
    auto fetch = [&](int m) {
        const LT *src = reinterpret_cast<const LT *>(a.data) + ((int64_t)s * a.nchan + m) * (int64_t)NF;
#pragma unroll
        for (int i = 0; i < PJ; ++i) {
            const int t = lane + 64 * i;
            pre[i] = ld_stream(src + (t < NF ? t : NF - 1));
        }
    };
    fetch(min(cbase + wave, cend - 1));
    for (int r = 0, n = cbase + wave; r < nround; ++r, n += kWmW) {
        const bool live = usable(n);
        if (n < cend && !live && lane < 4) a.chan[((int64_t)s * a.nchan + n) * 4 + lane] = 0.0;
        if (live) {
#pragma unroll
            for (int i = 0; i < PJ; ++i) {
                const int t = lane + 64 * i;
                if constexpr (ODD) {
                    if (t < NF) buf[t] = cmk((double)pre[i], 0.0);
                } else {
                    if (t < N) buf[t] = cmk((double)pre[i].x, (double)pre[i].y);
                }
            }
        }
        fetch(min(n + kWmW, cend - 1));
        if (live) {
            const int64_t crow = (int64_t)s * a.nchan + n;
            wfft::wave_sync();
            int L = 1, rem = NF;
            bool two = two0;
            while (rem > 1) {
                int R;
                if (two) { R = 2; two = false; }
                else if ((rem & 3) == 0) R = 4;
                else { R = 3; while (rem % R) R += 2; }
                switch (R) {
                    case 2: wmr_stage<2, NMAX>(buf, NF, L, twl, lane); break;
                    case 3: wmr_stage<3, NMAX>(buf, NF, L, twl, lane); break;
                    case 4: wmr_stage<4, NMAX>(buf, NF, L, twl, lane); break;
                    case 5: wmr_stage<5, NMAX>(buf, NF, L, twl, lane); break;
                    default: wmr_stage_g<NMAX>(buf, NF, L, R, twl, lane); break;
                }
                L *= R;
                rem /= R;
            }
            const double2 *Mrow = a.Mft + ((int64_t)mi * a.nchan + n) * NH;
            double pn = 0.0, pd = 0.0;
            for (int k = lane; ODD && k <= N; k += 64) {
                const double2 dk = buf[k];
                const double p0 = cabs2(dk);
                if (k >= a.kc) pn += p0;
                if (k >= 1) pd += p0;
                if (k < kw) buf[k] = k == 0 ? cmk(0.0, 0.0) : cmulc(dk, Mrow[k]);
            }
            for (int k = lane; !ODD && k <= N / 2; k += 64) {
                const int kn = N - k;
                const double2 dk = rfft_bin(buf, N, a.T2, k);
                const double2 dn = rfft_bin(buf, N, a.T2, kn);
                const double p0 = cabs2(dk), p1 = cabs2(dn);
                if (k >= a.kc) pn += p0;
                if (k >= 1) pd += p0;
// ... 101 lines not shown
            int L = 1, rem = NF;
            while (rem > 1) {
                int R = 3;
                while (rem % R) R += 2;
                switch (R) {
                    case 3: wmr_stage<3, NMAX>(buf, NF, L, twl, lane); break;
                    case 5: wmr_stage<5, NMAX>(buf, NF, L, twl, lane); break;
                    default: wmr_stage_g<NMAX>(buf, NF, L, R, twl, lane); break;
                }
                L *= R;
                rem /= R;
            }
            const double2 *MA = a.Mft + ((int64_t)mi * a.nchan + min(nA, cend - 1)) * NH;
            const double2 *MB = a.Mft + ((int64_t)mi * a.nchan + min(nB, cend - 1)) * NH;
            double pnA = 0.0, pdA = 0.0, pnB = 0.0, pdB = 0.0;
            for (int k = lane; k <= N; k += 64) {
                const int kn = k == 0 ? 0 : NF - k;
                const double2 zk = buf[k], c = cconj(buf[kn]);
                const double2 xa = cscale(cadd(zk, c), 0.5);
                const double2 d = csub(zk, c);
                const double2 xb = cmk(0.5 * d.y, -0.5 * d.x);
                const double qa = cabs2(xa), qb = cabs2(xb);
                if (k >= a.kc) { pnA += qa; pnB += qb; }
                if (k >= 1) { pdA += qa; pdB += qb; }
                if (k >= 1 && k < kw) {
                    buf[k] = cmulc(xa, MA[k]);
                    buf[kn] = cmulc(xb, MB[k]);
                }
            }
            pnA = wave_sum(pnA);
            pdA = wave_sum(pdA);
            pnB = wave_sum(pnB);
            pdB = wave_sum(pdB);
            const int rA = nA - cbase, rB = min(nB - cbase, 63);
            double eA, eB;
            if (a.errs) {
                eA = readlane_d(ch_err, rA) * sqrtN;
                eB = readlane_d(ch_err, rB) * sqrtN;
            } else {
                eA = sqrt(pnA / (double)(NH - a.kc) / (double)a.nbin) * sqrtN;
                eB = sqrt(pnB / (double)(NH - a.kc) / (double)a.nbin) * sqrtN;
            }
            const double ieA = 1.0 / (eA * eA), ieB = 1.0 / (eB * eB);
            const double mpA = readlane_d(ch_mpow, rA), mpB = readlane_d(ch_mpow, rB);
            if (lane == 0) {
                buf[0] = cmk(ieA, 0.0);
                buf[NF] = cmk(ieB, 0.0);
                if (liveA) {
                    double *chan = a.chan + ((int64_t)s * a.nchan + nA) * 4;
                    chan[0] = eA;
                    chan[1] = ieA;
                    chan[2] = pdA * ieA;
                    chan[3] = mpA * ieA;
                }
                if (liveB) {
                    double *chan = a.chan + ((int64_t)s * a.nchan + nB) * 4;
                    chan[0] = eB;
                    chan[1] = ieB;
                    chan[2] = pdB * ieB;
                    chan[3] = mpB * ieB;
                }
            }
        }
        __syncthreads();
        {
            const int c = threadIdx.x % RW, nc = cbase + r * RW + c;
            if (nc < cend) {
                const bool ok = !mask || mask[nc];
                const double2 *b = lds + (c % kWmW) * SL;
                const int o0 = c < kWmW ? 0 : NF, st = c < kWmW ? 1 : -1;
                const double ie2 = ok ? b[o0].x : 0.0;
                for (int k = threadIdx.x / RW; k < kw; k += 64 * kWmW / RW)
                    st_stream(Xs + (int64_t)k * a.nchan + nc, (ok && k) ? cscale(b[o0 + st * k], ie2) : cmk(0.0, 0.0));
            }
        }
        __syncthreads();
    }
}

bool xspec_wm_supported(int nbin) {
    if (nbin & 1) return nbin >= 33 && nbin < kWmMaxN;
    const int N = nbin / 2;
    return !is_pow2(N) && N <= kWmMaxN && fft_len_supported(N);
}

#define PPF_WM_LAUNCH(NM, ODD)                                                           \
    do {                                                                                 \
        if (a.dtype == 0) hipLaunchKernelGGL((k_xspec_wm<0, NM, ODD>), g, b, lds, st, a); \
        else hipLaunchKernelGGL((k_xspec_wm<1, NM, ODD>), g, b, lds, st, a);              \
    } while (0)

static bool use_xspec_wo() {
    static const bool on = [] {
        const char *e = getenv("PPF_XSPEC_WO");
        return e ? atoi(e) != 0 : true;
    }();
    return on;
}

hipError_t launch_xspec_wm(const XspecArgs &a, hipStream_t st) {
    const bool odd = a.nbin & 1;
    const int NF = rfft_len(a.nbin);
    if (odd && use_xspec_wo()) {
        const size_t lds = ((size_t)kWmW * (NF + 1) + NF) * sizeof(double2);
        dim3 g((unsigned)((int64_t)a.nsub * a.nblk)), b(64 * kWmW);
        if (NF <= 512) {
            if (a.dtype == 0) hipLaunchKernelGGL((k_xspec_wo<0, 512>), g, b, lds, st, a);
            else hipLaunchKernelGGL((k_xspec_wo<1, 512>), g, b, lds, st, a);
        } else {
            if (a.dtype == 0) hipLaunchKernelGGL((k_xspec_wo<0, 1024>), g, b, lds, st, a);
            else hipLaunchKernelGGL((k_xspec_wo<1, 1024>), g, b, lds, st, a);
        }
        return hipGetLastError();
    }
    const size_t lds = ((size_t)kWmW * (odd ? NF : NF + 2) + NF) * sizeof(double2);
    dim3 g((unsigned)((int64_t)a.nsub * a.nblk)), b(64 * kWmW);
    if (NF <= 512) {
        if (odd) PPF_WM_LAUNCH(512, true);
        else PPF_WM_LAUNCH(512, false);
    } else {
        if (odd) PPF_WM_LAUNCH(1024, true);
        else PPF_WM_LAUNCH(1024, false);
    }
    return hipGetLastError();
}

static bool use_xspec2() {
    static const bool on = [] {
        const char *e = getenv("PPF_XSPEC2");
        return e ? atoi(e) != 0 : true;
    }();
    return on;
}
bool xspec_tiled(int log2N) {
    static const bool on = [] {
        const char *e = getenv("PPF_XTILE");
        return e ? atoi(e) != 0 : true;
    }();
    return on && log2N == 10 && use_xspec2();
}

template <int L2, int DT>
static void launch_w(const XspecArgs &a, hipStream_t st) {
    if constexpr (L2 == 10) {
        if (use_xspec2()) {
            const size_t lds = (size_t)kX2W * kX2SL * sizeof(double2);
            dim3 g((unsigned)((int64_t)a.nsub * a.nblk)), b(64 * kX2W);
            if (a.xtile) {
                if (a.gflag)
                    hipLaunchKernelGGL((k_xspec_w2<DT, true, true>), g, b,
                                       lds + (size_t)256 * sizeof(double2), st, a);
                else hipLaunchKernelGGL((k_xspec_w2<DT, false, true>), g, b, lds, st, a);
            }
            if (a.gflag)
                hipLaunchKernelGGL((k_xspec_w2<DT, true, false>), g, b,
                                   lds + (size_t)guess_slots(10) * sizeof(double2), st, a);
            else hipLaunchKernelGGL((k_xspec_w2<DT, false, false>), g, b, lds, st, a);
            return;
        }
    }
    const size_t lds = ((size_t)xsw<L2>() * xspec_slw<L2>() + tw_slots<L2>()) * sizeof(double2);
    dim3 g((unsigned)((int64_t)a.nsub * a.nblk)), b(64 * xsw<L2>());
    if (a.gflag && L2 == 10)
        hipLaunchKernelGGL((k_xspec_w<L2, DT, L2 == 10>), g, b,
                           lds + (size_t)guess_slots(L2) * sizeof(double2), st, a);
    else hipLaunchKernelGGL((k_xspec_w<L2, DT, false>), g, b, lds, st, a);
}

bool xspec_wave_supported(int log2N, int cb) {
    return log2N >= 7 && log2N <= 10 && cb % xsw<7>() == 0 && cb % xsw<10>() == 0 && cb % kXW == 0;
}

hipError_t launch_xspec_wave(const XspecArgs &a, hipStream_t st) {
    switch (a.log2N * 2 + a.dtype) {
        case 14: launch_w<7, 0>(a, st); break;
        case 15: launch_w<7, 1>(a, st); break;
        case 16: launch_w<8, 0>(a, st); break;
        case 17: launch_w<8, 1>(a, st); break;
        case 18: launch_w<9, 0>(a, st); break;
        case 19: launch_w<9, 1>(a, st); break;
        case 20: launch_w<10, 0>(a, st); break;
        case 21: launch_w<10, 1>(a, st); break;
        default: return hipErrorInvalidValue;
    }
    return hipGetLastError();
}

constexpr int kNoiseW = 4;
template <int LOG2N, int DT>
__global__ __launch_bounds__(64 * kNoiseW) void k_noise_w(NoiseArgs a, int64_t nrows) {
    using P = wfft::Plan<LOG2N>;
    constexpr int N = P::N, R = P::R, NP = N / 128;
    constexpr int SL = wfft::buf_slots<LOG2N>();
    using RowT = typename std::conditional<DT == 0, vf2, vd2>::type;
    extern __shared__ __attribute__((aligned(16))) double2 lds[];
    const int lane = threadIdx.x & 63, wave = threadIdx.x >> 6;
    double2 *buf = lds + wave * SL;
    double2 *tw = lds + kNoiseW * SL;
    for (int i = threadIdx.x; i < tw_slots<LOG2N>(); i += 64 * kNoiseW) tw[i] = a.T[i];
    __syncthreads();
    const double2 w_seed = a.T2[lane], w_step = a.T2[64];
    const RowT *rows = reinterpret_cast<const RowT *>(a.in);
    const int64_t nw = (int64_t)gridDim.x * kNoiseW;
    int64_t row = (int64_t)blockIdx.x * kNoiseW + wave;
    RowT zr[R];
    auto fetch = [&](int64_t rr) {
        const RowT *src = rows + rr * N;
#pragma unroll
        for (int q = 0; q < R; ++q) zr[q] = src[lane + 64 * q];
    };
    if (row < nrows) fetch(row);
    for (; row < nrows; row += nw) {
        double2 x[R];
#pragma unroll
        for (int q = 0; q < R; ++q) x[q] = cmk((double)zr[q].x, (double)zr[q].y);
        if (row + nw < nrows) fetch(row + nw);
        wfft::fft_row<LOG2N>(x, buf, tw, lane);
        double pn = 0.0;
        double2 w = w_seed;
#pragma unroll
        for (int i = 0; i < NP; ++i) {
            const int klo = lane + 64 * i, khi = N - klo;
            double2 Dlo, Dhi;
            rfft_pair<LOG2N>(buf, klo, w, Dlo, Dhi);
            w = cmul(w, w_step);
            if (klo >= a.kc) pn += cabs2(Dlo);
            if (khi >= a.kc) pn += cabs2(Dhi);
        }
        if (lane == 0 && N / 2 >= a.kc) pn += cabs2(buf[wfft::pad<LOG2N>(N / 2)]);
        pn = wave_sum(pn);
        if (lane == 0) a.out[row] = sqrt(pn / (double)a.nbin / (double)(N + 1 - a.kc));
    }
}

template <int LOG2N, int DT>
static void launch_nw(const NoiseArgs &a, int64_t nrows, hipStream_t st) {
    const size_t lds = ((size_t)kNoiseW * wfft::buf_slots<LOG2N>() + tw_slots<LOG2N>()) * sizeof(double2);
    const int64_t want = (nrows + kNoiseW - 1) / kNoiseW;
    const unsigned grid = (unsigned)std::min<int64_t>(want, 256 * 16);
    hipLaunchKernelGGL((k_noise_w<LOG2N, DT>), dim3(grid), dim3(64 * kNoiseW), lds, st, a, nrows);
}

bool noise_wave_supported(int log2N) { return log2N >= 7 && log2N <= 10; }

hipError_t launch_noise_wave(const NoiseArgs &a, int64_t nrows, hipStream_t st) {
    switch (a.log2N * 2 + a.dtype) {
        case 14: launch_nw<7, 0>(a, nrows, st); break;
        case 15: launch_nw<7, 1>(a, nrows, st); break;
        case 16: launch_nw<8, 0>(a, nrows, st); break;
        case 17: launch_nw<8, 1>(a, nrows, st); break;
        case 18: launch_nw<9, 0>(a, nrows, st); break;
        case 19: launch_nw<9, 1>(a, nrows, st); break;
        case 20: launch_nw<10, 0>(a, nrows, st); break;
        case 21: launch_nw<10, 1>(a, nrows, st); break;
        default: return hipErrorInvalidValue;
    }
    return hipGetLastError();
}

template <int LOG2N, int DT>
__global__ __launch_bounds__(64 * kXW) void k_align_part_w(AlignArgs a) {
    using P = wfft::Plan<LOG2N>;
    constexpr int N = P::N, R = P::R, NP = N / 128;
    constexpr int SL = xspec_slw<LOG2N>();
    constexpr int SMID = SL - 2, SW = SL - 1;
    using RowT = typename std::conditional<DT == 0, vf2, vd2>::type;
    extern __shared__ __attribute__((aligned(16))) double2 lds[];
    const int lane = threadIdx.x & 63, wave = threadIdx.x >> 6;
    double2 *buf = lds + wave * SL;
    const int n = blockIdx.x % a.nchan, g = blockIdx.x / a.nchan;
    const int per = (a.nsub + a.ngroup - 1) / a.ngroup;
    const int s0 = g * per, s1 = min(a.nsub, s0 + per);
    const double2 w_seed = a.T2[lane], w_step = a.T2[64];
    const RowT *rows = reinterpret_cast<const RowT *>(a.in);
    double2 *twl = lds + kXW * SL;
    for (int i = threadIdx.x; i < tw_slots<LOG2N>(); i += 64 * kXW) twl[i] = a.T[i];
    __syncthreads();
    const double2 *tw = twl;
    double2 Alo[NP], Ahi[NP], Am = cmk(0.0, 0.0);
#pragma unroll
    for (int i = 0; i < NP; ++i) Alo[i] = Ahi[i] = cmk(0.0, 0.0);
    double wtot = 0.0;
    RowT zr[R];
    auto next_live = [&](int s) {
        while (s < s1 && a.weights[(int64_t)s * a.nchan + n] == 0.0) s += kXW;
        return s;
    };
    auto fetch = [&](int s) {
        const RowT *src = rows + ((int64_t)s * a.nchan + n) * N;
#pragma unroll
        for (int q = 0; q < R; ++q) zr[q] = ld_stream(src + lane + 64 * q);
    };
    int s = next_live(s0 + wave);
    if (s < s1) fetch(s);
    while (s < s1) {
        const int64_t row = (int64_t)s * a.nchan + n;
        const double w = a.weights[row], ph = a.phases[row];
        wtot += w;
        double2 x[R];
#pragma unroll
        for (int q = 0; q < R; ++q) x[q] = cmk((double)zr[q].x, (double)zr[q].y);
        const int sn = next_live(s + kXW);
        if (sn < s1) fetch(sn);
        wfft::fft_row<LOG2N>(x, buf, tw, lane);
        const double2 Es = cexp2pi(64.0 * ph);
        double2 E = cexp2pi((double)lane * ph);
        double2 Eh = cmul(cexp2pi((double)N * ph), cconj(E));
        double2 wt = w_seed;
#pragma unroll
        for (int i = 0; i < NP; ++i) {
            const int klo = lane + 64 * i;
            double2 Dlo, Dhi;
            rfft_pair<LOG2N>(buf, klo, wt, Dlo, Dhi);
            wt = cmul(wt, w_step);
            Alo[i] = cadd(Alo[i], cscale(cmul(Dlo, E), w));
            Ahi[i] = cadd(Ahi[i], cscale(cmul(Dhi, Eh), w));
            E = cmul(E, Es);
            Eh = cmul(Eh, cconj(Es));
        }
        if (lane == 0) {
// ... 182 lines not shown
```

Before: 323,200.

## Fuse classify/gflag with per-subint precompute and add list-driven xspec/dsum launches

```diff
diff --git a/pulseportraiture_amd/csrc/ppf_api.cpp b/pulseportraiture_amd/csrc/ppf_api.cpp
--- a/pulseportraiture_amd/csrc/ppf_api.cpp
+++ b/pulseportraiture_amd/csrc/ppf_api.cpp
@@ -165,11 +165,12 @@
 
 struct FitLayout {
     size_t M, X, chan, stats, x0, gP, gw, nuref, Msum, gpart, gwx, gflag, state, partials, active, mom, dphi,
-        mres, hcen, Mpow, MP, KC, needx, xslot, xtile, rclist, Bt, total;
+        mres, hcen, Mpow, MP, KC, needx, xslot, xtile, cls, rec, hmlist, nglist, rclist, Bt, total;
     int lng;
     size_t spec, lchirp, lA, lY, gprof, gspec, gsh;
     int64_t lrows;
     int nblk, cb, cbd, nblkd;
+    int cbx, nblkx;
     int fused;
     int momx;
     int xcap;
@@ -204,6 +205,9 @@
     L.cb = d->nchan < 32 ? d->nchan : 32;
     L.nblk = (d->nchan + L.cb - 1) / L.cb;
     L.fused = ppf::xspec_wave_supported(rfft_log2(d->nbin), L.cb) ? 1 : 0;
+    L.cbx = L.cb;
+    if (L.fused && ppf::xspec_own_cb(rfft_log2(d->nbin)) > 0) L.cbx = ppf::xspec_own_cb(rfft_log2(d->nbin));
+    L.nblkx = (d->nchan + L.cbx - 1) / L.cbx;
     const bool mom_auto = d->guess && rfft_log2(d->nbin) == 10;
     L.momx = (L.fused && !(d->options & PPF_OPT_FUSED_MOM) &&
               ((d->options & PPF_OPT_MOM_X) || mom_auto)) ? 1 : 0;
@@ -233,6 +237,10 @@
     L.needx = o; o += align256(nsub);
     L.xslot = o; o += align256(sizeof(int32_t) * nsub);
     L.xtile = o; o += L.tiled ? align256(nsub) : 0;
+    L.cls = o;   o += align256(sizeof(int32_t) * nsub);
+    L.rec = o;   o += align256(sizeof(double) * nsub * ppf::kRecN);
+    L.hmlist = o; o += align256(sizeof(int32_t) * nsub);
+    L.nglist = o; o += align256(sizeof(int32_t) * nsub);
     L.rclist = o; o += align256(sizeof(int32_t) * nsub);
     L.Bt = o;    o += align256(sizeof(double) * (nharm - 1) / 2 * 16);
     if (d->guess) {
@@ -242,8 +250,8 @@
         L.Msum = o; o += align256(sizeof(double2) * (size_t)(d->nmodel > 0 ? d->nmodel : 1) * nharm);
         if (L.fused) {
             const size_t ng = (size_t)ppf::guess_slots(rfft_log2(d->nbin));
-            L.gpart = o; o += align256(sizeof(double2) * nsub * (size_t)L.nblk * ng);
-            L.gwx = o;   o += align256(sizeof(double) * nsub * (size_t)L.nblk * 3);
+            L.gpart = o; o += align256(sizeof(double2) * nsub * (size_t)L.nblkx * ng);
+            L.gwx = o;   o += align256(sizeof(double) * nsub * (size_t)L.nblkx * 3);
             L.gflag = o; o += align256(nsub);
         }
     }
@@ -561,26 +569,34 @@
     uint8_t *needx = (uint8_t *)(ws + L.needx);
     int32_t *xslot = (int32_t *)(ws + L.xslot);
     uint8_t *xtile = L.tiled ? (uint8_t *)(ws + L.xtile) : nullptr;
-    if ((e = ppf::launch_classify(d->nsub, d->fit_flags, d->init, d->log10_tau, L.fused && !L.momx, L.xcap,
-                                  needx, xslot, xtile, st)) != hipSuccess)
-        return hip_fail(ctx, e, "k_classify");
     uint8_t *gflag = nullptr;
-    if (d->guess && L.fused && ppf::xspec_guess_fused_n(rfft_log2(d->nbin))) {
-        gflag = (uint8_t *)(ws + L.gflag);
-        const int klim = 64 * ppf::guess_npl(rfft_log2(d->nbin));
-        if ((e = ppf::launch_gflag(d->nsub, d->nchan, needx, (const int32_t *)(ws + L.KC),
-                                   d->model_index, klim, gflag, st)) != hipSuccess)
-            return hip_fail(ctx, e, "k_gflag");
-    }
+    if (d->guess && L.fused && ppf::xspec_guess_fused_n(rfft_log2(d->nbin))) gflag = (uint8_t *)(ws + L.gflag);
+    unsigned *kinds = (unsigned *)(ws + L.active + 16);
+    if ((e = hipMemsetAsync(kinds, 0, 8 * sizeof(unsigned), st)) != hipSuccess)
+        return hip_fail(ctx, e, "hipMemsetAsync");
+    ppf::ClassifyArgs ca{};
+    ca.nsub = d->nsub; ca.nchan = d->nchan; ca.log10_tau = d->log10_tau;
+    ca.fused = (L.fused && !L.momx) ? 1 : 0; ca.xcap = L.xcap;
+    ca.fit_flags = d->fit_flags; ca.init = d->init; ca.freqs = d->freqs; ca.P = d->P;
+    ca.nu_fits = d->nu_fits; ca.mask = d->chan_mask; ca.model_index = d->model_index;
+    ca.KC = (const int32_t *)(ws + L.KC);
+    ca.klim = gflag ? 64 * ppf::guess_npl(rfft_log2(d->nbin)) : -1;
+    ca.guess_DM = d->guess ? d->guess_DM : nullptr; ca.guess_ref = d->guess ? d->guess_ref : 0;
+    ca.needx = needx; ca.xslot = xslot; ca.xtile = xtile; ca.gflag = gflag;
+    ca.cls = (int32_t *)(ws + L.cls); ca.rec = (double *)(ws + L.rec);
+    ca.hm_list = (int32_t *)(ws + L.hmlist); ca.ng_list = (int32_t *)(ws + L.nglist);
+    ca.counts = kinds + 4;
+    if ((e = ppf::launch_classify(ca, st)) != hipSuccess) return hip_fail(ctx, e, "k_classify");
     mark(1);
 
     ppf::XspecArgs xa{};
     xa.nsub = d->nsub; xa.nchan = d->nchan; xa.nbin = d->nbin; xa.log2N = rfft_log2(d->nbin);
-    xa.kc = kc; xa.nblk = L.nblk; xa.cb = L.cb; xa.dtype = d->data_dtype;
+    xa.kc = kc; xa.nblk = L.nblkx; xa.cb = L.cbx; xa.dtype = d->data_dtype;
     constexpr long long kOrder2Bytes = 32ll << 20;
     const long long model_bytes = (long long)d->nchan * (d->nbin / 2 + 1) * 16;
     const int xcd1 = (L.nblk % 8 == 0) ? 1 : 0;
-    xa.xcd_swizzle = (xcd1 && model_bytes > kOrder2Bytes) ? 2 : xcd1;
+    const int xcdx = (L.nblkx % 8 == 0) ? 1 : 0;
+    xa.xcd_swizzle = (xcdx && model_bytes > kOrder2Bytes) ? 2 : xcdx;
     xa.data = d->data; xa.Mft = Mft; xa.model_index = d->model_index; xa.mask = d->chan_mask;
     xa.errs = d->errs; xa.freqs = d->freqs; xa.P = d->P; xa.T = T; xa.T2 = T2;
     xa.X = (double2 *)(ws + L.X); xa.chan = (double *)(ws + L.chan);
@@ -589,6 +605,13 @@
     xa.xtile = xtile;
     xa.xnh = L.xnh;
     xa.gflag = gflag;
+    xa.cls = ca.cls;
+    xa.rec = ca.rec;
+    const bool bounded = (d->options & PPF_OPT_NO_X) != 0;
+    if (bounded && xtile) {
+        xa.list = ca.hm_list;
+        xa.nlist = ca.counts + 1;
+    }
     if (gflag) {
         xa.gpart = (double2 *)(ws + L.gpart);
         xa.gw = (double *)(ws + L.gwx);
@@ -627,6 +650,10 @@
         da.gP = (double *)(ws + L.gP); da.gw = (double *)(ws + L.gw);
         da.nuref = (double *)(ws + L.nuref);
         da.gflag = gflag;
+        if (bounded && gflag) {
+            da.list = ca.ng_list;
+            da.nlist = ca.counts + 2;
+        }
         mark(7);
         if ((e = ppf::launch_dsum(da, st)) != hipSuccess) return hip_fail(ctx, e, "k_dsum");
         mark(8);
@@ -646,7 +673,7 @@
         ga.gflag = gflag;
         ga.gpart = xa.gpart;
         ga.gwx = xa.gw;
-        ga.nblk = L.nblk;
+        ga.nblk = L.nblkx;
         if (L.lng) {
             double *prof = (double *)(ws + L.gprof);
             double2 *gspec = (double2 *)(ws + L.gspec);
@@ -685,13 +712,12 @@
     sa.active = (unsigned *)(ws + L.active);
     sa.rc_count = sa.active + 1;
     sa.rc_list = (int32_t *)(ws + L.rclist);
-    sa.kinds = (unsigned *)(ws + L.active + 16);
+    sa.kinds = kinds;
+    sa.rec = ca.rec;
     if (!ctx->host_active) {
         e = hipHostMalloc((void **)&ctx->host_active, 4 * sizeof(unsigned));
         if (e != hipSuccess) return hip_fail(ctx, e, "hipHostMalloc");
     }
-    if ((e = hipMemsetAsync(sa.kinds, 0, 2 * sizeof(unsigned), st)) != hipSuccess)
-        return hip_fail(ctx, e, "hipMemsetAsync");
     sa.moments = use_moments;
     sa.mom = (double2 *)(ws + L.mom);
     sa.dphi = (double *)(ws + L.dphi);
diff --git a/pulseportraiture_amd/csrc/ppf_internal.hpp b/pulseportraiture_amd/csrc/ppf_internal.hpp
--- a/pulseportraiture_amd/csrc/ppf_internal.hpp
+++ b/pulseportraiture_amd/csrc/ppf_internal.hpp
@@ -36,7 +36,14 @@
     double *gw;
     const double *guess_weights, *guess_DM, *nu_fits;
     int guess_ref;
-};
+    const int32_t *cls;
+    const double *rec;
+    const int32_t *list;
+    const unsigned *nlist;
+};
+
+constexpr int kClsNeedX = 1, kClsTile = 2, kClsGflag = 4;
+constexpr int kRecNuRefM2 = 0, kRecDg = 1, kRecCnt = 2, kRecNuMean = 3, kRecN = 4;
 
 __host__ __device__ constexpr int guess_npl(int log2N) { return log2N >= 10 ? 7 : (log2N == 9 ? 3 : (log2N == 8 ? 2 : 1)); }
 __host__ __device__ constexpr int guess_slots(int log2N) { return 64 * guess_npl(log2N); }
@@ -52,6 +59,8 @@
     double *gw;
     const uint8_t *gflag;
     double *nuref;
+    const int32_t *list;
+    const unsigned *nlist;
 };
 
 struct XmomArgs {
@@ -140,6 +149,7 @@
     int xnh;
     unsigned *rc_count;
     int32_t *rc_list;
+    const double *rec;
 };
 
 struct RotateArgs {
@@ -322,19 +332,35 @@
 hipError_t launch_rfft_rows(const RfftArgs &a, int64_t nrows, hipStream_t st);
 hipError_t launch_xspec(const XspecArgs &a, hipStream_t st);
 hipError_t launch_guess(const GuessArgs &a, hipStream_t st);
-hipError_t launch_gflag(int nsub, int nchan, const uint8_t *needx, const int32_t *KC,
-                        const int32_t *model_index, int klim, uint8_t *gflag, hipStream_t st);
 hipError_t launch_dsum(const DsumArgs &a, hipStream_t st);
 bool xspec_wave_supported(int log2N, int cb);
+int xspec_own_cb(int log2N);
 bool xspec_wm_supported(int nbin);
 bool xspec_guess_fused_n(int log2N);
 hipError_t launch_xspec_wm(const XspecArgs &a, hipStream_t st);
 hipError_t launch_xspec_wave(const XspecArgs &a, hipStream_t st);
 hipError_t launch_xmom(const XmomArgs &a, bool full, hipStream_t st);
 hipError_t launch_btab(int N, double *Bt, hipStream_t st);
-hipError_t launch_classify(int nsub, const int32_t *fit_flags, const double *init, int log10_tau,
-                           int fused, int xcap, uint8_t *needx, int32_t *xslot, uint8_t *xtile,
-                           hipStream_t st);
+struct ClassifyArgs {
+    int nsub, nchan, log10_tau, fused, xcap;
+    const int32_t *fit_flags;
+    const double *init, *freqs, *P, *nu_fits;
+    const uint8_t *mask;
+    const int32_t *model_index;
+    const int32_t *KC;
+    int klim;
+    const double *guess_DM;
+    int guess_ref;
+    uint8_t *needx;
+    int32_t *xslot;
+    uint8_t *xtile;
+    uint8_t *gflag;
+    int32_t *cls;
+    double *rec;
+    int32_t *hm_list, *ng_list;
+    unsigned *counts;
+};
+hipError_t launch_classify(const ClassifyArgs &a, hipStream_t st);
 bool xspec_tiled(int log2N);
 constexpr int kXTile = 8;
 inline int64_t xtile_harm(int64_t nharm) { return (nharm + kXTile - 1) / kXTile * kXTile; }
diff --git a/pulseportraiture_amd/csrc/ppf_kernels.hip b/pulseportraiture_amd/csrc/ppf_kernels.hip
--- a/pulseportraiture_amd/csrc/ppf_kernels.hip
+++ b/pulseportraiture_amd/csrc/ppf_kernels.hip
@@ -562,7 +562,7 @@
 }
 
 template <int DT, int LOG2NB>
-__global__ __launch_bounds__(kBlock) void k_dsum_w(DsumArgs a) {
+__device__ __forceinline__ void dsum_w_block(const DsumArgs &a, const int s, const int blk) {
     using ElT = typename std::conditional<DT == 0, float, double>::type;
     typedef float vf4 __attribute__((ext_vector_type(4)));
     typedef double vd2 __attribute__((ext_vector_type(2)));
@@ -572,7 +572,6 @@
     extern __shared__ __attribute__((aligned(16))) double dlds[];
     const int lane = threadIdx.x & 63, wave = threadIdx.x >> 6;
     ElT *xs = reinterpret_cast<ElT *>(dlds) + wave * NB;
-    const int s = blockIdx.x / a.nblkd, blk = blockIdx.x % a.nblkd;
     if (a.gflag && a.gflag[s]) return;
     const uint8_t *mask = a.mask ? a.mask + (int64_t)s * a.nchan : nullptr;
     const double *fr = a.freqs + (int64_t)s * a.nchan;
@@ -657,6 +656,21 @@
         for (int w2 = 0; w2 < kWaves; ++w2) { s0 += wred[w2 * 2]; s1 += wred[w2 * 2 + 1]; }
         a.gw[((int64_t)s * a.nblkd + blk) * 2 + 0] = s0;
         a.gw[((int64_t)s * a.nblkd + blk) * 2 + 1] = s1;
+    }
+}
+
+template <int DT, int LOG2NB>
+__global__ __launch_bounds__(kBlock) void k_dsum_w(DsumArgs a) {
+    dsum_w_block<DT, LOG2NB>(a, blockIdx.x / a.nblkd, blockIdx.x % a.nblkd);
+}
+
+constexpr int kDsumListGrid = 1024;
+template <int DT, int LOG2NB>
+__global__ __launch_bounds__(kBlock) void k_dsum_w_list(DsumArgs a) {
+    const int64_t items = (int64_t)*a.nlist * a.nblkd;
+    for (int64_t it = blockIdx.x; it < items; it += gridDim.x) {
+        dsum_w_block<DT, LOG2NB>(a, a.list[it / a.nblkd], (int)(it % a.nblkd));
+        __syncthreads();
     }
 }
 
@@ -1396,8 +1410,11 @@
     constexpr int NB = 1 << L2;
     const size_t row = (size_t)kWaves * NB * (DT == 0 ? 4 : 8);
     const size_t lds = row > (size_t)NB * 8 ? row : (size_t)NB * 8;
-    hipLaunchKernelGGL((k_dsum_w<DT, L2>), dim3((unsigned)((int64_t)a.nsub * a.nblkd)), dim3(kBlock),
-                       lds, st, a);
+    if (a.list)
+        hipLaunchKernelGGL((k_dsum_w_list<DT, L2>), dim3(kDsumListGrid), dim3(kBlock), lds, st, a);
+    else
+        hipLaunchKernelGGL((k_dsum_w<DT, L2>), dim3((unsigned)((int64_t)a.nsub * a.nblkd)), dim3(kBlock),
+                           lds, st, a);
 }
 
 hipError_t launch_dsum(const DsumArgs &a_in, hipStream_t st) {
diff --git a/pulseportraiture_amd/csrc/ppf_solve.hip b/pulseportraiture_amd/csrc/ppf_solve.hip
--- a/pulseportraiture_amd/csrc/ppf_solve.hip
+++ b/pulseportraiture_amd/csrc/ppf_solve.hip
@@ -108,63 +108,107 @@
 }
 
 constexpr int kClassifyBlock = 1024;
-__global__ __launch_bounds__(kClassifyBlock) void k_classify(int nsub, const int32_t *fit_flags,
-                                                             const double *init, int log10_tau,
-                                                             int fused, int xcap, uint8_t *needx,
-                                                             int32_t *xslot, uint8_t *xtile) {
-    __shared__ int wtot[kClassifyBlock / 64];
+constexpr int kClsOk = 8;
+__global__ __launch_bounds__(kClassifyBlock) void k_classify(ClassifyArgs a) {
+    constexpr int NW = kClassifyBlock / 64;
+    __shared__ int wtot[3][NW];
+    __shared__ int is_last;
     const int tid = threadIdx.x, lane = tid & 63, wave = tid >> 6;
-    int base_slot = 0;
-    for (int s0 = 0; s0 < nsub; s0 += kClassifyBlock) {
+    {
+        const int s = blockIdx.x * NW + wave;
+        if (s < a.nsub) {
+            const double *fr = a.freqs + (int64_t)s * a.nchan;
+            const uint8_t *mask = a.mask ? a.mask + (int64_t)s * a.nchan : nullptr;
+            double sf = 0.0, cnt = 0.0;
+            for (int n = lane; n < a.nchan; n += 64)
+                if (!mask || mask[n]) { sf += fr[n]; cnt += 1.0; }
+            sf = wave_sum(sf); cnt = wave_sum(cnt);
+            double mx = 0.0;
+            if (a.klim >= 0) {
+                const int64_t m = a.model_index ? a.model_index[s] : 0;
+                for (int n = lane; n < a.nchan; n += 64) mx = fmax(mx, (double)a.KC[m * a.nchan + n]);
+                mx = wave_max(mx);
+            }
+            if (lane == 0) {
+                const double mu = sf / cnt;
+                double nu_ref_m2 = 1.0 / (mu * mu);
+                if (a.guess_ref) {
+                    const double nf = a.nu_fits[(int64_t)s * 3];
+                    if (nf == nf) nu_ref_m2 = 1.0 / (nf * nf);
+                }
+                double *rec = a.rec + (int64_t)s * kRecN;
+                rec[kRecNuRefM2] = nu_ref_m2;
+                rec[kRecDg] = a.guess_DM ? kDconst * a.guess_DM[s] / a.P[s] : 0.0;
+                rec[kRecCnt] = cnt;
+                rec[kRecNuMean] = mu;
+                const double x3 = a.init[(int64_t)s * 5 + 3];
+                const double tau0 = a.log10_tau ? pow(10.0, x3) : x3;
+                const bool scat =
+                    a.fit_flags[(int64_t)s * 5 + 3] || a.fit_flags[(int64_t)s * 5 + 4] || tau0 != 0.0;
+                a.cls[s] = ((!a.fused || scat) ? kClsNeedX : 0) |
+                           (scat ? 0 : kClsTile) |
+                           ((a.klim >= 0 && mx <= (double)a.klim) ? kClsOk : 0);
+            }
+        }
+    }
+    asm volatile("s_waitcnt vmcnt(0)" ::: "memory");
+    __syncthreads();
+    if (tid == 0) {
+        __builtin_amdgcn_fence(__ATOMIC_RELEASE, "agent");
+        asm volatile("s_waitcnt vmcnt(0)" ::: "memory");
+        const unsigned t = __hip_atomic_fetch_add(a.counts, 1u, __ATOMIC_RELAXED, __HIP_MEMORY_SCOPE_AGENT);
+        is_last = t == gridDim.x - 1 ? 1 : 0;
+        if (is_last) {
+            __builtin_amdgcn_fence(__ATOMIC_ACQUIRE, "agent");
+            asm volatile("s_waitcnt vmcnt(0)" ::: "memory");
+        }
+    }
+    __syncthreads();
+    if (!is_last) return;
+    int base[3] = {0, 0, 0};
+    for (int s0 = 0; s0 < a.nsub; s0 += kClassifyBlock) {
         const int s = s0 + tid;
-        int need = 0, tile = 0;
-        if (s < nsub) {
-            const double x3 = init[(int64_t)s * 5 + 3];
-            const double tau0 = log10_tau ? pow(10.0, x3) : x3;
-            const bool scat =
-                fit_flags[(int64_t)s * 5 + 3] || fit_flags[(int64_t)s * 5 + 4] || tau0 != 0.0;
-            need = (!fused || scat) ? 1 : 0;
-            tile = scat ? 0 : 1;
-        }
-        const unsigned long long bal = __ballot(need);
-        const int below = __popcll(bal & ((1ull << lane) - 1ull));
-        if (lane == 0) wtot[wave] = __popcll(bal);
+        const int pre = s < a.nsub ? a.cls[s] : 0;
+        const int need = pre & kClsNeedX ? 1 : 0;
+        unsigned long long bal = __ballot(need);
+        const int slot_w = __popcll(bal & ((1ull << lane) - 1ull));
+        if (lane == 0) wtot[0][wave] = __popcll(bal);
         __syncthreads();
-        int off = base_slot;
-        for (int w = 0; w < wave; ++w) off += wtot[w];
-        int chunk = 0;
-        for (int w = 0; w < kClassifyBlock / 64; ++w) chunk += wtot[w];
-        if (s < nsub) {
-            const int slot = off + below;
-            needx[s] = (need && slot < xcap) ? 1 : 0;
-            xslot[s] = need ? (slot < xcap ? slot : -2) : -1;
-            if (xtile) xtile[s] = (uint8_t)tile;
-        }
-        base_slot += chunk;
+        int slot = base[0] + slot_w;
+        for (int w = 0; w < wave; ++w) slot += wtot[0][w];
+        for (int w = 0; w < NW; ++w) base[0] += wtot[0][w];
+        const int nx = (need && slot < a.xcap) ? 1 : 0;
+        const int tile = (a.xtile && (pre & kClsTile)) ? 1 : 0;
+        const int gf = (a.gflag && nx && (pre & kClsOk)) ? 1 : 0;
+        const int in[2] = {(s < a.nsub && nx && !tile) ? 1 : 0,
+                           (s < a.nsub && a.gflag && !gf) ? 1 : 0};
+        int pos[2];
+        for (int j = 0; j < 2; ++j) {
+            bal = __ballot(in[j]);
+            pos[j] = __popcll(bal & ((1ull << lane) - 1ull));
+            if (lane == 0) wtot[1 + j][wave] = __popcll(bal);
+        }
         __syncthreads();
-    }
-}
-
-__global__ __launch_bounds__(kBlock) void k_gflag(int nsub, int nchan, const uint8_t *needx,
-                                                  const int32_t *KC, const int32_t *model_index,
-                                                  int klim, uint8_t *gflag) {
-    const int s = blockIdx.x * kBlock + threadIdx.x;
-    if (s >= nsub) return;
-    int ok = 0;
-    if (!needx || needx[s]) {
-        const int64_t m = model_index ? model_index[s] : 0;
-        int mx = 0;
-        for (int n = 0; n < nchan; ++n) mx = max(mx, KC[m * nchan + n]);
-        ok = mx <= klim ? 1 : 0;
-    }
-    gflag[s] = (uint8_t)ok;
-}
-
-hipError_t launch_gflag(int nsub, int nchan, const uint8_t *needx, const int32_t *KC,
-                        const int32_t *model_index, int klim, uint8_t *gflag, hipStream_t st) {
-    hipLaunchKernelGGL(k_gflag, dim3((unsigned)((nsub + kBlock - 1) / kBlock)), dim3(kBlock), 0, st,
-                       nsub, nchan, needx, KC, model_index, klim, gflag);
-    return hipGetLastError();
+        for (int j = 0; j < 2; ++j) {
+            pos[j] += base[1 + j];
+            for (int w = 0; w < wave; ++w) pos[j] += wtot[1 + j][w];
+            for (int w = 0; w < NW; ++w) base[1 + j] += wtot[1 + j][w];
+        }
+        if (s < a.nsub) {
+            a.needx[s] = (uint8_t)nx;
+            a.xslot[s] = need ? (nx ? slot : -2) : -1;
+            if (a.xtile) a.xtile[s] = (pre & kClsTile) ? 1 : 0;
+            if (a.gflag) a.gflag[s] = (uint8_t)gf;
+            a.cls[s] = (nx ? kClsNeedX : 0) | (tile ? kClsTile : 0) | (gf ? kClsGflag : 0);
+            if (in[0]) a.hm_list[pos[0]] = s;
+            if (in[1]) a.ng_list[pos[1]] = s;
+        }
+        __syncthreads();
+    }
+    if (tid == 0) {
+        a.counts[1] = (unsigned)base[1];
+        a.counts[2] = (unsigned)base[2];
+    }
 }
 
 __global__ __launch_bounds__(kBlock) void k_tr_init(SolveArgs a) {
@@ -173,10 +217,7 @@
     if (s >= a.nsub) return;
     const double *fr = a.freqs + (int64_t)s * a.nchan;
     const uint8_t *mask = a.mask ? a.mask + (int64_t)s * a.nchan : nullptr;
-    double sf = 0.0, cnt = 0.0;
-    for (int n = lane; n < a.nchan; n += 64)
-        if (!mask || mask[n]) { sf += fr[n]; cnt += 1.0; }
-    sf = wave_sum(sf); cnt = wave_sum(cnt);
+    const double cnt = a.rec[(int64_t)s * kRecN + kRecCnt];
     TRState &S = a.state[s];
     int flagmask = 0, nf = 0;
     for (int i = 0; i < 5; ++i)
@@ -199,7 +240,7 @@
     }
     const double tau0 = a.log10_tau ? pow(10.0, x[3]) : x[3];
     const int scat = ((flagmask & 0x18) || tau0 != 0.0) ? 1 : 0;
-    const double nu_mean = sf / cnt;
+    const double nu_mean = a.rec[(int64_t)s * kRecN + kRecNuMean];
     double nu_fit[3];
     for (int i = 0; i < 3; ++i) {
         nu_fit[i] = a.nu_fits[(int64_t)s * 3 + i];
@@ -1614,11 +1655,9 @@
     }
 }
 
-hipError_t launch_classify(int nsub, const int32_t *fit_flags, const double *init, int log10_tau,
-                           int fused, int xcap, uint8_t *needx, int32_t *xslot, uint8_t *xtile,
-                           hipStream_t st) {
-    hipLaunchKernelGGL(k_classify, dim3(1), dim3(kClassifyBlock), 0, st, nsub, fit_flags, init,
-                       log10_tau, fused, xcap, needx, xslot, xtile);
+hipError_t launch_classify(const ClassifyArgs &a, hipStream_t st) {
+    constexpr int NW = kClassifyBlock / 64;
+    hipLaunchKernelGGL(k_classify, dim3((unsigned)((a.nsub + NW - 1) / NW)), dim3(kClassifyBlock), 0, st, a);
     return hipGetLastError();
 }
 
diff --git a/pulseportraiture_amd/csrc/ppf_xspec.hip b/pulseportraiture_amd/csrc/ppf_xspec.hip
--- a/pulseportraiture_amd/csrc/ppf_xspec.hip
+++ b/pulseportraiture_amd/csrc/ppf_xspec.hip
@@ -623,8 +623,7 @@
 __device__ __forceinline__ int x2slot(int k) { return k + (k >> 6); }
 
 template <int DT, bool GS, bool TL>
-__global__ __launch_bounds__(64 * kX2W) __attribute__((amdgpu_waves_per_eu(2)))
-void k_xspec_w2(XspecArgs a) {
+__device__ __forceinline__ void xspec_w2_block(const XspecArgs &a, const int s, const int cb) {
     constexpr int N = 1024, NH = N + 1;
     constexpr bool GR = TL;
     constexpr bool LT = GR && GS;
@@ -635,16 +634,49 @@
     const int wave = __builtin_amdgcn_readfirstlane(threadIdx.x >> 6);
     double2 *buf = lds + wave * kX2SL;
 
-    int s, cb;
-    block_map(a.xcd_swizzle, a.nblk, s, cb, a.nsub);
-    if (a.needx && !a.needx[s]) return;
-    if (a.xtile ? (a.xtile[s] != 0) != TL : TL) return;
     const int cbase = cb * a.cb, cend = min(a.nchan, cbase + a.cb);
-    const int nround = (a.cb + kX2W - 1) / kX2W;
+    const int nround = (cend - cbase + kX2W - 1) / kX2W;
+    const RowT *rows = reinterpret_cast<const RowT *>(a.data);
+    RowT zr[16];
+    auto fetch = [&](int n) {
+        const RowT *src = rows + ((int64_t)s * a.nchan + n) * N;
+#pragma unroll
+        for (int q = 0; q < 16; ++q) zr[q] = __builtin_nontemporal_load(src + lane0 + 64 * q);
+    };
+    auto fetch_c = [&](int m) { fetch(m < cend ? m : cend - 1); };
+    auto rows_ready = [&]() {
+#pragma unroll
+        for (int q = 0; q < 16; ++q) asm volatile("" ::"v"(zr[q].x), "v"(zr[q].y));
+    };
+    int n = cbase + wave;
+    if constexpr (TL) fetch_c(n);
+    const int cls = a.cls[s];
     const int mi = a.model_index ? a.model_index[s] : 0;
+    const int xsl = a.xslot ? a.xslot[s] : s;
+    double g_Dg = 0.0, g_nrm2 = 0.0, g_w2e2 = 0.0;
+    if constexpr (GS) {
+        g_Dg = readfirst_d(a.rec[(int64_t)s * kRecN + kRecDg]);
+        g_nrm2 = readfirst_d(a.rec[(int64_t)s * kRecN + kRecNuRefM2]);
+    }
+    if (a.needx && !(cls & kClsNeedX)) return;
+    if (((cls & kClsTile) != 0) != TL) return;
+    const bool gon = GS && (cls & kClsGflag) != 0;
     const uint8_t *mask = a.mask ? a.mask + (int64_t)s * a.nchan : nullptr;
+    const int nl = cbase + lane0;
+    const bool lin = nl < cend;
+    const int nlc = lin ? nl : cend - 1;
+    const int64_t scn = (int64_t)s * a.nchan + nlc;
+    const int nkw = (cbase & ~63) + lane0;
+    int ld_kc = a.KC ? a.KC[(int64_t)mi * a.nchan + (nkw < a.nchan ? nkw : a.nchan - 1)] : 0;
+    int ld_mask = mask ? mask[nlc] : 1;
+    double ld_mpow = a.Mpow[(int64_t)mi * a.nchan + nlc];
+    double ld_err = a.errs ? a.errs[scn] : 0.0;
+    double ld_wn = 0.0, ld_f = 1.0;
+    if constexpr (GS) {
+        ld_wn = a.guess_weights[scn];
+        ld_f = a.freqs[scn];
+    }
     const double sqrtN = sqrt((double)N);
-    const RowT *rows = reinterpret_cast<const RowT *>(a.data);
     const wf2::Seeds sd = wf2::make_seeds(lane0);
     double2 wA0, wstep;
     {
@@ -654,12 +686,10 @@
         sincospi(-64.0 / (double)N, &sn, &cs);
         wstep = cmk(cs, sn);
     }
-    double2 *Xs = a.X + (int64_t)(a.xslot ? a.xslot[s] : s) * a.xnh * a.nchan;
+    asm volatile("" : "+v"(ld_kc), "+v"(ld_mask), "+v"(ld_mpow), "+v"(ld_err), "+v"(ld_wn), "+v"(ld_f));
+    double2 *Xs = a.X + (int64_t)xsl * a.xnh * a.nchan;
     int kw = NH;
-    if (a.KC) {
-        const int nn = (cbase & ~63) + lane0;
-        kw = (int)wave_max(nn < a.nchan ? (double)a.KC[(int64_t)mi * a.nchan + nn] : 1.0);
-    }
+    if (a.KC) kw = (int)wave_max(nkw < a.nchan ? (double)ld_kc : 1.0);
     auto store_tiles = [&](int n, const double2 *b, double ie2, bool ok) {
         const int kwp = (kw + kXTile - 1) & ~(kXTile - 1);
         double2 *Xn = Xs + (int64_t)n * kXTile + (lane0 & (kXTile - 1));
@@ -670,48 +700,27 @@
                                         reinterpret_cast<vd2 *>(Xn + (int64_t)(h >> 3) * a.nchan * kXTile));
         }
     };
-    const int mlane = (cbase + lane0 < cend && (!mask || mask[cbase + lane0])) ? 1 : 0;
+    const int mlane = (lin && ld_mask) ? 1 : 0;
     auto usable = [&](int n) {
         return n < cend && __builtin_amdgcn_readlane(mlane, n - cbase) != 0;
     };
     constexpr int NL = 64 * guess_npl(10);
-    bool gon = false;
-    double g_Dg = 0.0, g_nrm2 = 0.0, g_w2e2 = 0.0;
     double2 *gacc = lds + kX2W * kX2SL;
-    if constexpr (GS) {
-        gon = a.gflag[s] != 0;
+    if constexpr (GS && !GR) {
         if (gon) {
-            if constexpr (!GR)
-                for (int t = threadIdx.x; t < NL; t += 64 * kX2W) gacc[t] = cmk(0.0, 0.0);
-            const double *fr = a.freqs + (int64_t)s * a.nchan;
-            double v0 = 0.0, v1 = 0.0;
-            for (int nn = lane0; nn < a.nchan; nn += 64)
-                if (!mask || mask[nn]) { v0 += fr[nn]; v1 += 1.0; }
-            v0 = wave_sum(v0);
-            v1 = wave_sum(v1);
-            const double mu = v0 / v1;
-            double nu_ref_m2 = 1.0 / (mu * mu);
-            if (a.guess_ref) {
-                const double nf = a.nu_fits[(int64_t)s * 3];
-                if (nf == nf) nu_ref_m2 = 1.0 / (nf * nf);
-            }
-            g_Dg = readlane_d(kDconst * a.guess_DM[s] / a.P[s], 0);
-            g_nrm2 = readlane_d(nu_ref_m2, 0);
-            if constexpr (!GR) __syncthreads();
+            for (int t = threadIdx.x; t < NL; t += 64 * kX2W) gacc[t] = cmk(0.0, 0.0);
+            __syncthreads();
         }
     }
     double2 gr[8];
 #pragma unroll
     for (int i = 0; i < 8; ++i) gr[i] = cmk(0.0, 0.0);
-    const int nl = cbase + lane0;
-    const bool lin = nl < cend;
-    const double ch_mpow = lin ? a.Mpow[(int64_t)mi * a.nchan + nl] : 0.0;
-    const double ch_err = (a.errs && lin) ? a.errs[(int64_t)s * a.nchan + nl] : 0.0;
+    const double ch_mpow = lin ? ld_mpow : 0.0;
+    const double ch_err = (a.errs && lin) ? ld_err : 0.0;
     double ch_wn = 0.0, ch_dg = 0.0;
     if (GS && gon && lin) {
-        ch_wn = a.guess_weights[(int64_t)s * a.nchan + nl];
-        const double f = a.freqs[(int64_t)s * a.nchan + nl];
-        ch_dg = g_Dg * (1.0 / (f * f) - g_nrm2);
+        ch_wn = ld_wn;
+        ch_dg = g_Dg * (1.0 / (ld_f * ld_f) - g_nrm2);
     }
     double2 ch_e1 = cmk(1.0, 0.0);
     if constexpr (GR) {
@@ -727,19 +736,7 @@
         }
         __syncthreads();
     }
-    RowT zr[16];
-    auto fetch = [&](int n) {
-        const RowT *src = rows + ((int64_t)s * a.nchan + n) * N;
-#pragma unroll
-        for (int q = 0; q < 16; ++q) zr[q] = __builtin_nontemporal_load(src + lane0 + 64 * q);
-    };
-    auto fetch_c = [&](int m) { fetch(m < cend ? m : cend - 1); };
-    auto rows_ready = [&]() {
-#pragma unroll
-        for (int q = 0; q < 16; ++q) asm volatile("" ::"v"(zr[q].x), "v"(zr[q].y));
-    };
-    int n = cbase + wave;
-    fetch_c(n);
+    if constexpr (!TL) fetch_c(n);
     rows_ready();
     XP_INIT();
     for (int r = 0; r < nround; ++r, n += kX2W) {
@@ -934,7 +931,7 @@
             double2 *gp = a.gpart + ((int64_t)s * a.nblk + cb) * NL;
             if constexpr (!GR)
                 for (int t = threadIdx.x; t < NL; t += 64 * kX2W) gp[t] = cscale(gacc[t], 0.5);
-            const double gwl = mlane ? a.guess_weights[(int64_t)s * a.nchan + cbase + lane0] : 0.0;
+            const double gwl = mlane ? ch_wn : 0.0;
             const double wsum = wave_sum(gwl), cnt = wave_sum(mlane ? 1.0 : 0.0);
             if constexpr (GR) {
                 const bool lo = lane0 <= 32;
@@ -968,6 +965,25 @@
                 o[2] = acc;
             }
         }
+    }
+}
+
+template <int DT, bool GS, bool TL>
+__global__ __launch_bounds__(64 * kX2W) __attribute__((amdgpu_waves_per_eu(2)))
+void k_xspec_w2(XspecArgs a) {
+    int s, cb;
+    block_map(a.xcd_swizzle, a.nblk, s, cb, a.nsub);
+    xspec_w2_block<DT, GS, TL>(a, s, cb);
+}
+
+constexpr int kX2ListGrid = 512;
+template <int DT, bool GS>
+__global__ __launch_bounds__(64 * kX2W) __attribute__((amdgpu_waves_per_eu(2)))
+void k_xspec_w2_list(XspecArgs a) {
+    const int64_t items = (int64_t)*a.nlist * a.nblk;
+    for (int64_t it = blockIdx.x; it < items; it += gridDim.x) {
+        xspec_w2_block<DT, GS, false>(a, a.list[it / a.nblk], (int)(it % a.nblk));
+        __syncthreads();
     }
 }
 
@@ -1375,10 +1391,15 @@
                                        lds + (size_t)256 * sizeof(double2), st, a);
                 else hipLaunchKernelGGL((k_xspec_w2<DT, false, true>), g, b, lds, st, a);
             }
-            if (a.gflag)
-                hipLaunchKernelGGL((k_xspec_w2<DT, true, false>), g, b,
-                                   lds + (size_t)guess_slots(10) * sizeof(double2), st, a);
-            else hipLaunchKernelGGL((k_xspec_w2<DT, false, false>), g, b, lds, st, a);
+            const dim3 gh = a.list ? dim3(kX2ListGrid) : g;
+            if (a.gflag) {
+                const size_t ldg = lds + (size_t)guess_slots(10) * sizeof(double2);
+                if (a.list) hipLaunchKernelGGL((k_xspec_w2_list<DT, true>), gh, b, ldg, st, a);
+                else hipLaunchKernelGGL((k_xspec_w2<DT, true, false>), gh, b, ldg, st, a);
+            } else {
+                if (a.list) hipLaunchKernelGGL((k_xspec_w2_list<DT, false>), gh, b, lds, st, a);
+                else hipLaunchKernelGGL((k_xspec_w2<DT, false, false>), gh, b, lds, st, a);
+            }
             return;
         }
     }
@@ -1389,6 +1410,8 @@
                            lds + (size_t)guess_slots(L2) * sizeof(double2), st, a);
     else hipLaunchKernelGGL((k_xspec_w<L2, DT, false>), g, b, lds, st, a);
 }
+
+int xspec_own_cb(int log2N) { return (log2N == 10 && use_xspec2()) ? 64 : 0; }
 
 bool xspec_wave_supported(int log2N, int cb) {
     return log2N >= 7 && log2N <= 10 && cb % xsw<7>() == 0 && cb % xsw<10>() == 0 && cb % kXW == 0;
```

After: 335,200, median of 6. +3.7%, better.
